# feixue94/sfd2

Measured on AMD Instinct MI355X. Metric: images/sec extract+match (1600x1200, n4096), higher is better.
Workload: dtype f16c

## Files before the change

sfd2_amd/csrc/api_core.hip:

```cpp
#include "sfd2_ctx.h"

static thread_local std::string g_err;
int sfd2_fail(const std::string &m)
{
    g_err = m;
    return -1;
}

std::atomic<unsigned long long> g_alloc_gen{0};

thread_local int g_sfd2_cu_limit = 0;

extern "C" int sfd2_version(void) { return 112; }
extern "C" const char *sfd2_last_error(void) { return g_err.c_str(); }

extern "C" int sfd2_ctx_create(int device, sfd2_ctx **out)
{
    if (!out) return fail("sfd2_ctx_create: out is null");
    int ndev = 0;
    hipError_t e = hipGetDeviceCount(&ndev);
    if (e != hipSuccess || ndev <= 0) return fail("sfd2_ctx_create: no HIP device available (libsfd2hip has no CPU fallback)");
    if (device < 0 || device >= ndev) return fail("sfd2_ctx_create: bad device index");
    HIPCHECK(hipSetDevice(device));
    sfd2_ctx *c = new sfd2_ctx();
    c->device = device;
    HIPCHECK(hipStreamCreateWithFlags(&c->stream, hipStreamNonBlocking));
    for (int i = 0; i < 4; ++i) HIPCHECK(hipEventCreate(&c->ev[i]));
    HIPCHECK(hipEventCreateWithFlags(&c->ev_jobs, hipEventDisableTiming));
    HIPCHECK(hipStreamCreateWithFlags(&c->copy_stream, hipStreamNonBlocking));
    HIPCHECK(hipStreamCreateWithFlags(&c->side_stream, hipStreamNonBlocking));
    HIPCHECK(hipEventCreateWithFlags(&c->ev_fork, hipEventDisableTiming));
    HIPCHECK(hipEventCreateWithFlags(&c->ev_join, hipEventDisableTiming));
    c->cur_stream = c->stream;
    for (int i = 0; i < SFD2_IMG_SLOTS; ++i) {
        HIPCHECK(hipEventCreateWithFlags(&c->ev_copied[i], hipEventDisableTiming));
        HIPCHECK(hipEventCreateWithFlags(&c->ev_img_free[i], hipEventDisableTiming));
    }
    c->fuse = sfd2_env("SFD2_NO_FUSE") ? 0 : 1;
    HIPCHECK(c->zero_page.ensure(SFD2_ZERO_PAGE_BYTES + ((size_t)SFD2_RS_COUNT * (SFD2_RANGE_SUB + 1) + 4) * sizeof(unsigned int)));
    HIPCHECK(hipMemset(c->zero_page.p, 0, c->zero_page.cap));
    c->range_stat.p = c->zero_page.as<char>() + SFD2_ZERO_PAGE_BYTES;
    c->range_hist_dev.p = c->range_stat.as<unsigned int>() + SFD2_RS_COUNT * SFD2_RANGE_SUB;
    c->extract_rec.p = c->range_hist_dev.as<unsigned int>() + SFD2_RS_COUNT;
    static_assert(SFD2_RS_COUNT == SFD2_RANGE_TENSORS && AE_COUNT == SFD2_RANGE_GROUPS, "include/sfd2_hip.h and the internal tables agree");

    *out = c;
    return 0;
}

extern "C" int sfd2_device_pci_bus_id(int device, char *out, int len, int *n_devices)
{
    int ndev = 0;
    hipError_t e = hipGetDeviceCount(&ndev);
    if (e != hipSuccess || ndev <= 0) return fail("sfd2_device_pci_bus_id: no HIP device available");
    if (n_devices) *n_devices = ndev;
    if (device < 0 || device >= ndev) return fail("sfd2_device_pci_bus_id: bad device index");
    if (!out || len < 13) return fail("sfd2_device_pci_bus_id: buffer of at least 13 bytes needed");
    HIPCHECK(hipDeviceGetPCIBusId(out, len, device));
    return 0;
}

extern "C" void sfd2_ctx_destroy(sfd2_ctx *c)
{
    if (!c) return;
    (void)hipSetDevice(c->device);
    (void)hipStreamSynchronize(c->stream);
    graphs_release(c);
    for (int i = 0; i < 4; ++i) if (c->ev[i]) (void)hipEventDestroy(c->ev[i]);
    if (c->ev_jobs) (void)hipEventDestroy(c->ev_jobs);
    for (int i = 0; i < SFD2_IMG_SLOTS; ++i) {
        if (c->ev_copied[i]) (void)hipEventDestroy(c->ev_copied[i]);
        if (c->ev_img_free[i]) (void)hipEventDestroy(c->ev_img_free[i]);
    }
    if (c->copy_stream) (void)hipStreamDestroy(c->copy_stream);
    if (c->side_stream) (void)hipStreamDestroy(c->side_stream);
    if (c->ev_fork) (void)hipEventDestroy(c->ev_fork);
    if (c->ev_join) (void)hipEventDestroy(c->ev_join);
    for (hipEvent_t e : c->prof_ev) (void)hipEventDestroy(e);
    if (c->pin_jobs) (void)hipHostFree(c->pin_jobs);
    if (c->stream) (void)hipStreamDestroy(c->stream);
    delete c;
}

extern "C" void *sfd2_get_stream(sfd2_ctx *c) { return c ? (void *)c->stream : nullptr; }

extern "C" int sfd2_set_precision(sfd2_ctx *c, int mode)
{
    if (!c) return fail("sfd2_set_precision: null ctx");
    if (mode != SFD2_PREC_F16 && mode != SFD2_PREC_F32 && mode != SFD2_PREC_F16X3 && mode != SFD2_PREC_F16C)
        return fail("sfd2_set_precision: unknown mode");
    HIPCHECK(hipSetDevice(c->device));
    HIPCHECK(hipStreamSynchronize(c->stream));
    if (mode != c->precision) graphs_release(c);
    c->precision = mode;
    return sfd2_margin_selfcheck_if_pending(c);
}

extern "C" int sfd2_set_option(sfd2_ctx *c, const char *key, int value)
{
    if (!c || !key) return fail("sfd2_set_option: null argument");
    HIPCHECK(hipSetDevice(c->device));
    HIPCHECK(hipStreamSynchronize(c->stream));
    const std::string k(key);
    graphs_release(c);
    if (k == "fuse") c->fuse = value ? 1 : 0;
    else if (k == "fuse_det") c->fuse_det = value ? 1 : 0;
    else if (k == "alias") c->opt_alias = value ? 1 : 0;
    else if (k == "graphs") c->use_graphs = value ? 1 : 0;
    else if (k == "branches") c->opt_branches = value ? 1 : 0;
    else if (k == "sta_side") c->opt_sta_side = value ? 1 : 0;
    else if (k == "fuse_post") c->opt_fuse_post = value ? 1 : 0;
    else if (k == "sparse_desc") c->opt_sparse_desc = value ? 1 : 0;
    else if (k == "sparse_da3") c->opt_sparse_da3 = value ? 1 : 0;
    else if (k == "cu_limit") c->opt_cu_limit = value < 0 ? 0 : value;
    else if (k == "auto_range") c->opt_auto_range = value ? 1 : 0;
    else if (k == "range_fallback") c->opt_range_fallback = value ? 1 : 0;
    else if (k == "x3_pp") c->opt_x3_pp = value ? 1 : 0;
    else if (k == "x3_desc16") c->opt_x3_desc16 = value ? 1 : 0;
    else if (k == "auto_margin") c->opt_auto_margin = value ? 1 : 0;
    else if (k == "fp6_filters") c->opt_fp6_filters = value ? 1 : 0;
    else if (k == "fp6_acts") c->opt_fp6_acts = value ? 1 : 0;
    else if (k == "s2d") c->opt_s2d = value ? 1 : 0;
    else if (k == "trunk_r1") c->opt_trunk_r1 = value ? 1 : 0;
    else if (k == "fuse_pb") c->opt_fuse_pb = value ? 1 : 0;
    else if (k == "generic_c") c->opt_generic_c = value ? 1 : 0;
    else if (k == "comp_rb") c->opt_comp_rb = value ? 1 : 0;
    else if (k == "no_rf_c") c->opt_no_rf_c = value ? 1 : 0;
    else if (k == "comp_heads") { c->opt_comp_heads = c->user_comp_heads = value ? 1 : 0; c->user_set_comp_heads = true; }
    else if (k == "c3b_plain") { c->user_c3b_plain = value < 0 ? -1 : (value ? 1 : 0); c->opt_c3b_plain = value > 0 ? 1 : 0; }
    else if (k == "comp_det") c->opt_comp_det = value ? 1 : 0;
    else if (k == "fuse_rb23") c->opt_fuse_rb23 = value ? 1 : 0;
    else if (k == "rb_inner") { c->opt_rb_inner = c->user_rb_inner = value < 0 ? 0 : (value > 2 ? 2 : value); c->user_set_rb_inner = true; }
    else return fail("sfd2_set_option: unknown key '" + k + "'");
    return 0;
}

extern "C" int sfd2_get_option(sfd2_ctx *c, const char *key, int *value)
{
    if (!c || !key || !value) return fail("sfd2_get_option: null argument");
    const std::string k(key);
    const struct { const char *name; int v; } tab[] = {
        {"fuse", c->fuse}, {"fuse_det", c->fuse_det}, {"alias", c->opt_alias}, {"graphs", c->use_graphs}, {"branches", c->opt_branches}, {"sta_side", c->opt_sta_side},
        {"fuse_post", c->opt_fuse_post}, {"sparse_desc", c->opt_sparse_desc}, {"sparse_da3", c->opt_sparse_da3}, {"cu_limit", c->opt_cu_limit},
        {"auto_range", c->opt_auto_range}, {"range_fallback", c->opt_range_fallback}, {"x3_pp", c->opt_x3_pp}, {"x3_desc16", c->opt_x3_desc16},
        {"auto_margin", c->opt_auto_margin}, {"fp6_filters", c->opt_fp6_filters}, {"fp6_acts", c->opt_fp6_acts}, {"s2d", c->opt_s2d},
        {"trunk_r1", c->opt_trunk_r1}, {"fuse_pb", c->opt_fuse_pb}, {"generic_c", c->opt_generic_c}, {"comp_rb", c->opt_comp_rb},
        {"no_rf_c", c->opt_no_rf_c}, {"comp_heads", c->opt_comp_heads}, {"c3b_plain", c->opt_c3b_plain}, {"comp_det", c->opt_comp_det},
        {"fuse_rb23", c->opt_fuse_rb23}, {"rb_inner", c->opt_rb_inner},
    };
    for (const auto &e : tab)
        if (k == e.name) { *value = e.v; return 0; }
    return fail("sfd2_get_option: unknown key '" + k + "'");
}

extern "C" int sfd2_sync(sfd2_ctx *c)
{
    if (!c) return fail("sfd2_sync: null ctx");
    HIPCHECK(hipSetDevice(c->device));
    HIPCHECK(hipStreamSynchronize(c->stream));
    return 0;
}

extern "C" int sfd2_set_profiling(sfd2_ctx *c, int max_steps)
{
    if (!c) return fail("sfd2_set_profiling: null ctx");
    HIPCHECK(hipSetDevice(c->device));
    HIPCHECK(hipStreamSynchronize(c->stream));
    if (max_steps < 0 || max_steps > 4096) return fail("sfd2_set_profiling: max_steps out of range");
    const size_t need = (size_t)max_steps * PROF_SLOTS * 2;
    while (c->prof_ev.size() < need) {
        hipEvent_t e;
        HIPCHECK(hipEventCreate(&e));
        c->prof_ev.push_back(e);
    }
    c->prof_max_steps = max_steps;
    c->prof_step = 0;
    c->prof_slot = 0;
    c->prof_used.assign(max_steps, 0);
    c->prof_row.assign((size_t)max_steps * PROF_SLOTS, 0);
    c->prof_tab.clear();
    return 0;
}

extern "C" int sfd2_set_profile_filter(sfd2_ctx *c, const char *substr)
{
    if (!c) return fail("sfd2_set_profile_filter: null ctx");
    c->prof_filter = substr ? substr : "";
    return 0;
}

extern "C" int sfd2_get_layer_timings(sfd2_ctx *c, sfd2_layer_timing *out, int cap, int *n)
{
    if (!c || !n) return fail("sfd2_get_layer_timings: null argument");
    HIPCHECK(hipSetDevice(c->device));
    HIPCHECK(hipStreamSynchronize(c->stream));
    for (int st = 0; st < c->prof_step; ++st)
        for (int sl = 0; sl < c->prof_used[st]; ++sl) {
            float ms = 0.0f;
            const size_t e = ((size_t)st * PROF_SLOTS + sl) * 2;
            const int row = c->prof_row[(size_t)st * PROF_SLOTS + sl];
            if (hipEventElapsedTime(&ms, c->prof_ev[e], c->prof_ev[e + 1]) == hipSuccess) {
                c->prof_tab[row].ms_total += ms;
                c->prof_tab[row].launches += 1;
            }
        }
    c->prof_step = 0;
    *n = (int)c->prof_tab.size();
    if (out)
        for (int i = 0; i < *n && i < cap; ++i) out[i] = c->prof_tab[i];
    return 0;
}

extern "C" int sfd2_get_timings(sfd2_ctx *c, sfd2_timings *out)
{
    if (!c || !out) return fail("sfd2_get_timings: null argument");
    *out = c->tim;
    return 0;
}

static const int kRsGroup[SFD2_RS_COUNT] = {AE_CONV1A, AE_CONV1B, AE_CONV2A, AE_CONV2B, AE_CONV3A, AE_TRUNK, AE_T1_0, AE_T1_1, AE_T1_2,
                                            AE_T2_0, AE_T2_1, AE_T2_2, AE_TRUNK, AE_TRUNK, AE_TRUNK, AE_PA0, AE_DA0};
extern "C" const char *sfd2_range_tensor_name(int i)
{
    static const char *names[SFD2_RS_COUNT] = {"conv1a", "conv1b", "conv2a", "conv2b", "conv3a", "conv3b", "conv4.0.t1", "conv4.1.t1", "conv4.2.t1",
                                               "conv4.0.t2", "conv4.1.t2", "conv4.2.t2", "conv4.0", "conv4.1", "conv4.2", "convPa.0", "convDa.0"};
    return (i >= 0 && i < SFD2_RS_COUNT) ? names[i] : "";
}

static int fetch_range_words(sfd2_ctx *c, unsigned int *raw , bool clear)
{
    const size_t bytes = (size_t)SFD2_RS_COUNT * (SFD2_RANGE_SUB + 1) * sizeof(unsigned int);
    HIPCHECK(hipMemcpyAsync(raw, c->range_stat.p, bytes, hipMemcpyDeviceToHost, c->stream));
    if (clear) HIPCHECK(hipMemsetAsync(c->range_stat.p, 0, bytes, c->stream));
    HIPCHECK(hipStreamSynchronize(c->stream));
    return 0;
}

int read_range_status(sfd2_ctx *c, sfd2_range_status *out, int reset)
{
    unsigned int raw[SFD2_RS_COUNT * (SFD2_RANGE_SUB + 1)];
    if (fetch_range_words(c, raw, reset != 0)) return -1;
    std::memset(out, 0, sizeof(*out));
    out->n_tensors = SFD2_RS_COUNT;
    const unsigned int sat_bits = 0x44E00000u;
    for (int t = 0; t < SFD2_RS_COUNT; ++t) {
        unsigned int m = raw[SFD2_RS_COUNT * SFD2_RANGE_SUB + t];
        for (int s = 0; s < SFD2_RANGE_SUB; ++s) m = std::max(m, raw[t * SFD2_RANGE_SUB + s]);
        float f;
        std::memcpy(&f, &m, 4);
        const bool sat = m >= sat_bits || c->range_hist[t] >= SFD2_C_SAT;
        if (!(f >= c->range_hist[t])) f = c->range_hist[t];
        if (reset) c->range_hist[t] = 0.0f;
        const int e = c->act_exp[kRsGroup[t]];
        out->max_stored[t] = f;
        out->max_value[t] = std::ldexp(f, -e);
        out->exponent[t] = e;
        if (sat) out->saturated |= 1u << t;
        if (f > 0.0f && f < 0.03125f) out->low |= 1u << t;
    }
    out->fallbacks = c->range_fallbacks;
    return 0;
}

int reset_range_records(sfd2_ctx *c)
{
    if (!c->range_stat.p) return 0;
    HIPCHECK(hipMemsetAsync(c->range_stat.p, 0, (size_t)SFD2_RS_COUNT * (SFD2_RANGE_SUB + 1) * sizeof(unsigned int), c->stream));
    for (int t = 0; t < SFD2_RS_COUNT; ++t) c->range_hist[t] = 0.0f;
    return 0;
}

int range_fold_before_sync_extract(sfd2_ctx *c)
{
    if (c->precision != SFD2_PREC_F16C || !c->opt_range_fallback || c->in_fallback) return 0;
    launch_extract_record(c->stream, c->range_stat.as<unsigned int>(), c->range_hist_dev.as<unsigned int>(), nullptr, 0, 0, nullptr);
    HIPCHECK(hipGetLastError());
    return 0;
}

extern "C" int sfd2_get_range_status(sfd2_ctx *c, sfd2_range_status *out, int reset)
{
    if (!c || !out) return fail("sfd2_get_range_status: null argument");
    HIPCHECK(hipSetDevice(c->device));
    return read_range_status(c, out, reset);
}

int range_wants_fallback(sfd2_ctx *c)
{
    if (c->precision != SFD2_PREC_F16C || !c->opt_range_fallback || c->in_fallback) return 0;
    unsigned int raw[SFD2_RS_COUNT * SFD2_RANGE_SUB];
    HIPCHECK(hipMemcpyAsync(raw, c->range_stat.p, sizeof(raw), hipMemcpyDeviceToHost, c->stream));
    HIPCHECK(hipStreamSynchronize(c->stream));
    bool sat = false;
    float mx[SFD2_RS_COUNT];
    for (int t = 0; t < SFD2_RS_COUNT; ++t) {
        unsigned int m = 0;
        for (int s = 0; s < SFD2_RANGE_SUB; ++s) m = std::max(m, raw[t * SFD2_RANGE_SUB + s]);
        std::memcpy(&mx[t], &m, 4);
        sat = sat || m >= 0x44E00000u;
    }
    if (!sat) return 0;
// ... 20 lines not shown
```

sfd2_amd/csrc/api_extract.hip:

```cpp
#include "sfd2_ctx.h"

static int release_image_slot(sfd2_ctx *c);
static int stage_image(sfd2_ctx *c, const void *x, int on_device, int H, int W, const float **dev, int u8 = 0)
{
    if (u8 == 2) {
        const float *raw = nullptr;
        if (on_device) raw = static_cast<const float *>(x);
        else if (stage_image(c, x, 0, H, W, &raw, 3)) return -1;
        HIPCHECK(c->img_u8_packed.ensure((size_t)3 * H * W + 16));
        launch_unpack_rgbx(c->stream, reinterpret_cast<const unsigned char *>(raw), c->img_u8_packed.as<unsigned char>(), (size_t)H * W);
        if (release_image_slot(c)) return -1;
        *dev = c->img_u8_packed.as<float>();
        return 0;
    }
    if (on_device) { *dev = static_cast<const float *>(x); return 0; }
    const size_t bytes = u8 == 3 ? (size_t)4 * H * W : (size_t)3 * H * W * (u8 ? 1 : sizeof(float));
    const int slot = c->img_slot = (c->img_slot + 1) % SFD2_IMG_SLOTS;
    HIPCHECK(c->img2[slot].ensure(bytes));
    HIPCHECK(hipStreamWaitEvent(c->copy_stream, c->ev_img_free[slot], 0));
    HIPCHECK(hipMemcpyAsync(c->img2[slot].p, x, bytes, hipMemcpyHostToDevice, c->copy_stream));
    HIPCHECK(hipEventRecord(c->ev_copied[slot], c->copy_stream));
    HIPCHECK(hipStreamWaitEvent(c->stream, c->ev_copied[slot], 0));
    c->img_slot_used = slot;
    *dev = c->img2[slot].as<float>();
    return 0;
}

static int release_image_slot(sfd2_ctx *c)
{
    if (c->img_slot_used >= 0) {
        HIPCHECK(hipEventRecord(c->ev_img_free[c->img_slot_used], c->stream));
        c->img_slot_used = -1;
    }
    return 0;
}

static int extract_begin(sfd2_ctx *c, int flags)
{
    c->prof_step_entry = c->prof_step;
    if (!(flags & SFD2_FLAG_ASYNC) && range_fold_before_sync_extract(c)) return -1;
    return 0;
}

int copy_out(sfd2_ctx *c, void *dst, const void *src_dev, size_t bytes, int dst_on_device)
{
    if (!dst || bytes == 0) return 0;
    HIPCHECK(hipMemcpyAsync(dst, src_dev, bytes, dst_on_device ? hipMemcpyDeviceToDevice : hipMemcpyDeviceToHost, c->stream));
    return 0;
}

extern "C" int sfd2_det(sfd2_ctx *c, const float *x, int x_on_device, int H, int W, int flags, float *score,
                        float *stability, float *desc, int out_on_device, int *hs, int *ws, int *hc, int *wc)
{
    if (!c || !x) return fail("sfd2_det: null argument");
    if (!c->weights_loaded) return fail("sfd2_det: weights not loaded");
    if (stability && !c->has_sta) return fail("sfd2_det: stability requested but the loaded state_dict has no ConvSta");
    HIPCHECK(hipSetDevice(c->device));
    const PassPlan plan = plan_pass(c, PASS_DET, H, W);
    if (ensure_workspace(c, plan, H, W)) return -1;
    const float *img = nullptr;
    if (stage_image(c, x, x_on_device, H, W, &img)) return -1;
    prof_step_begin(c);
    if (run_network(c, plan, img, (flags & SFD2_FLAG_IMG_NORMALISED) ? 0 : 1)) return -1;
    if (release_image_slot(c)) return -1;
    prof_step_end(c);
    const int HS = 8 * c->H8, WS = 8 * c->W8;
    if (hs) *hs = HS;
    if (ws) *ws = WS;
    if (hc) *hc = c->H4;
    if (wc) *wc = c->W4;
    if (copy_out(c, score, c->score.p, (size_t)HS * WS * sizeof(float), out_on_device)) return -1;
    if (stability) {
        HIPCHECK(c->stab.ensure((size_t)H * W * sizeof(float)));
        launch_heatmap(c->stream, c->score.as<float>(), HS, WS, c->sta.as<float>(), c->H4, c->W4, H, W, nullptr,
                       c->stab.as<float>());
        if (copy_out(c, stability, c->stab.p, (size_t)H * W * sizeof(float), out_on_device)) return -1;
    }
    if (desc) {
        const size_t n = (size_t)c->H4 * c->W4;
        HIPCHECK(c->desc_nchw.ensure(n * 128 * sizeof(float)));
        launch_desc_normalise_nchw(c->stream, c->draw.as<float>(), (int)n, c->desc_nchw.as<float>());
        if (copy_out(c, desc, c->desc_nchw.p, n * 128 * sizeof(float), out_on_device)) return -1;
    }
    HIPCHECK(hipGetLastError());
    if (!(flags & SFD2_FLAG_ASYNC)) HIPCHECK(hipStreamSynchronize(c->stream));
    return 0;
}

static int run_selection(sfd2_ctx *c, const float *heat_dev, int H, int W, float conf_th, int radius, int border,
                         int top_k, float *nms_dense, float *kpts_dev = nullptr, float *scores_dev = nullptr,
                         int Hb = 0, int Wb = 0)
{
    if (Hb <= 0) Hb = H;
    if (Wb <= 0) Wb = W;
    if (radius < 0 || radius > 4) return fail("nms radius must be in [0,4] (reference uses 4)");
    const int sel_cap = top_k > 0 ? std::min(top_k, c->cand_cap) : c->cand_cap;
    c->last_sel_cap = sel_cap;
    HIPCHECK(c->sel.ensure((size_t)sel_cap * 8));
    HIPCHECK(c->sorted.ensure((size_t)sel_cap * 8));
    HIPCHECK(c->kpts.ensure((size_t)sel_cap * 2 * sizeof(float)));
    HIPCHECK(c->kscores.ensure((size_t)sel_cap * sizeof(float)));
    if (!c->counters_clean) HIPCHECK(hipMemsetAsync(c->counters.p, 0, SFD2_COUNTER_BYTES, c->stream));
    c->counters_clean = false;
    bool threshold_done = false;
    {
        ProfScope ps(c, "nms_select", "nms_select_kernel", 0.0, (double)H * W * 4);
        threshold_done = launch_nms_select(c->stream, heat_dev, H, W, radius, conf_th, border, Hb, Wb, nms_dense,
                                           c->cand.as<unsigned long long>(), c->cand_cap, c->counters.as<unsigned int>(), 1, top_k);
    }
    {
        ProfScope ps(c, "topk_sort", "hist_select+compact+rank_sort", 0.0, (double)sel_cap * 24);
        c->kpts_cur = kpts_dev ? kpts_dev : c->kpts.as<float>();
        c->kscores_cur = scores_dev ? scores_dev : c->kscores.as<float>();
        launch_topk_sort(c->stream, threshold_done, c->cand.as<unsigned long long>(), c->cand_cap, top_k,
                         c->sel.as<unsigned long long>(), c->sorted.as<unsigned long long>(), sel_cap,
                         c->counters.as<unsigned int>(), c->bnd.as<unsigned long long>(), W, c->kpts_cur, c->kscores_cur);
    }
    HIPCHECK(hipGetLastError());
    return 0;
}

static int read_counts(sfd2_ctx *c, int64_t cap_out, int *n_out)
{
    unsigned int cnt[4] = {0, 0, 0, 0};
    HIPCHECK(hipMemcpyAsync(cnt, c->counters.p, sizeof(cnt), hipMemcpyDeviceToHost, c->stream));
    HIPCHECK(hipStreamSynchronize(c->stream));
    c->tim.n_candidates = cnt[0];
    if (cnt[0] > (unsigned int)c->cand_cap)
        return fail("candidate buffer overflow: " + std::to_string(cnt[0]) + " NMS survivors > capacity " +
                    std::to_string(c->cand_cap));
    int64_t n = cnt[1];
    if (n > c->last_sel_cap) n = c->last_sel_cap;
    if (cap_out >= 0 && n > cap_out) n = cap_out;
    if (n_out) *n_out = (int)n;
    return 0;
}

extern "C" int sfd2_extract(sfd2_ctx *c, const void *img, int img_on_device, int H, int W, float conf_th, int top_k,
                            int flags, float *kpts_xy, float *scores, float *desc, int out_on_device, int64_t cap_out,
                            int *n_out)
{
    if (!c || !img) return fail("sfd2_extract: null argument");
    if (!c->weights_loaded) return fail("sfd2_extract: weights not loaded");
    if (!(flags & SFD2_FLAG_NO_STABILITY) && !c->has_sta)
        return fail("sfd2_extract: the loaded state_dict has no ConvSta; pass SFD2_FLAG_NO_STABILITY (use_stability=False)");
    HIPCHECK(hipSetDevice(c->device));
    if (extract_begin(c, flags)) return -1;
    const PassPlan plan = plan_pass(c, PASS_EXTRACT, H, W, top_k, desc != nullptr);
    if (ensure_workspace(c, plan, H, W)) return -1;
    const float *img_dev = nullptr;
    const int u8 = (flags & SFD2_FLAG_IMG_U8_HWC) ? 1 : 0;
    if (u8 && (flags & SFD2_FLAG_IMG_NORMALISED)) return fail("sfd2_extract: a uint8 image cannot be pre-normalised");
    if ((flags & SFD2_FLAG_IMG_BGR) && !u8) return fail("sfd2_extract: SFD2_FLAG_IMG_BGR needs SFD2_FLAG_IMG_U8_HWC");
    if ((flags & SFD2_FLAG_IMG_U8_X) && !u8) return fail("sfd2_extract: SFD2_FLAG_IMG_U8_X needs SFD2_FLAG_IMG_U8_HWC");
    if (stage_image(c, img, img_on_device, H, W, &img_dev, u8 ? ((flags & SFD2_FLAG_IMG_U8_X) ? 2 : 1) : 0)) return -1;
    HIPCHECK(hipEventRecord(c->ev[0], c->stream));
    prof_step_begin(c);
    const int in_mode = ((flags & SFD2_FLAG_IMG_NORMALISED) ? 0 : 1) | (u8 ? 2 : 0) | ((flags & SFD2_FLAG_IMG_BGR) ? 4 : 0);
    if (run_network(c, plan, img_dev, in_mode)) return -1;
    if (release_image_slot(c)) return -1;
    HIPCHECK(hipEventRecord(c->ev[1], c->stream));
    const int HS = 8 * c->H8, WS = 8 * c->W8;
    if (plan.skip_pb) {
        ProfScope ps(c, "convPb+heads+heatmap", "pb_heads_heat_kernel", 2.0 * c->H8 * c->W8 * 65 * 256,
                     (double)c->H8 * c->W8 * 512 + (double)H * W * 4);
        launch_pb_heads_heat(c->stream, c->pa_cur, c->H8, c->W8, c->pb.w.as<half_t>(), c->pb.cout_pad, c->pb.scale.as<float>(),
                             c->pb.shift.as<float>(), (flags & SFD2_FLAG_NO_STABILITY) ? nullptr : c->sta.as<float>(), c->H4, c->W4,
                             H, W, c->heat.as<float>(), c->counters.as<unsigned int>(), SFD2_COUNTER_BYTES / 4);
        c->counters_clean = pb_heads_heat_clears(c->H8, c->W8, SFD2_COUNTER_BYTES / 4);
    } else if (plan.skip_head) {
        ProfScope ps(c, "heads+heatmap", "heads_heat_kernel", 0.0, (double)c->H8 * c->W8 * 65 * 4 + (double)H * W * 4);
        launch_heads_heat(c->stream, c->logits.as<float>(), 128, c->H8, c->W8,
                          (flags & SFD2_FLAG_NO_STABILITY) ? nullptr : c->sta.as<float>(), c->H4, c->W4, H, W, c->heat.as<float>());
    } else {
        ProfScope ps(c, "heatmap", "heatmap_kernel", 0.0, (double)H * W * 8);
        launch_heatmap(c->stream, c->score.as<float>(), HS, WS,
                       (flags & SFD2_FLAG_NO_STABILITY) ? nullptr : c->sta.as<float>(), c->H4, c->W4, H, W,
                       c->heat.as<float>(), nullptr);
    }
    const int sel_guess = top_k > 0 ? std::min(top_k, c->cand_cap) : c->cand_cap;
    const bool direct = out_on_device && kpts_xy && scores && cap_out >= sel_guess;
    if (run_selection(c, c->heat.as<float>(), H, W, conf_th, 4, 4, top_k, nullptr, direct ? kpts_xy : nullptr,
                      direct ? scores : nullptr)) return -1;
    const int sel_cap = c->last_sel_cap;
    int64_t ncopy = sel_cap;
    if (cap_out >= 0 && ncopy > cap_out) ncopy = cap_out;
    const bool store64 = desc && (flags & SFD2_FLAG_DESC_STORE64);
    if (store64 && cap_out < 1) return fail("sfd2_extract: SFD2_FLAG_DESC_STORE64 needs cap_out >= 1 (desc is double [128][cap_out])");
    float *desc_dst = nullptr;
    if (desc) {
        if (out_on_device && cap_out >= sel_cap && !store64) {
            desc_dst = desc;
        } else {
            HIPCHECK(c->kdesc.ensure((size_t)sel_cap * 128 * sizeof(float)));
            desc_dst = c->kdesc.as<float>();
        }
        if (plan.sparse_x3 && !plan.desc16) {
            const size_t nin = (size_t)c->H4 * c->W4 * 256;
            const int rows32 = (sel_cap * 4 + 31) / 32;
            HIPCHECK(c->da3_sparse.ensure((size_t)rows32 * 32 * 256 * sizeof(float)));
            HIPCHECK(c->db_sparse.ensure((size_t)rows32 * 32 * 128 * sizeof(float)));
            const ConvW &L3 = c->fda3;
            {
                ProfScope ps(c, "convDa.3", "sparse_da3_kernel<x3>", 2.0 * 4 * sel_cap * 256.0 * 256.0 * 9, (double)sel_cap * (16 * 1024 + 4 * 1024));
                launch_sparse_da3_x3(c->stream, c->x3_da0_planes.as<half_t>(), c->x3_da0_planes.as<half_t>() + nin, c->H4, c->W4, H, W,
                                     L3.wx3p.as<half_t>(), L3.wsl.as<half_t>(), L3.cout_pad, L3.scale.as<float>(), L3.shift.as<float>(), 0, c->kpts_cur,
                                     c->counters.as<unsigned int>() + 1, sel_cap, c->da3_sparse.as<float>(), c->zero_page.as<half_t>());
            }
            if (convf(c, StrictConv{}, "convDb", c->fdb, c->da3_sparse, rows32, 32, c->db_sparse, rows32, 32, 0)) return -1;
            ProfScope ps(c, "sample_desc", "sample_desc_kernel", 0.0, (double)sel_cap * 128 * 4 * 5);
            launch_sample_desc(c->stream, c->db_sparse.as<float>(), c->H4, c->W4, H, W, c->kpts_cur, c->counters.as<unsigned int>() + 1,
                               sel_cap, desc_dst, 1);
        } else if (plan.sparse_da3 || (plan.sparse_x3 && plan.desc16)) {
            HIPCHECK(c->da3_sparse.ensure((size_t)sel_cap * 4 * 256 * sizeof(half_t)));
            {
                ProfScope ps(c, "convDa.3", "sparse_da3_kernel", 2.0 * 4 * sel_cap * 256.0 * 256.0 * 9, (double)sel_cap * (16 * 512 + 4 * 512) + 2.0 * 256 * 256 * 9);
                launch_sparse_da3(c->stream, c->da0_cur, c->H4, c->W4, H, W, c->da3.w.as<half_t>(), c->da3.wsl.as<half_t>(), c->da3.cout_pad, c->da3.scale.as<float>(),
                                  c->da3.shift.as<float>(), 0, c->kpts_cur, c->counters.as<unsigned int>() + 1, sel_cap,
                                  c->da3_sparse.as<half_t>(), c->zero_page.as<half_t>());
            }
            ProfScope ps(c, "desc_head", "desc_head_kernel", 2.0 * 4 * sel_cap * 128 * 256, (double)sel_cap * (4 * 512 + 512));
            launch_desc_head(c->stream, c->da3_sparse.as<half_t>(), c->H4, c->W4, H, W, c->db.w.as<half_t>(), c->db.cout_pad, c->db.scale.as<float>(),
                             c->db.shift.as<float>(), c->kpts_cur, c->counters.as<unsigned int>() + 1, sel_cap, desc_dst, 1);
        } else if (plan.sparse_desc) {
            ProfScope ps(c, "desc_head", "desc_head_kernel", 2.0 * 4 * sel_cap * 128 * 256, (double)sel_cap * (4 * 512 + 512));
            launch_desc_head(c->stream, c->da_cur, c->H4, c->W4, H, W, c->db.w.as<half_t>(), c->db.cout_pad, c->db.scale.as<float>(),
                             c->db.shift.as<float>(), c->kpts_cur, c->counters.as<unsigned int>() + 1, sel_cap, desc_dst);
        } else {
            ProfScope ps(c, "sample_desc", "sample_desc_kernel", 0.0, (double)sel_cap * 128 * 4 * 5);
            launch_sample_desc(c->stream, c->draw.as<float>(), c->H4, c->W4, H, W, c->kpts_cur,
                               c->counters.as<unsigned int>() + 1, sel_cap, desc_dst);
        }
    }
    size_t desc_bytes_fixed = 0;
    if (store64) {
        float *d64_dst = out_on_device ? desc : nullptr;
        if (!out_on_device) {
            HIPCHECK(c->kdesc64.ensure((size_t)128 * cap_out * sizeof(double)));
            d64_dst = c->kdesc64.as<float>();
        }
        ProfScope ps(c, "desc_store64", "desc_store64_kernel", 0.0, (double)sel_cap * 128 * 4 + (double)cap_out * 128 * 8);
        launch_desc_store64(c->stream, desc_dst, c->counters.as<unsigned int>() + 1, sel_cap, reinterpret_cast<double *>(d64_dst), (int)cap_out);
        desc_dst = d64_dst;
        desc_bytes_fixed = (size_t)128 * cap_out * sizeof(double);
    }
    prof_step_end(c);
    HIPCHECK(hipEventRecord(c->ev[2], c->stream));
    HIPCHECK(hipGetLastError());
    if (flags & SFD2_FLAG_ASYNC) {
        if (!direct && copy_out(c, kpts_xy, c->kpts.p, (size_t)ncopy * 2 * sizeof(float), out_on_device)) return -1;
        if (!direct && copy_out(c, scores, c->kscores.p, (size_t)ncopy * sizeof(float), out_on_device)) return -1;
        if (desc && desc_dst != desc && copy_out(c, desc, desc_dst, desc_bytes_fixed ? desc_bytes_fixed : (size_t)ncopy * 128 * sizeof(float), out_on_device)) return -1;
        if (n_out) *n_out = -1;
        return 0;
    }
    int n = 0;
    if (read_counts(c, cap_out, &n)) return -1;
    {
        const int fb = range_wants_fallback(c);
        if (fb < 0) return -1;
        if (fb) {
            FallbackScope scope(c);
            return sfd2_extract(c, img, img_on_device, H, W, conf_th, top_k, flags, kpts_xy, scores, desc, out_on_device, cap_out, n_out);
        }
    }
    if (!direct && copy_out(c, kpts_xy, c->kpts.p, (size_t)n * 2 * sizeof(float), out_on_device)) return -1;
    if (!direct && copy_out(c, scores, c->kscores.p, (size_t)n * sizeof(float), out_on_device)) return -1;
    if (desc && desc_dst != desc && copy_out(c, desc, desc_dst, desc_bytes_fixed ? desc_bytes_fixed : (size_t)n * 128 * sizeof(float), out_on_device)) return -1;
    HIPCHECK(hipStreamSynchronize(c->stream));
    float ms = 0.0f;
    if (hipEventElapsedTime(&ms, c->ev[0], c->ev[2]) == hipSuccess) c->tim.ms_total = ms;
    if (hipEventElapsedTime(&ms, c->ev[0], c->ev[1]) == hipSuccess) c->tim.ms_backbone = ms;
    if (hipEventElapsedTime(&ms, c->ev[1], c->ev[2]) == hipSuccess) c->tim.ms_post = ms;
    if (n_out) *n_out = n;
    return 0;
}

extern "C" int sfd2_preprocess(sfd2_ctx *c, const unsigned char *img_hwc, int on_device, int H, int W, int flags, int new_h,
                               int new_w, float *out_chw_dev)
{
    if (!c || !img_hwc || !out_chw_dev) return fail("sfd2_preprocess: null argument");
    if (H < 1 || W < 1 || new_h < 1 || new_w < 1) return fail("sfd2_preprocess: bad size");
    HIPCHECK(hipSetDevice(c->device));
    const float *staged = nullptr;
    if (stage_image(c, img_hwc, on_device, H, W, &staged, (flags & SFD2_FLAG_IMG_U8_X) ? 2 : 1)) return -1;
    launch_ingest_u8(c->stream, reinterpret_cast<const unsigned char *>(staged), H, W, (flags & SFD2_FLAG_IMG_BGR) ? 1 : 0, new_h,
                     new_w, out_chw_dev);
    if (release_image_slot(c)) return -1;
    HIPCHECK(hipGetLastError());
    if (!(flags & SFD2_FLAG_ASYNC)) HIPCHECK(hipStreamSynchronize(c->stream));
    return 0;
}

extern "C" int sfd2_extract_multiscale(sfd2_ctx *c, const void *img, int img_on_device, int H, int W, const double *scales,
                                       int n_scales, float conf_th, int top_k, int flags, float *kpts_xy, float *scores,
                                       float *desc, int out_on_device, int64_t cap_out, int *n_out)
{
    if (!c || !img || !scales) return fail("sfd2_extract_multiscale: null argument");
    if (n_scales < 1 || n_scales > 8) return fail("sfd2_extract_multiscale: 1..8 scales");
    if (!c->weights_loaded) return fail("sfd2_extract_multiscale: weights not loaded");
    if (!(flags & SFD2_FLAG_NO_STABILITY) && !c->has_sta)
        return fail("sfd2_extract_multiscale: the loaded state_dict has no ConvSta; pass SFD2_FLAG_NO_STABILITY");
    if (flags & SFD2_FLAG_ASYNC) return fail("sfd2_extract_multiscale: SFD2_FLAG_ASYNC is not supported");
    if (flags & SFD2_FLAG_DESC_STORE64) return fail("sfd2_extract_multiscale: SFD2_FLAG_DESC_STORE64 is not supported (single-scale sfd2_extract only)");
    if (!kpts_xy || !scores) return fail("sfd2_extract_multiscale: kpts_xy and scores are required");
    HIPCHECK(hipSetDevice(c->device));
    if (extract_begin(c, 0)) return -1;
    const int u8 = (flags & SFD2_FLAG_IMG_U8_HWC) ? 1 : 0;
    if (u8 && (flags & SFD2_FLAG_IMG_NORMALISED)) return fail("sfd2_extract_multiscale: a uint8 image cannot be pre-normalised");
    if ((flags & SFD2_FLAG_IMG_BGR) && !u8) return fail("sfd2_extract_multiscale: SFD2_FLAG_IMG_BGR needs SFD2_FLAG_IMG_U8_HWC");
    if (flags & SFD2_FLAG_IMG_U8_X) return fail("sfd2_extract_multiscale: SFD2_FLAG_IMG_U8_X is taken by sfd2_extract and sfd2_preprocess only");
    const int in_mode = ((flags & SFD2_FLAG_IMG_NORMALISED) ? 0 : 1) | (u8 ? 2 : 0) | ((flags & SFD2_FLAG_IMG_BGR) ? 4 : 0);
    int nh[8], nw[8], cap[8], off[8];
    int cap_total = 0;
    for (int l = 0; l < n_scales; ++l) {
        nh[l] = scales[l] == 1.0 ? H : (int)((double)H * scales[l]);
        nw[l] = scales[l] == 1.0 ? W : (int)((double)W * scales[l]);
        if (nh[l] < 8 || nw[l] < 8) return fail("sfd2_extract_multiscale: a pyramid level is smaller than 8x8");
        const size_t P1 = (size_t)nh[l] * nw[l];
        const size_t cc = std::min(std::max<size_t>(65536, P1 / 8), P1);
        cap[l] = top_k > 0 ? (int)std::min<size_t>((size_t)top_k, cc) : (int)cc;
        off[l] = cap_total;
        cap_total += cap[l];
    }
    const float *img_dev = nullptr;
    if (stage_image(c, img, img_on_device, H, W, &img_dev, u8)) return -1;
    HIPCHECK(c->ms_kp.ensure((size_t)cap_total * 2 * sizeof(float)));
    HIPCHECK(c->ms_sc.ensure((size_t)cap_total * sizeof(float)));
    if (desc) HIPCHECK(c->ms_de.ensure((size_t)cap_total * 128 * sizeof(float)));
    HIPCHECK(c->ms_keys.ensure((size_t)cap_total * 8));
    HIPCHECK(c->ms_sorted.ensure((size_t)cap_total * 8));
    HIPCHECK(c->ms_cnt.ensure(64));
    HIPCHECK(hipMemsetAsync(c->ms_cnt.p, 0, 64, c->stream));
    unsigned int *level_count = c->ms_cnt.as<unsigned int>();
    unsigned int *ms_counters = level_count + 8;
    HIPCHECK(hipEventRecord(c->ev[0], c->stream));
    for (int l = 0; l < n_scales; ++l) {
        const float *lvl_img = img_dev;
        int mode = in_mode;
        if (nh[l] != H || nw[l] != W) {
            HIPCHECK(c->img_scaled.ensure((size_t)3 * nh[l] * nw[l] * sizeof(float)));
            launch_norm_resize(c->stream, img_dev, in_mode, H, W, nh[l], nw[l], c->img_scaled.as<float>());
            lvl_img = c->img_scaled.as<float>();
            mode = 0;
        }
        const PassPlan plan = plan_pass(c, PASS_DENSE, nh[l], nw[l]);
        if (ensure_workspace(c, plan, nh[l], nw[l])) return -1;
        if (run_network(c, plan, lvl_img, mode)) return -1;
        launch_heatmap(c->stream, c->score.as<float>(), 8 * c->H8, 8 * c->W8,
                       (flags & SFD2_FLAG_NO_STABILITY) ? nullptr : c->sta.as<float>(), c->H4, c->W4, nh[l], nw[l],
                       c->heat.as<float>(), nullptr);
        if (run_selection(c, c->heat.as<float>(), nh[l], nw[l], conf_th, 4, 4, top_k, nullptr, nullptr, nullptr, H, W)) return -1;
        if (c->last_sel_cap != cap[l]) return fail("sfd2_extract_multiscale: internal capacity mismatch");
        if (desc)
            launch_sample_desc(c->stream, c->draw.as<float>(), c->H4, c->W4, nh[l], nw[l], c->kpts_cur,
                               c->counters.as<unsigned int>() + 1, cap[l], c->ms_de.as<float>() + (size_t)off[l] * 128);
        launch_ms_append(c->stream, c->kpts_cur, c->kscores_cur, c->counters.as<unsigned int>() + 1, cap[l], W, nw[l], H, nh[l],
                         c->ms_kp.as<float>() + (size_t)off[l] * 2, c->ms_sc.as<float>() + off[l], level_count + l);
        HIPCHECK(hipMemcpyAsync(c->ms_cand_seen + l, c->counters.p, 4, hipMemcpyDeviceToHost, c->stream));
        c->ms_cand_cap[l] = c->cand_cap;
    }
    if (release_image_slot(c)) return -1;
    const int64_t want = top_k > 0 ? std::min<int64_t>(top_k, cap_total) : cap_total;
    const int64_t n_max = cap_out >= 0 ? std::min<int64_t>(want, cap_out) : want;
    float *kp_dst = kpts_xy, *sc_dst = scores, *de_dst = desc;
    if (!out_on_device) {
        HIPCHECK(c->kpts.ensure((size_t)std::max<int64_t>(n_max, 1) * 2 * sizeof(float)));
        HIPCHECK(c->kscores.ensure((size_t)std::max<int64_t>(n_max, 1) * sizeof(float)));
        kp_dst = c->kpts.as<float>();
        sc_dst = c->kscores.as<float>();
        if (desc) {
            HIPCHECK(c->kdesc.ensure((size_t)std::max<int64_t>(n_max, 1) * 128 * sizeof(float)));
            de_dst = c->kdesc.as<float>();
        }
    }
    launch_ms_merge(c->stream, n_scales, off, level_count, c->ms_kp.as<float>(), c->ms_sc.as<float>(),
                    desc ? c->ms_de.as<float>() : nullptr, cap_total, top_k, c->ms_keys.as<unsigned long long>(),
                    c->ms_sorted.as<unsigned long long>(), ms_counters, (int)n_max, kp_dst, sc_dst, de_dst);
    HIPCHECK(hipEventRecord(c->ev[2], c->stream));
    HIPCHECK(hipGetLastError());
// ... 311 lines not shown
```

sfd2_amd/csrc/api_graph.hip:

```cpp
#include "sfd2_ctx.h"

struct GraphKey {
    int H, W, top_k, flags, k, dim, n0;
    float conf_th;
    sfd2_match_conf conf;
    const void *img, *kp, *sc, *de, *m, *ms;
    unsigned long long db_hash;
    bool operator==(const GraphKey &o) const { return memcmp(this, &o, sizeof(GraphKey)) == 0; }
};
struct GraphEntry {
    GraphKey key;
    hipGraph_t graph = nullptr;
    hipGraphExec_t exec = nullptr;
    unsigned long long gen = 0, last_use = 0;
    int seen = 0;
    void *pin = nullptr;
    size_t pin_cap = 0;
    DevBuf jobs, fins;
};
#define SFD2_MAX_GRAPHS 16

static void graph_entry_release(GraphEntry &e)
{
    if (e.exec) (void)hipGraphExecDestroy(e.exec);
    if (e.graph) (void)hipGraphDestroy(e.graph);
    if (e.pin) (void)hipHostFree(e.pin);
    e.jobs.release();
    e.fins.release();
    e = GraphEntry();
}

void graphs_release(sfd2_ctx *c)
{
    if (!c->graphs) return;
    for (int i = 0; i < c->n_graphs; ++i) graph_entry_release(c->graphs[i]);
    delete[] c->graphs;
    c->graphs = nullptr;
    c->n_graphs = 0;
}

static int extract_match_eager(sfd2_ctx *c, const void *img, int H, int W, float conf_th, int top_k, int flags, float *kp,
                               float *sc, float *de, const sfd2_desc_set *db, int k, int dim, const sfd2_match_conf *conf,
                               int64_t *m, float *ms)
{
    int n_dummy = 0;
    if (sfd2_extract(c, img, 1, H, W, conf_th, top_k, flags | SFD2_FLAG_ASYNC, kp, sc, de, 1, top_k, &n_dummy)) return -1;
    if (k > 0) {
        const sfd2_desc_set q = {de, top_k, SFD2_DT_F32, SFD2_LAYOUT_ND, 1, nullptr, 0, 0};
        if (sfd2_match_batch(c, &q, db, k, dim, conf, m, ms, 1, SFD2_FLAG_ASYNC)) return -1;
    }
    return 0;
}

extern "C" int sfd2_extract_match(sfd2_ctx *c, const void *img_dev, int H, int W, float conf_th, int top_k, int flags,
                                  float *kpts_xy, float *scores, float *desc, const sfd2_desc_set *db, int k, int dim,
                                  const sfd2_match_conf *conf, int64_t *matches0, float *scores0)
{
    if (!c || !img_dev || !kpts_xy || !scores || !desc) return fail("sfd2_extract_match: null argument");
    if (top_k <= 0) return fail("sfd2_extract_match: top_k must be positive (fixed-capacity device outputs)");
    if (flags & SFD2_FLAG_DESC_STORE64) return fail("sfd2_extract_match: SFD2_FLAG_DESC_STORE64 is for stores; the matcher reads the float [n][128] descriptors");
    if (k < 0 || (k > 0 && (!db || !conf || !matches0 || !scores0))) return fail("sfd2_extract_match: null matcher argument");
    for (int i = 0; i < k; ++i)
        if (!db[i].on_device || db[i].rows) return fail("sfd2_extract_match: database sets must be device resident, without row selection");
    HIPCHECK(hipSetDevice(c->device));
    if (!c->use_graphs || c->prof_max_steps > 0)
        return extract_match_eager(c, img_dev, H, W, conf_th, top_k, flags, kpts_xy, scores, desc, db, k, dim, conf, matches0, scores0);

    GraphKey key;
    memset(&key, 0, sizeof(key));
    key.H = H; key.W = W; key.top_k = top_k; key.flags = flags; key.k = k; key.dim = dim; key.n0 = top_k; key.conf_th = conf_th;
    if (conf) key.conf = *conf;
    key.img = img_dev; key.kp = kpts_xy; key.sc = scores; key.de = desc; key.m = matches0; key.ms = scores0;
    unsigned long long h = 1469598103934665603ull;
    for (int i = 0; i < k; ++i) {
        const unsigned long long v[3] = {(unsigned long long)(uintptr_t)db[i].data, (unsigned long long)db[i].n,
                                         ((unsigned long long)db[i].dtype << 8) | (unsigned long long)db[i].layout};
        for (unsigned long long x : v) { h ^= x; h *= 1099511628211ull; }
    }
    key.db_hash = h;
    if (!c->graphs) { c->graphs = new GraphEntry[SFD2_MAX_GRAPHS]; c->n_graphs = SFD2_MAX_GRAPHS; }
    GraphEntry *e = nullptr, *lru = &c->graphs[0];
    for (int i = 0; i < c->n_graphs; ++i) {
        GraphEntry &g = c->graphs[i];
        if (g.seen && g.key == key) { e = &g; break; }
        if (g.last_use < lru->last_use) lru = &g;
    }
    if (!e) {
        graph_entry_release(*lru);
        e = lru;
        e->key = key;
    }
    e->last_use = ++c->graph_clock;
    if (e->exec && e->gen == g_alloc_gen) {
        HIPCHECK(hipGraphLaunch(e->exec, c->stream));
        return 0;
    }
    if (e->exec) {
        (void)hipGraphExecDestroy(e->exec); e->exec = nullptr;
        (void)hipGraphDestroy(e->graph); e->graph = nullptr;
        e->seen = 0;
    }
    if (e->seen == 0) {
        e->seen = 1;
        return extract_match_eager(c, img_dev, H, W, conf_th, top_k, flags, kpts_xy, scores, desc, db, k, dim, conf, matches0, scores0);
    }
    const size_t jb = 2 * (size_t)std::max(k, 1) * sizeof(MatchJob), fb = (size_t)std::max(k, 1) * sizeof(MatchFinal);
    if (!e->pin) {
        HIPCHECK(hipHostMalloc(&e->pin, jb + fb, hipHostMallocDefault));
        e->pin_cap = jb + fb;
        HIPCHECK(e->jobs.ensure(jb + fb));
    }
    HIPCHECK(hipStreamSynchronize(c->stream));
    HIPCHECK(hipEventSynchronize(c->ev_jobs));
    const unsigned long long gen0 = g_alloc_gen.load();
    std::swap(c->pin_jobs, e->pin); std::swap(c->pin_cap, e->pin_cap);
    std::swap(c->m_jobs, e->jobs); std::swap(c->m_fins, e->fins);
    hipError_t be = hipStreamBeginCapture(c->stream, hipStreamCaptureModeThreadLocal);
    int rc = -1;
    hipGraph_t g = nullptr;
    if (be == hipSuccess) {
        rc = extract_match_eager(c, img_dev, H, W, conf_th, top_k, flags, kpts_xy, scores, desc, db, k, dim, conf, matches0, scores0);
        const hipError_t ee = hipStreamEndCapture(c->stream, &g);
        if (ee != hipSuccess) rc = fail(std::string("hipStreamEndCapture: ") + hipGetErrorString(ee));
    } else {
        fail(std::string("hipStreamBeginCapture: ") + hipGetErrorString(be));
    }
    std::swap(c->pin_jobs, e->pin); std::swap(c->pin_cap, e->pin_cap);
    std::swap(c->m_jobs, e->jobs); std::swap(c->m_fins, e->fins);
    if (rc != 0 || g_alloc_gen != gen0) {
        if (g) (void)hipGraphDestroy(g);
        e->seen = 0;
        if (rc == 0) return fail("sfd2_extract_match: workspace changed during capture");
        return -1;
    }
    e->graph = g;
    HIPCHECK(hipGraphInstantiate(&e->exec, g, nullptr, nullptr, 0));
    e->gen = g_alloc_gen;
    HIPCHECK(hipGraphLaunch(e->exec, c->stream));
    return 0;
}
```

sfd2_amd/csrc/api_match.hip:

```cpp
#include "sfd2_ctx.h"

static size_t elt_size(int dtype) { return dtype == SFD2_DT_F64 ? 8 : (dtype == SFD2_DT_F16 ? 2 : 4); }

static int prep_set(sfd2_ctx *c, const void *src, int n_src, const int32_t *rows, int n, int dim, int dtype, int layout,
                    int on_device, int need_lo, DevBuf &stage, size_t &stage_off, half_t *hi_dst, half_t *lo_dst,
                    const half_t **hi, const half_t **lo, const int **rows_dev = nullptr)
{
    if (rows_dev) *rows_dev = nullptr;
    if (!rows && dtype == SFD2_DT_F16 && layout == SFD2_LAYOUT_ND && on_device && dim == 128 && !need_lo) {
        *hi = reinterpret_cast<const half_t *>(src);
        *lo = nullptr;
        return 0;
    }
    const void *dev_src = src;
    if (!on_device) {
        const size_t bytes = (size_t)n_src * dim * elt_size(dtype);
        void *dst = reinterpret_cast<char *>(stage.p) + stage_off;
        HIPCHECK(hipMemcpyAsync(dst, src, bytes, hipMemcpyHostToDevice, c->stream));
        dev_src = dst;
        stage_off += (bytes + 255) & ~(size_t)255;
    }
    const int *rd = nullptr;
    if (rows) {
        void *dst = reinterpret_cast<char *>(stage.p) + stage_off;
        HIPCHECK(hipMemcpyAsync(dst, rows, (size_t)n * sizeof(int32_t), hipMemcpyHostToDevice, c->stream));
        rd = reinterpret_cast<const int *>(dst);
        stage_off += ((size_t)n * sizeof(int32_t) + 255) & ~(size_t)255;
        if (rows_dev) *rows_dev = rd;
    }
    launch_match_prep(c->stream, dev_src, n, n_src, rd, dim, dtype, layout, hi_dst, need_lo ? lo_dst : nullptr);
    *hi = hi_dst;
    *lo = need_lo ? lo_dst : nullptr;
    return 0;
}

extern "C" int sfd2_desc_pack(sfd2_ctx *c, const sfd2_desc_set *src, int dim, void *dst_f16_dev, int flags)
{
    if (!c || !src || !dst_f16_dev) return fail("sfd2_desc_pack: null argument");
    if (dim <= 0 || dim > 128) return fail("descriptor dimension must be in [1,128]");
    if (src->n < 0 || src->n_rows < 0) return fail("negative size");
    if (src->dtype != SFD2_DT_F32 && src->dtype != SFD2_DT_F64 && src->dtype != SFD2_DT_F16) return fail("sfd2_desc_pack: unknown dtype");
    if (src->layout != SFD2_LAYOUT_ND && src->layout != SFD2_LAYOUT_DN) return fail("sfd2_desc_pack: unknown layout");
    const int n = src->rows ? src->n_rows : src->n;
    if (n == 0) return 0;
    if (!src->data) return fail("sfd2_desc_pack: null descriptors");
    if (src->rows)
        for (int r = 0; r < src->n_rows; ++r)
            if (src->rows[r] < 0 || src->rows[r] >= src->n) return fail("sfd2_desc_pack: row index out of range");
    HIPCHECK(hipSetDevice(c->device));
    size_t stage_bytes = 256;
    if (!src->on_device) stage_bytes += (((size_t)src->n * dim * elt_size(src->dtype)) + 255) & ~(size_t)255;
    if (src->rows) stage_bytes += ((size_t)n * sizeof(int32_t) + 255) & ~(size_t)255;
    HIPCHECK(c->m_stage.ensure(stage_bytes));
    size_t off = 0;
    void *dev_src = const_cast<void *>(src->data);
    if (!src->on_device) {
        const size_t bytes = (size_t)src->n * dim * elt_size(src->dtype);
        HIPCHECK(hipMemcpyAsync(c->m_stage.p, src->data, bytes, hipMemcpyHostToDevice, c->stream));
        dev_src = c->m_stage.p;
        off += (bytes + 255) & ~(size_t)255;
    }
    const int *rd = nullptr;
    if (src->rows) {
        void *dst = c->m_stage.as<char>() + off;
        HIPCHECK(hipMemcpyAsync(dst, src->rows, (size_t)n * sizeof(int32_t), hipMemcpyHostToDevice, c->stream));
        rd = reinterpret_cast<const int *>(dst);
    }
    launch_match_prep(c->stream, dev_src, n, src->n, rd, dim, src->dtype, src->layout, reinterpret_cast<half_t *>(dst_f16_dev), nullptr);
    HIPCHECK(hipGetLastError());
    if (!(flags & SFD2_FLAG_ASYNC)) HIPCHECK(hipStreamSynchronize(c->stream));
    return 0;
}

extern "C" int sfd2_match_batch(sfd2_ctx *c, const sfd2_desc_set *q, const sfd2_desc_set *db, int k, int dim,
                                const sfd2_match_conf *conf, int64_t *matches0, float *scores0, int out_on_device,
                                int flags)
{
    if (!c || !conf || !q || (k > 0 && !db)) return fail("sfd2_match_batch: null argument");
    if (dim <= 0 || dim > 128) return fail("descriptor dimension must be in [1,128]");
    const int n0 = q->n;
    if (n0 < 0 || k < 0) return fail("negative size");
    if (k == 0 || n0 == 0) return 0;
    if (!q->data) return fail("sfd2_match_batch: null query descriptors");
    HIPCHECK(hipSetDevice(c->device));
    const int need_lo = conf->sim_mode == SFD2_SIM_F16X2;
    const bool o16 = (flags & SFD2_FLAG_MATCH_OUT16) != 0;
    const size_t msz = o16 ? sizeof(short) : sizeof(long long), ssz = o16 ? sizeof(half_t) : sizeof(float);
    int max_n1 = 0;
    size_t tot_n1 = 0, stage_bytes = 0;
    if (q->rows) return fail("sfd2_match_batch: row selection applies to database sets only");
    std::vector<int> eff_n1(k);
    for (int i = 0; i < k; ++i) {
        if (db[i].n < 0 || db[i].n_rows < 0) return fail("negative n1");
        if (db[i].n > 0 && !db[i].data) return fail("sfd2_match_batch: null database descriptors");
        if (db[i].rows)
            for (int r = 0; r < db[i].n_rows; ++r)
                if (db[i].rows[r] < 0 || db[i].rows[r] >= db[i].n) return fail("sfd2_match_batch: row index out of range");
        eff_n1[i] = db[i].rows ? db[i].n_rows : db[i].n;
        max_n1 = std::max(max_n1, eff_n1[i]);
        tot_n1 += (size_t)eff_n1[i];
        if (!db[i].on_device) stage_bytes += (((size_t)db[i].n * dim * elt_size(db[i].dtype)) + 255) & ~(size_t)255;
        if (db[i].rows) stage_bytes += ((size_t)db[i].n_rows * sizeof(int32_t) + 255) & ~(size_t)255;
    }
    if (!q->on_device) stage_bytes += (((size_t)n0 * dim * elt_size(q->dtype)) + 255) & ~(size_t)255;
    const int max_n = std::max(n0, max_n1);
    const int blocks_per_job = (max_n + 255) / 256;
    int splits = (768 * 6 + 2 * k * blocks_per_job - 1) / (2 * k * blocks_per_job);
    splits = std::max(1, std::min(splits, 8));
    const int min_n = std::max(1, std::min(n0, max_n1 > 0 ? max_n1 : 1));
    splits = std::min(splits, std::max(1, (min_n + 31) / 32));
    if (const char *e = sfd2_env("SFD2_MATCH_SPLITS")) splits = std::max(1, std::min(16, atoi(e)));

    const int need_top2 = (conf->flavour == SFD2_MATCH_ITLOC_NNR) ||
                          (conf->flavour == SFD2_MATCH_HLOC && conf->ratio_threshold > 0.0f);
    const bool single_gemm = !need_lo && !need_top2 && sfd2_env("SFD2_MATCH_TWO_GEMM") == nullptr;
    if (single_gemm) {
        const int qblocks = (n0 + 255) / 256;
        splits = (512 * 6 + k * qblocks - 1) / (k * qblocks);
        splits = std::max(1, std::min(splits, 8));
        splits = std::min(splits, std::max(1, (std::max(1, max_n1) + 31) / 32));
        if (const char *e = sfd2_env("SFD2_MATCH_SPLITS")) splits = std::max(1, std::min(16, atoi(e)));
        splits = std::max(splits, (max_n1 + match_mutual_max_chunk() - 1) / match_mutual_max_chunk());
    }
    const int nstrip = (n0 + match_mutual_strip() - 1) / match_mutual_strip();

    HIPCHECK(c->m_stage.ensure(std::max<size_t>(stage_bytes, 256)));
    HIPCHECK(c->m_hi0.ensure((size_t)n0 * 128 * 2));
    if (need_lo) HIPCHECK(c->m_lo0.ensure((size_t)n0 * 128 * 2));
    HIPCHECK(c->m_hi1.ensure(std::max<size_t>(tot_n1, 1) * 128 * 2));
    if (need_lo) HIPCHECK(c->m_lo1.ensure(std::max<size_t>(tot_n1, 1) * 128 * 2));
    const size_t per_pair_f = (size_t)splits * n0, tot_part = (size_t)k * per_pair_f + (size_t)splits * tot_n1;
    HIPCHECK(c->m_part_f.ensure(std::max<size_t>(tot_part, 1) * 2 * sizeof(float)));
    HIPCHECK(c->m_part_i.ensure(std::max<size_t>(tot_part, 1) * sizeof(int)));
    if (single_gemm) HIPCHECK(c->m_rkeys.ensure(std::max<size_t>((size_t)nstrip * tot_n1, 1) * sizeof(float)));
    HIPCHECK(c->m_red.ensure(((size_t)k * n0 + tot_n1 + 1) * 3 * sizeof(float)));
    HIPCHECK(c->m_jobs.ensure((size_t)2 * k * sizeof(MatchJob) + (size_t)k * sizeof(MatchFinal)));
    HIPCHECK(c->m_out_m.ensure((size_t)k * n0 * sizeof(long long)));
    HIPCHECK(c->m_out_s.ensure((size_t)k * n0 * sizeof(float)));

    HIPCHECK(hipEventRecord(c->ev[0], c->stream));
    prof_step_begin(c);
    size_t stage_off = 0;
    const half_t *q_hi = nullptr, *q_lo = nullptr;
    if (prep_set(c, q->data, n0, nullptr, n0, dim, q->dtype, q->layout, q->on_device, need_lo, c->m_stage, stage_off,
                 c->m_hi0.as<half_t>(), c->m_lo0.as<half_t>(), &q_hi, &q_lo)) return -1;
    static_assert(sizeof(MatchJob2) <= 2 * sizeof(MatchJob), "descriptor buffer sizing");
    const size_t jobs_bytes = 2 * (size_t)k * sizeof(MatchJob), fins_bytes = (size_t)k * sizeof(MatchFinal);
    hipStreamCaptureStatus cap_status = hipStreamCaptureStatusNone;
    (void)hipStreamIsCapturing(c->stream, &cap_status);
    const bool capturing = cap_status != hipStreamCaptureStatusNone;
    if (!capturing) HIPCHECK(hipEventSynchronize(c->ev_jobs));
    if (jobs_bytes + fins_bytes > c->pin_cap) {
        if (c->pin_jobs) (void)hipHostFree(c->pin_jobs);
        c->pin_jobs = nullptr;
        c->pin_cap = 0;
        HIPCHECK(hipHostMalloc(&c->pin_jobs, jobs_bytes + fins_bytes, hipHostMallocDefault));
        c->pin_cap = jobs_bytes + fins_bytes;
    }
    MatchJob *jobs = reinterpret_cast<MatchJob *>(c->pin_jobs);
    MatchJob2 *jobs2 = reinterpret_cast<MatchJob2 *>(c->pin_jobs);
    MatchFinal *fins = reinterpret_cast<MatchFinal *>(reinterpret_cast<char *>(c->pin_jobs) + jobs_bytes);
    float *pf = c->m_part_f.as<float>();
    int *pi = c->m_part_i.as<int>();
    float *red = c->m_red.as<float>();
    size_t off1 = 0, poff = 0, roff = 0;
    for (int i = 0; i < k; ++i) {
        const int n1 = eff_n1[i];
        const half_t *h = nullptr, *l = nullptr;
        const int *remap = nullptr;
        if (n1 > 0) {
            if (prep_set(c, db[i].data, db[i].n, db[i].rows, n1, dim, db[i].dtype, db[i].layout, db[i].on_device, need_lo,
                         c->m_stage, stage_off, c->m_hi1.as<half_t>() + off1 * 128,
                         need_lo ? c->m_lo1.as<half_t>() + off1 * 128 : nullptr, &h, &l, &remap))
                return -1;
        }
        MatchFinal &fn = fins[i];
        fn.remap = remap;
        if (single_gemm) {
            MatchJob2 &j2 = jobs2[i];
            j2.q_hi = q_hi; j2.d_hi = h; j2.n0 = n0; j2.n1 = n1;
            j2.part_v1 = pf + 2 * poff; j2.part_i1 = pi + poff;
            j2.rkeys = c->m_rkeys.as<float>() + (size_t)nstrip * off1;
            poff += (size_t)splits * n0 + (size_t)splits * n1;
            fn.f_v1 = fn.f_v2 = fn.r_v1 = fn.r_v2 = nullptr; fn.f_i1 = fn.r_i1 = nullptr;
        } else {
            MatchJob &f = jobs[2 * i], &r = jobs[2 * i + 1];
            f.a_hi = h; f.a_lo = l; f.b_hi = q_hi; f.b_lo = q_lo; f.na = n1; f.nb = n0;
            f.part_v1 = pf + 2 * poff; f.part_v2 = pf + 2 * poff + (size_t)splits * n0; f.part_i1 = pi + poff;
            poff += (size_t)splits * n0;
            r.a_hi = q_hi; r.a_lo = q_lo; r.b_hi = h; r.b_lo = l; r.na = n0; r.nb = n1;
            r.part_v1 = pf + 2 * poff; r.part_v2 = pf + 2 * poff + (size_t)splits * n1; r.part_i1 = pi + poff;
            poff += (size_t)splits * n1;
            fn.f_v1 = f.part_v1; fn.f_v2 = f.part_v2; fn.f_i1 = f.part_i1;
            fn.r_v1 = r.part_v1; fn.r_v2 = r.part_v2; fn.r_i1 = r.part_i1;
        }
        off1 += (size_t)n1;
        fn.n0 = n0; fn.n1 = n1;
        fn.out16 = o16 ? 1 : 0; fn.pad_ = 0;
        const bool direct_out = out_on_device && matches0 && scores0;
        fn.matches0 = reinterpret_cast<long long *>((direct_out ? reinterpret_cast<char *>(matches0) : c->m_out_m.as<char>()) + (size_t)i * n0 * msz);
        fn.scores0 = reinterpret_cast<float *>((direct_out ? reinterpret_cast<char *>(scores0) : c->m_out_s.as<char>()) + (size_t)i * n0 * ssz);
        fn.red_f = red + 3 * roff; roff += (size_t)n0;
        fn.red_r = red + 3 * roff; roff += (size_t)n1;
    }
    HIPCHECK(hipMemcpyAsync(c->m_jobs.p, jobs, jobs_bytes + fins_bytes, hipMemcpyHostToDevice, c->stream));
    MatchFinal *fins_dev = reinterpret_cast<MatchFinal *>(static_cast<char *>(c->m_jobs.p) + jobs_bytes);
    if (!capturing) HIPCHECK(hipEventRecord(c->ev_jobs, c->stream));
    if (single_gemm) {
        {
            ProfScope ps(c, "match_mutual", "match_mutual_kernel", 2.0 * (double)n0 * (double)tot_n1 * 128.0,
                         2.0 * ((double)k * n0 + (double)tot_n1) * 128.0);
            launch_match_mutual(c->stream, c->m_jobs.as<MatchJob2>(), fins_dev, k, n0, max_n1, splits,
                                conf->flavour == SFD2_MATCH_HLOC && !conf->do_mutual_check);
        }
        {
            ProfScope ps(c, "match_finalize", "match_decide", 0.0, (double)tot_part * 12);
            launch_match_decide(c->stream, fins_dev, k, max_n, conf->flavour, conf->do_mutual_check,
                                conf->ratio_threshold, conf->distance_threshold);
        }
    } else {
        {
            ProfScope ps(c, "match_top2", need_lo ? "match_top2_kernel<x2>" : "match_top2_kernel",
                         2.0 * 2.0 * (double)n0 * (double)tot_n1 * 128.0 * (need_lo ? 3.0 : 1.0),
                         2.0 * 2.0 * ((double)k * n0 + (double)tot_n1) * 128.0);
            launch_match_top2(c->stream, c->m_jobs.as<MatchJob>(), 2 * k, max_n, splits, need_lo, need_top2,
                              c->zero_page.as<half_t>());
        }
        {
            ProfScope ps(c, "match_finalize", "match_reduce+decide", 0.0, (double)tot_part * 12);
            launch_match_finalize(c->stream, fins_dev, k, max_n, splits, conf->flavour,
                                  conf->do_mutual_check, conf->ratio_threshold, conf->distance_threshold);
        }
    }
    prof_step_end(c);
    HIPCHECK(hipGetLastError());
    HIPCHECK(hipEventRecord(c->ev[3], c->stream));
    if (!(out_on_device && matches0 && scores0)) {
        if (copy_out(c, matches0, c->m_out_m.p, (size_t)k * n0 * msz, out_on_device)) return -1;
        if (copy_out(c, scores0, c->m_out_s.p, (size_t)k * n0 * ssz, out_on_device)) return -1;
    }
    if (!(flags & SFD2_FLAG_ASYNC)) {
        HIPCHECK(hipStreamSynchronize(c->stream));
        float ms = 0.0f;
        if (hipEventElapsedTime(&ms, c->ev[0], c->ev[3]) == hipSuccess) c->tim.ms_match = ms;
    }
    return 0;
}

extern "C" int sfd2_match_segments(sfd2_ctx *c, const void *d0, int n0, const void *d1, int n1, int dim, int dtype, int layout,
                                   int on_device, int n_seg, const int32_t *seg0, const int32_t *seg1,
                                   const sfd2_match_conf *conf, int64_t *matches0, float *scores0, int out_on_device)
{
    if (!c || !conf || !seg0 || !seg1 || !matches0 || !scores0) return fail("sfd2_match_segments: null argument");
    if (dim <= 0 || dim > 128) return fail("descriptor dimension must be in [1,128]");
    if (n0 < 0 || n1 < 0 || n_seg < 0) return fail("negative size");
    if (n0 == 0) return 0;
    if (!d0 || (n1 > 0 && !d1)) return fail("sfd2_match_segments: null descriptors");
    if (seg0[0] != 0 || seg1[0] != 0 || seg0[n_seg] != n0 || seg1[n_seg] != n1) return fail("sfd2_match_segments: segment offsets must span [0, n]");
    for (int i = 0; i < n_seg; ++i)
        if (seg0[i + 1] < seg0[i] || seg1[i + 1] < seg1[i]) return fail("sfd2_match_segments: segment offsets must ascend");
    HIPCHECK(hipSetDevice(c->device));
    const int need_lo = conf->sim_mode == SFD2_SIM_F16X2;
    const int need_top2 = (conf->flavour == SFD2_MATCH_ITLOC_NNR) || (conf->flavour == SFD2_MATCH_HLOC && conf->ratio_threshold > 0.0f);
    const bool single_gemm = !need_lo && !need_top2;
    std::vector<int> live;
    int max_a = 0, max_b = 0;
    for (int i = 0; i < n_seg; ++i)
        if (seg0[i + 1] > seg0[i] && seg1[i + 1] > seg1[i]) {
            live.push_back(i);
            max_a = std::max(max_a, seg0[i + 1] - seg0[i]);
            max_b = std::max(max_b, seg1[i + 1] - seg1[i]);
        }
    const int k = (int)live.size();
    HIPCHECK(c->m_out_m.ensure((size_t)n0 * sizeof(long long)));
    HIPCHECK(c->m_out_s.ensure((size_t)n0 * sizeof(float)));
    long long *out_m = out_on_device ? reinterpret_cast<long long *>(matches0) : c->m_out_m.as<long long>();
    float *out_s = out_on_device ? scores0 : c->m_out_s.as<float>();
    HIPCHECK(hipMemsetAsync(out_m, 0xFF, (size_t)n0 * sizeof(long long), c->stream));
    HIPCHECK(hipMemsetAsync(out_s, 0, (size_t)n0 * sizeof(float), c->stream));
    if (k > 0) {
        int splits = std::max(1, (max_b + match_mutual_max_chunk() - 1) / match_mutual_max_chunk());
        const int strip = match_mutual_strip();
        size_t stage_bytes = 256 + (((size_t)n1 * sizeof(int32_t)) + 255);
        if (!on_device) stage_bytes += ((((size_t)n0 + n1) * dim * elt_size(dtype)) + 511);
        HIPCHECK(c->m_stage.ensure(stage_bytes));
        HIPCHECK(c->m_hi0.ensure((size_t)n0 * 128 * 2));
        HIPCHECK(c->m_hi1.ensure((size_t)std::max(n1, 1) * 128 * 2));
        if (need_lo) { HIPCHECK(c->m_lo0.ensure((size_t)n0 * 128 * 2)); HIPCHECK(c->m_lo1.ensure((size_t)std::max(n1, 1) * 128 * 2)); }
        const size_t tot_part = (size_t)splits * ((size_t)n0 + n1);
        HIPCHECK(c->m_part_f.ensure(tot_part * 2 * sizeof(float)));
        HIPCHECK(c->m_part_i.ensure(tot_part * sizeof(int)));
        size_t rk = 0;
        for (int i : live) rk += (size_t)((seg0[i + 1] - seg0[i] + strip - 1) / strip) * (size_t)(seg1[i + 1] - seg1[i]);
        if (single_gemm) HIPCHECK(c->m_rkeys.ensure(std::max<size_t>(rk, 1) * sizeof(float)));
        HIPCHECK(c->m_red.ensure(((size_t)n0 + n1 + 1) * 3 * sizeof(float)));
        HIPCHECK(c->m_jobs.ensure((size_t)2 * k * sizeof(MatchJob) + (size_t)k * sizeof(MatchFinal)));
        prof_step_begin(c);
        size_t stage_off = 0;
        const half_t *h0 = nullptr, *l0 = nullptr, *h1 = nullptr, *l1 = nullptr;
        if (prep_set(c, d0, n0, nullptr, n0, dim, dtype, layout, on_device, need_lo, c->m_stage, stage_off, c->m_hi0.as<half_t>(),
                     c->m_lo0.as<half_t>(), &h0, &l0)) return -1;
        if (prep_set(c, d1, n1, nullptr, n1, dim, dtype, layout, on_device, need_lo, c->m_stage, stage_off, c->m_hi1.as<half_t>(),
                     c->m_lo1.as<half_t>(), &h1, &l1)) return -1;
        std::vector<int32_t> iota((size_t)n1);
        for (int i = 0; i < n1; ++i) iota[i] = i;
        int32_t *iota_dev = reinterpret_cast<int32_t *>(reinterpret_cast<char *>(c->m_stage.p) + ((stage_off + 255) & ~(size_t)255));
        HIPCHECK(hipMemcpyAsync(iota_dev, iota.data(), (size_t)n1 * sizeof(int32_t), hipMemcpyHostToDevice, c->stream));
        HIPCHECK(hipStreamSynchronize(c->stream));
        const size_t jobs_bytes = 2 * (size_t)k * sizeof(MatchJob), fins_bytes = (size_t)k * sizeof(MatchFinal);
        HIPCHECK(hipEventSynchronize(c->ev_jobs));
        if (jobs_bytes + fins_bytes > c->pin_cap) {
            if (c->pin_jobs) (void)hipHostFree(c->pin_jobs);
            c->pin_jobs = nullptr;
            c->pin_cap = 0;
            HIPCHECK(hipHostMalloc(&c->pin_jobs, jobs_bytes + fins_bytes, hipHostMallocDefault));
            c->pin_cap = jobs_bytes + fins_bytes;
        }
        MatchJob *jobs = reinterpret_cast<MatchJob *>(c->pin_jobs);
        MatchJob2 *jobs2 = reinterpret_cast<MatchJob2 *>(c->pin_jobs);
        MatchFinal *fins = reinterpret_cast<MatchFinal *>(reinterpret_cast<char *>(c->pin_jobs) + jobs_bytes);
        float *pf = c->m_part_f.as<float>();
        int *pi = c->m_part_i.as<int>();
        float *red = c->m_red.as<float>();
        size_t poff = 0, roff = 0, rkoff = 0;
        for (int j = 0; j < k; ++j) {
            const int sg = live[j], a0 = seg0[sg], na = seg0[sg + 1] - a0, b0 = seg1[sg], nb = seg1[sg + 1] - b0;
            MatchFinal &fn = fins[j];
            fn.out16 = 0; fn.pad_ = 0;
            fn.remap = iota_dev + b0;
            if (single_gemm) {
                MatchJob2 &j2 = jobs2[j];
                j2.q_hi = h0 + (size_t)a0 * 128; j2.d_hi = h1 + (size_t)b0 * 128; j2.n0 = na; j2.n1 = nb;
                j2.part_v1 = pf + 2 * poff; j2.part_i1 = pi + poff;
                j2.rkeys = c->m_rkeys.as<float>() + rkoff;
                rkoff += (size_t)((na + strip - 1) / strip) * nb;
                poff += (size_t)splits * na + (size_t)splits * nb;
                fn.f_v1 = fn.f_v2 = fn.r_v1 = fn.r_v2 = nullptr; fn.f_i1 = fn.r_i1 = nullptr;
            } else {
                MatchJob &f = jobs[2 * j], &r = jobs[2 * j + 1];
                f.a_hi = h1 + (size_t)b0 * 128; f.a_lo = l1 ? l1 + (size_t)b0 * 128 : nullptr;
                f.b_hi = h0 + (size_t)a0 * 128; f.b_lo = l0 ? l0 + (size_t)a0 * 128 : nullptr; f.na = nb; f.nb = na;
                f.part_v1 = pf + 2 * poff; f.part_v2 = pf + 2 * poff + (size_t)splits * na; f.part_i1 = pi + poff;
                poff += (size_t)splits * na;
                r.a_hi = f.b_hi; r.a_lo = f.b_lo; r.b_hi = f.a_hi; r.b_lo = f.a_lo; r.na = na; r.nb = nb;
                r.part_v1 = pf + 2 * poff; r.part_v2 = pf + 2 * poff + (size_t)splits * nb; r.part_i1 = pi + poff;
                poff += (size_t)splits * nb;
                fn.f_v1 = f.part_v1; fn.f_v2 = f.part_v2; fn.f_i1 = f.part_i1;
                fn.r_v1 = r.part_v1; fn.r_v2 = r.part_v2; fn.r_i1 = r.part_i1;
            }
            fn.n0 = na; fn.n1 = nb;
            fn.matches0 = out_m + a0;
            fn.scores0 = out_s + a0;
            fn.red_f = red + 3 * roff; roff += (size_t)na;
            fn.red_r = red + 3 * roff; roff += (size_t)nb;
        }
        HIPCHECK(hipMemcpyAsync(c->m_jobs.p, jobs, jobs_bytes + fins_bytes, hipMemcpyHostToDevice, c->stream));
        MatchFinal *fins_dev = reinterpret_cast<MatchFinal *>(static_cast<char *>(c->m_jobs.p) + jobs_bytes);
        HIPCHECK(hipEventRecord(c->ev_jobs, c->stream));
        const int max_n = std::max(max_a, max_b);
        if (single_gemm) {
            ProfScope ps(c, "match_segments", "match_mutual_kernel", 0.0, 0.0);
            launch_match_mutual(c->stream, c->m_jobs.as<MatchJob2>(), fins_dev, k, max_a, max_b, splits,
                                conf->flavour == SFD2_MATCH_HLOC && !conf->do_mutual_check);
            launch_match_decide(c->stream, fins_dev, k, max_n, conf->flavour, conf->do_mutual_check,
                                conf->ratio_threshold, conf->distance_threshold);
        } else {
// ... 24 lines not shown
```

sfd2_amd/csrc/match_kernels.hip:

```cpp
#include "sfd2_internal.h"
#include <math.h>
#include <stdlib.h>

#define NT 256
#define KD 128
#define TA 64
#define APITCH 136

__global__ __launch_bounds__(NT)
void match_prep_kernel(const void *__restrict__ src, int n, int n_src, const int *__restrict__ rows, int dim, int dtype,
                       int layout, half_t *__restrict__ hi, half_t *__restrict__ lo)
{
    const size_t t = (size_t)blockIdx.x * blockDim.x + threadIdx.x;
    if (t >= (size_t)n * KD) return;
    const int i = (int)(t / KD), d = (int)(t % KD);
    double v = 0.0;
    if (d < dim) {
        const int r = rows ? rows[i] : i;
        const size_t off = layout == 0 ? (size_t)r * dim + d : (size_t)d * n_src + r;
        if (dtype == 0) v = (double)reinterpret_cast<const float *>(src)[off];
        else if (dtype == 1) v = reinterpret_cast<const double *>(src)[off];
        else v = (double)(float)reinterpret_cast<const half_t *>(src)[off];
    }
    const half_t h = (half_t)(float)v;
// ... 185 lines not shown
        const int ja = ja0 + (stage_)*TA2 + row;                                                          \
        const half_t *src = ja < ja1 ? job.a_hi + (size_t)ja * KD + slot * 8 : zero_page + (lane & 3) * 8; \
        __builtin_amdgcn_global_load_lds((gbl_void_t *)src,                                              \
                                         (lds_void_t *)(smem + (buf_)*TA2 * 256 + (wave * (TA2 / 16) + c) * 1024), 16, 0, 0); \
    }
        ISSUE_A(0, 0)
        SFD2_BARRIER_DRAIN();
        for (int s = 0; s < nst; ++s) {
            const int buf = s & 1;
            if (s + 1 < nst) { ISSUE_A(s + 1, buf ^ 1) }
#pragma unroll
            for (int sub = 0; sub < TA2 / 32; ++sub) {
                f32x16_t acc0 = zero16, acc1 = zero16;
                const int row = sub * 32 + lcol;
                const unsigned char *arow = smem + (buf * TA2 + row) * 256;
                const int sw = row & 15;
#pragma unroll
                for (int ks = 0; ks < 8; ++ks) {
                    const h8_t a = *reinterpret_cast<const h8_t *>(arow + (((ks * 2 + lhi) ^ sw) << 4));
                    acc0 = __builtin_amdgcn_mfma_f32_32x32x16_f16(a, bq[0][ks], acc0, 0, 0, 0);
                    acc1 = __builtin_amdgcn_mfma_f32_32x32x16_f16(a, bq[1][ks], acc1, 0, 0, 0);
                }
                const int jbase = ja0 + s * TA2 + sub * 32 + 4 * lhi;
                const bool full = ja0 + s * TA2 + sub * 32 + 32 <= ja1;
                if (ABL == 1) {
                    bp[0] = fmaxf(bp[0], acc0[0] + acc0[5] + acc0[10] + acc0[15]);
                    bp[1] = fmaxf(bp[1], acc1[0] + acc1[5] + acc1[10] + acc1[15]);
                } else if (!NEED2 && full) {
                    const int sub_id = s * (TA2 / 32) + sub;
                    float m0 = -INFINITY, m1 = -INFINITY;
#pragma unroll
                    for (int r = 0; r < 16; ++r) {
                        const float p0 = __uint_as_float((__float_as_uint(acc0[r]) & 0xFFFFFFF0u) | (unsigned)(15 - r));
                        const float p1 = __uint_as_float((__float_as_uint(acc1[r]) & 0xFFFFFFF0u) | (unsigned)(15 - r));
                        m0 = fmaxf(m0, p0);
                        m1 = fmaxf(m1, p1);
                    }
                    sid[0] = m0 > bp[0] ? sub_id : sid[0]; bp[0] = fmaxf(bp[0], m0);
                    sid[1] = m1 > bp[1] ? sub_id : sid[1]; bp[1] = fmaxf(bp[1], m1);
                } else {
#pragma unroll
                    for (int r = 0; r < 16; ++r) {
                        const int j = jbase + (r & 3) + 8 * (r >> 2);
                        const bool in = j < ja1;
                        const float v0 = in ? acc0[r] : -INFINITY, v1 = in ? acc1[r] : -INFINITY;
                        if (NEED2) {
                            top2_update(v0, j, b1[0], b2[0], i1[0]);
                            top2_update(v1, j, b1[1], b2[1], i1[1]);
                        } else {
                            i1[0] = v0 > b1[0] ? j : i1[0]; b1[0] = fmaxf(b1[0], v0);
                            i1[1] = v1 > b1[1] ? j : i1[1]; b1[1] = fmaxf(b1[1], v1);
                        }
                    }
                }
            }
            SFD2_BARRIER_DRAIN();
        }
#undef ISSUE_A
    }
    if (!NEED2) {
#pragma unroll
        for (int t = 0; t < 2; ++t) {
            const unsigned int bits = __float_as_uint(bp[t]);
            const float v = __uint_as_float(bits & 0xFFFFFFF0u);
            const int r = 15 - (int)(bits & 15u);
            const int j = ja0 + sid[t] * 32 + (r & 3) + 8 * (r >> 2) + 4 * lhi;
            if (bp[t] != -INFINITY && (v > b1[t] || (v == b1[t] && j < i1[t]))) { b1[t] = v; i1[t] = j; }
        }
    }
#pragma unroll
    for (int t = 0; t < 2; ++t) {
        const float c1 = __shfl_xor(b1[t], 32), c2 = __shfl_xor(b2[t], 32);
        const int j1 = __shfl_xor(i1[t], 32);
        float n1v, n2v;
        int n1i;
        if (c1 > b1[t] || (c1 == b1[t] && j1 < i1[t])) { n1v = c1; n1i = j1; n2v = fmaxf(b1[t], c2); }
        else { n1v = b1[t]; n1i = i1[t]; n2v = fmaxf(b2[t], c1); }
        const int qi = i_base + wave * 64 + t * 32 + lcol;
        if (lane < 32 && qi < nb) {
            const size_t o = (size_t)blockIdx.y * nb + qi;
            job.part_v1[o] = n1v;
            job.part_v2[o] = NEED2 ? n2v : -INFINITY;
            job.part_i1[o] = n1i;
        }
    }
}

#define MQ_NEG (-0x1p100f)
void launch_match_mutual_gemm(hipStream_t st, const MatchJob2 *jobs_dev, int npairs, int max_n0, int splits, int fwd_ids);
int match_mutual_strip(void);

__global__ __launch_bounds__(NT)
void match_mutual_reduce_kernel(const MatchJob2 *__restrict__ jobs, const MatchFinal *__restrict__ fins, int splits, int strip, int fwd_ids)
{
    const MatchJob2 job = jobs[blockIdx.y];
    const MatchFinal f = fins[blockIdx.y];
    const int dir = blockIdx.z;
    const int n = dir == 0 ? job.n0 : job.n1;
    const int i = blockIdx.x * blockDim.x + threadIdx.x;
    if (i >= n) return;
    float b1 = -INFINITY;
    int bi = 0;
    if (dir == 0) {
        for (int s = 0; s < splits; ++s) {
            const float c1 = job.part_v1[(size_t)s * n + i];
            if (c1 > b1) { b1 = c1; if (fwd_ids) bi = job.part_i1[(size_t)s * n + i]; }
        }
        if (!fwd_ids) bi = -1;
        f.red_f[i] = b1;
        f.red_f[(size_t)n + i] = -INFINITY;
        reinterpret_cast<int *>(f.red_f)[2 * (size_t)n + i] = bi;
    } else {
        const int nstrip = (job.n0 + strip - 1) / strip;
        float best = MQ_NEG;
        unsigned int bkey = __float_as_uint(MQ_NEG);
        int bs = 0;
        int sidx = 0;
        for (; sidx + 8 <= nstrip; sidx += 8) {
            float k[8];
#pragma unroll
            for (int u = 0; u < 8; ++u) k[u] = job.rkeys[(size_t)(sidx + u) * n + i];
#pragma unroll
            for (int u = 0; u < 8; ++u) {
                const float v = __uint_as_float(__float_as_uint(k[u]) & 0xFFFFFF00u);
                if (v > best) { best = v; bkey = __float_as_uint(k[u]); bs = sidx + u; }
            }
        }
        for (; sidx < nstrip; ++sidx) {
            const float k = job.rkeys[(size_t)sidx * n + i];
            const float v = __uint_as_float(__float_as_uint(k) & 0xFFFFFF00u);
            if (v > best) { best = v; bkey = __float_as_uint(k); bs = sidx; }
        }
        const unsigned int bits = bkey;
        const bool any = best > MQ_NEG;
        f.red_r[i] = any ? __uint_as_float(bits & 0xFFFFFF00u) : -INFINITY;
        f.red_r[(size_t)n + i] = -INFINITY;
        reinterpret_cast<int *>(f.red_r)[2 * (size_t)n + i] = any ? bs * strip + 255 - (int)(bits & 255u) : 0;
    }
}

__global__ __launch_bounds__(NT)
void match_mutual_claim_kernel(const MatchFinal *__restrict__ fins)
{
    const MatchFinal f = fins[blockIdx.y];
    const int j = blockIdx.x * blockDim.x + threadIdx.x;
    if (j >= f.n1) return;
    const float r = f.red_r[j];
    if (!(r > -INFINITY)) return;
    const int i = reinterpret_cast<const int *>(f.red_r)[2 * (size_t)f.n1 + j];
    if ((__float_as_uint(f.red_f[i]) & 0xFFFFFF00u) == __float_as_uint(r))
        atomicMin(reinterpret_cast<unsigned int *>(f.red_f) + 2 * (size_t)f.n0 + i, (unsigned int)j);
}

void launch_match_mutual(hipStream_t st, const MatchJob2 *jobs_dev, const MatchFinal *fins_dev, int npairs, int max_n0,
                         int max_n1, int splits, int fwd_ids)
{
    if (npairs <= 0 || max_n0 <= 0) return;
    launch_match_mutual_gemm(st, jobs_dev, npairs, max_n0, splits, fwd_ids);
    const int max_n = max_n0 > max_n1 ? max_n0 : max_n1;
    hipLaunchKernelGGL(match_mutual_reduce_kernel, dim3((max_n + NT - 1) / NT, npairs, 2), dim3(NT), 0, st, jobs_dev, fins_dev, splits,
                       match_mutual_strip(), fwd_ids);
    if (!fwd_ids && max_n1 > 0)
        hipLaunchKernelGGL(match_mutual_claim_kernel, dim3((max_n1 + NT - 1) / NT, npairs), dim3(NT), 0, st, fins_dev);
}

void launch_match_top2(hipStream_t st, const MatchJob *jobs_dev, int njobs, int max_nb, int splits, int use_lo,
                       int need_top2, const half_t *zero_page)
{
    if (njobs <= 0 || max_nb <= 0) return;
    static bool attr_done = false;
    const size_t lds_hi = (size_t)2 * TA * APITCH * sizeof(half_t);
    if (!attr_done) {
        (void)hipFuncSetAttribute(reinterpret_cast<const void *>(match_top2_kernel<true>),
                                  hipFuncAttributeMaxDynamicSharedMemorySize, (int)(2 * lds_hi));
        attr_done = true;
    }
    if (!use_lo && zero_page && sfd2_env("SFD2_MATCH_V1") == nullptr) {
        const dim3 grid((max_nb + 255) / 256, splits, njobs);
        const size_t lds = (size_t)2 * TA2 * 256;
        static bool attr2 = false;
        if (!attr2) {
            (void)hipFuncSetAttribute(reinterpret_cast<const void *>(match_top2_v2_kernel<true>), hipFuncAttributeMaxDynamicSharedMemorySize, (int)lds);
            (void)hipFuncSetAttribute(reinterpret_cast<const void *>(match_top2_v2_kernel<false>), hipFuncAttributeMaxDynamicSharedMemorySize, (int)lds);
#ifdef SFD2_EXPERIMENTS
            (void)hipFuncSetAttribute(reinterpret_cast<const void *>(match_top2_v2_kernel<false, 1>), hipFuncAttributeMaxDynamicSharedMemorySize, (int)lds);
#endif
            attr2 = true;
        }
        if (need_top2) hipLaunchKernelGGL(match_top2_v2_kernel<true>, grid, dim3(NT), lds, st, jobs_dev, splits, zero_page);
#ifdef SFD2_EXPERIMENTS
        else if (sfd2_env("SFD2_MATCH_ABLATE")) hipLaunchKernelGGL((match_top2_v2_kernel<false, 1>), grid, dim3(NT), lds, st, jobs_dev, splits, zero_page);
#endif
        else hipLaunchKernelGGL(match_top2_v2_kernel<false>, grid, dim3(NT), lds, st, jobs_dev, splits, zero_page);
        return;
    }
    const dim3 grid((max_nb + 127) / 128, splits, njobs);
    if (use_lo) hipLaunchKernelGGL(match_top2_kernel<true>, grid, dim3(NT), 2 * lds_hi, st, jobs_dev, splits);
    else hipLaunchKernelGGL(match_top2_kernel<false>, grid, dim3(NT), lds_hi, st, jobs_dev, splits);
}

__global__ __launch_bounds__(NT)
void match_reduce_kernel(const MatchFinal *__restrict__ fins, int splits)
{
    const MatchFinal f = fins[blockIdx.y];
    const int dir = blockIdx.z;
    const int n = dir == 0 ? f.n0 : f.n1;
    const int i = blockIdx.x * blockDim.x + threadIdx.x;
    if (i >= n) return;
    const float *v1 = dir == 0 ? f.f_v1 : f.r_v1;
    const float *v2 = dir == 0 ? f.f_v2 : f.r_v2;
    const int *i1 = dir == 0 ? f.f_i1 : f.r_i1;
    float *red = dir == 0 ? f.red_f : f.red_r;
    float b1 = -INFINITY, b2 = -INFINITY;
    int bi = 0;
    for (int s = 0; s < splits; ++s) {
        const float c1 = v1[(size_t)s * n + i], c2 = v2[(size_t)s * n + i];
        const int ci = i1[(size_t)s * n + i];
        if (c1 > b1) { b2 = fmaxf(b1, c2); b1 = c1; bi = ci; }
        else { b2 = fmaxf(b2, c1); }
    }
    red[i] = b1;
    red[(size_t)n + i] = b2;
    reinterpret_cast<int *>(red)[2 * (size_t)n + i] = bi;
}

__device__ __forceinline__ bool hloc_pass(float s1, float s2, float ratio, float dist)
{
    const float d0 = 2.0f * (1.0f - s1), d1 = 2.0f * (1.0f - s2);
    bool ok = true;
    if (ratio > 0.0f) ok = ok && (d0 <= (ratio * ratio) * d1);
    if (dist > 0.0f) ok = ok && (d0 <= dist * dist);
    return ok;
}
__device__ __forceinline__ float lowe_ratio(float s1, float s2)
{
    const float d0 = sqrtf(fmaxf(2.0f - 2.0f * s1, 0.0f)), d1 = sqrtf(fmaxf(2.0f - 2.0f * s2, 0.0f));
    return d0 / (d1 + 1e-8f);
}

__global__ __launch_bounds__(NT)
void match_decide_kernel(const MatchFinal *__restrict__ fins, int flavour, int mutual, float ratio, float dist)
{
    const MatchFinal f = fins[blockIdx.y];
    const int i = blockIdx.x * blockDim.x + threadIdx.x;
    if (i >= f.n0) return;
    const float s1 = f.red_f[i], s2 = f.red_f[(size_t)f.n0 + i];
    const int j = reinterpret_cast<const int *>(f.red_f)[2 * (size_t)f.n0 + i];
    long long m = -1;
    float score = 0.0f;
    if (f.n1 > 0 && j < 0) {
        score = flavour == 0 ? (hloc_pass(s1, s2, ratio, dist) ? (s1 + 1.0f) / 2.0f : 0.0f) : s1;
    } else if (f.n1 > 0) {
        const float t1 = f.red_r[j], t2 = f.red_r[(size_t)f.n1 + j];
        const int back = reinterpret_cast<const int *>(f.red_r)[2 * (size_t)f.n1 + j];
        if (flavour == 0) {
            const bool ok = hloc_pass(s1, s2, ratio, dist);
            score = ok ? (s1 + 1.0f) / 2.0f : 0.0f;
            m = ok ? j : -1;
            if (ok && mutual) {
                const bool ok_back = hloc_pass(t1, t2, ratio, dist);
                if (!(ok_back && back == i)) m = -1;
            }
        } else if (flavour == 1) {
            score = s1;
            m = (back == i) ? j : -1;
        } else {
            score = s1;
            const bool ok = (back == i) && lowe_ratio(s1, s2) <= ratio && lowe_ratio(t1, t2) <= ratio;
            m = ok ? j : -1;
        }
    }
    const long long mm = (m >= 0 && f.remap) ? (long long)f.remap[m] : m;
    if (f.out16) {
        reinterpret_cast<short *>(f.matches0)[i] = (short)mm;
        reinterpret_cast<half_t *>(f.scores0)[i] = (half_t)score;
    } else {
        f.matches0[i] = mm;
        f.scores0[i] = score;
    }
}

void launch_match_decide(hipStream_t st, const MatchFinal *fin_dev, int npairs, int max_n, int flavour, int mutual,
                         float ratio, float dist)
{
    if (npairs <= 0 || max_n <= 0) return;
    hipLaunchKernelGGL(match_decide_kernel, dim3((max_n + NT - 1) / NT, npairs), dim3(NT), 0, st, fin_dev, flavour,
                       mutual, ratio, dist);
}

void launch_match_finalize(hipStream_t st, const MatchFinal *fin_dev, int npairs, int max_n, int splits, int flavour,
                           int mutual, float ratio, float dist)
{
    if (npairs <= 0 || max_n <= 0) return;
    hipLaunchKernelGGL(match_reduce_kernel, dim3((max_n + NT - 1) / NT, npairs, 2), dim3(NT), 0, st, fin_dev, splits);
    hipLaunchKernelGGL(match_decide_kernel, dim3((max_n + NT - 1) / NT, npairs), dim3(NT), 0, st, fin_dev, flavour,
                       mutual, ratio, dist);
}
```

sfd2_amd/csrc/post_kernels.hip:

```cpp
#include "sfd2_internal.h"
#include <math.h>
#include <stdlib.h>

#define NT 256

__device__ __forceinline__ float wave_sum(float v)
{
#pragma unroll
    for (int m = 32; m >= 1; m >>= 1) v += __shfl_xor(v, m);
    return v;
}

__global__ __launch_bounds__(NT)
void detector_head_kernel(const float *__restrict__ logits, int pitch, int hc, int wc, float *__restrict__ score)
{
    const int lane = threadIdx.x & 63;
    const int cell = blockIdx.x * (NT / 64) + (threadIdx.x >> 6);
    if (cell >= hc * wc) return;
    const int y = cell / wc, x = cell - y * wc;
    const float *p = logits + (size_t)cell * pitch;
    const float e = expf(p[lane]);
    const float ed = expf(p[64]);
    const float den = (wave_sum(e) + ed) + 0.00001f;
    score[(size_t)(8 * y + (lane >> 3)) * (8 * wc) + 8 * x + (lane & 7)] = e / den;
// ... 193 lines not shown
{
    const float st_y = hc > 0 ? (float)hc / (float)H : 1.0f, st_x = wc > 0 ? (float)wc / (float)W : 1.0f;
    const int cells = hc8 * wc8;
    const int grid = (cells + PH_CELLS - 1) / PH_CELLS;
    if (grid * NT < n_zero) zero_words = nullptr;
    hipLaunchKernelGGL(pb_heads_heat_kernel, dim3(grid), dim3(NT), 0, st, fmap, hc8, wc8, wpk, CoutP,
                       scale, shift, sta, hc, wc, st_y, st_x, H, W, heat, zero_words, n_zero);
}

bool pb_heads_heat_clears(int hc8, int wc8, int n_zero) { return ((hc8 * wc8 + PH_CELLS - 1) / PH_CELLS) * NT >= n_zero; }

#define NMS_TH 32
#define NMS_TW 64
#define NMS_RMAX 4
#define NMS_RH (NMS_TH + 10 * NMS_RMAX)
#define NMS_RW (NMS_TW + 10 * NMS_RMAX)
#define NMS_N (NMS_RH * NMS_RW)

__device__ __forceinline__ void pool_rows(const float *__restrict__ src, float *__restrict__ dst, int r)
{
    for (int i = threadIdx.x; i < NMS_N; i += blockDim.x) {
        const int y = i / NMS_RW, x = i - y * NMS_RW;
        const int a = x - r < 0 ? 0 : x - r, b = x + r >= NMS_RW ? NMS_RW - 1 : x + r;
        float m = src[y * NMS_RW + a];
        for (int t = a + 1; t <= b; ++t) m = fmaxf(m, src[y * NMS_RW + t]);
        dst[i] = m;
    }
}
__device__ __forceinline__ void pool_cols(const float *__restrict__ src, float *__restrict__ dst, int r)
{
    for (int i = threadIdx.x; i < NMS_N; i += blockDim.x) {
        const int y = i / NMS_RW, x = i - y * NMS_RW;
        const int a = y - r < 0 ? 0 : y - r, b = y + r >= NMS_RH ? NMS_RH - 1 : y + r;
        float m = src[a * NMS_RW + x];
        for (int t = a + 1; t <= b; ++t) m = fmaxf(m, src[t * NMS_RW + x]);
        dst[i] = m;
    }
}

__global__ __launch_bounds__(512)
void nms_select_kernel(const float *__restrict__ heat, int H, int W, int radius, float conf_th, int border, int Hb, int Wb,
                       float *__restrict__ nms_dense, unsigned long long *__restrict__ cand, int cand_cap,
                       unsigned int *__restrict__ counters)
{
    extern __shared__ __attribute__((aligned(16))) unsigned char smem[];
    float *S = reinterpret_cast<float *>(smem);
    float *A = S + NMS_N;
    float *B = A + NMS_N;
    unsigned char *M = reinterpret_cast<unsigned char *>(B + NMS_N);
    const int halo = 5 * radius;
    const int gy0 = blockIdx.y * NMS_TH - halo, gx0 = blockIdx.x * NMS_TW - halo;
    const float NEG = -INFINITY;

    for (int i = threadIdx.x; i < NMS_N; i += blockDim.x) {
        const int y = i / NMS_RW, x = i - y * NMS_RW;
        const int gy = gy0 + y, gx = gx0 + x;
        S[i] = (gy >= 0 && gy < H && gx >= 0 && gx < W) ? heat[(size_t)gy * W + gx] : NEG;
    }
    __syncthreads();
    pool_rows(S, A, radius);
    __syncthreads();
    pool_cols(A, B, radius);
    __syncthreads();
    for (int i = threadIdx.x; i < NMS_N; i += blockDim.x) {
        const bool oob = S[i] == NEG;
        const bool mk = !oob && (S[i] == B[i]);
        M[i] = mk ? 1 : 0;
        B[i] = mk ? 1.0f : 0.0f;
    }
    __syncthreads();
    for (int it = 0; it < 2; ++it) {
        pool_rows(B, A, radius);
        __syncthreads();
        pool_cols(A, B, radius);
        __syncthreads();
        for (int i = threadIdx.x; i < NMS_N; i += blockDim.x) {
            const bool oob = S[i] == NEG;
            const bool supp = B[i] > 0.0f;
            M[i] = (M[i] & 1) | (supp ? 2 : 0);
            B[i] = oob ? NEG : (supp ? 0.0f : S[i]);
        }
        __syncthreads();
        pool_rows(B, A, radius);
        __syncthreads();
        pool_cols(A, B, radius);
        __syncthreads();
        for (int i = threadIdx.x; i < NMS_N; i += blockDim.x) {
            const bool oob = S[i] == NEG;
            const bool supp = (M[i] & 2) != 0;
            const float ss = supp ? 0.0f : S[i];
            const bool new_max = (ss == B[i]);
            bool mk = (M[i] & 1) != 0;
            if (!oob && new_max && !supp) mk = true;
            M[i] = mk ? 1 : 0;
            B[i] = mk ? 1.0f : 0.0f;
        }
        __syncthreads();
    }
    for (int i = threadIdx.x; i < NMS_TH * NMS_TW; i += blockDim.x) {
        const int ty = i / NMS_TW, tx = i - ty * NMS_TW;
        const int gy = blockIdx.y * NMS_TH + ty, gx = blockIdx.x * NMS_TW + tx;
        if (gy >= H || gx >= W) continue;
        const int li = (ty + halo) * NMS_RW + tx + halo;
        const float v = M[li] ? S[li] : 0.0f;
        if (nms_dense) nms_dense[(size_t)gy * W + gx] = v;
        if (cand && v > conf_th && gx >= border && gx < Wb - border && gy >= border && gy < Hb - border) {
            const unsigned int idx = (unsigned int)(gy * W + gx);
            const unsigned long long key =
                ((unsigned long long)__float_as_uint(v) << 32) | (unsigned long long)(0xFFFFFFFFu - idx);
            const unsigned int pos = atomicAdd(&counters[0], 1u);
            if (pos < (unsigned int)cand_cap) cand[pos] = key;
        }
    }
}

__global__ __launch_bounds__(NT)
void hist_from_cand_kernel(const unsigned long long *__restrict__ cand, int cand_cap,
                           const unsigned int *__restrict__ counters, unsigned int *__restrict__ hist)
{
    unsigned int n = counters[0];
    if (n > (unsigned int)cand_cap) n = cand_cap;
    for (unsigned int i = blockIdx.x * blockDim.x + threadIdx.x; i < n; i += gridDim.x * blockDim.x)
        atomicAdd(&hist[key_bin(cand[i])], 1u);
}

bool launch_nms_select(hipStream_t st, const float *heat, int H, int W, int radius, float conf_th, int border, int Hb, int Wb,
                       float *nms_dense, unsigned long long *cand, int cand_cap, unsigned int *counters, int fuse_threshold, int top_k)
{
    unsigned int *hist = counters + 16;
    if (radius == 4) {
        launch_nms4_select(st, heat, H, W, conf_th, border, Hb, Wb, nms_dense, cand, cand_cap, counters, hist, fuse_threshold, top_k);
        return fuse_threshold != 0 && cand != nullptr;
    }
    static bool attr_done = false;
    const size_t lds = (size_t)NMS_N * (3 * sizeof(float) + 1);
    if (!attr_done) {
        (void)hipFuncSetAttribute(reinterpret_cast<const void *>(nms_select_kernel),
                                  hipFuncAttributeMaxDynamicSharedMemorySize, (int)lds);
        attr_done = true;
    }
    hipLaunchKernelGGL(nms_select_kernel, dim3((W + NMS_TW - 1) / NMS_TW, (H + NMS_TH - 1) / NMS_TH), dim3(512), lds,
                       st, heat, H, W, radius, conf_th, border, Hb, Wb, nms_dense, cand, cand_cap, counters);
    if (cand) hipLaunchKernelGGL(hist_from_cand_kernel, dim3(64), dim3(NT), 0, st, cand, cand_cap, counters, hist);
    return false;
}

__global__ __launch_bounds__(1024)
void select_threshold_kernel(int cand_cap, int top_k, unsigned int *__restrict__ counters)
{
    __shared__ unsigned int wsum[16];
    sfd2_select_threshold<false>(cand_cap, top_k, counters, wsum);
}

__global__ __launch_bounds__(NT)
void compact_selected_kernel(const unsigned long long *__restrict__ cand, int cand_cap,
                             unsigned long long *__restrict__ sel, int sel_cap,
                             unsigned long long *__restrict__ bnd, unsigned int *__restrict__ counters)
{
    unsigned int n = counters[0];
    if (n > (unsigned int)cand_cap) n = cand_cap;
    const unsigned int bstar = counters[4], all = counters[6];
    const int lane = threadIdx.x & 63;
    const unsigned long long below = (1ull << lane) - 1ull;
    const unsigned int stride = gridDim.x * blockDim.x;
    for (unsigned int i0 = blockIdx.x * blockDim.x; i0 < n; i0 += stride) {
        const unsigned int i = i0 + threadIdx.x;
        const bool live = i < n;
        const unsigned long long key = live ? cand[i] : 0ull;
        const unsigned int bin = key_bin(key);
        const bool to_sel = live && (all || bin > bstar), to_bnd = live && !to_sel && bin == bstar;
        const unsigned long long ms = __ballot(to_sel), mb = __ballot(to_bnd);
        unsigned int base_s = 0, base_b = 0;
        if (lane == 0) {
            if (ms) base_s = atomicAdd(&counters[2], (unsigned int)__popcll(ms));
            if (mb) base_b = atomicAdd(&counters[3], (unsigned int)__popcll(mb));
        }
        base_s = __shfl(base_s, 0);
        base_b = __shfl(base_b, 0);
        if (to_sel) {
            const unsigned int pos = base_s + (unsigned int)__popcll(ms & below);
            if (pos < (unsigned int)sel_cap) sel[pos] = key;
        } else if (to_bnd) {
            __hip_atomic_store(bnd + base_b + (unsigned int)__popcll(mb & below), key, __ATOMIC_RELAXED, __HIP_MEMORY_SCOPE_AGENT);
        }
    }
    __shared__ unsigned int s_last;
    SFD2_BARRIER_DRAIN();
    if (threadIdx.x == 0) s_last = atomicAdd(&counters[8], 1u) == gridDim.x - 1 ? 1u : 0u;
    __syncthreads();
    if (!s_last) return;
    const unsigned int nb = sfd2_ld_agent(counters + 3), need = counters[5], k = counters[1];
    if (counters[6] || need == 0) return;
    __shared__ unsigned long long tile[NT];
    const unsigned int base_out = k - need;
    for (unsigned int i0 = 0; i0 < nb; i0 += blockDim.x) {
        const unsigned int i = i0 + threadIdx.x;
        const unsigned long long mine = i < nb ? __hip_atomic_load(bnd + i, __ATOMIC_RELAXED, __HIP_MEMORY_SCOPE_AGENT) : 0ull;
        unsigned int rank = 0;
        for (unsigned int b = 0; b < nb; b += NT) {
            tile[threadIdx.x] = (b + threadIdx.x < nb) ? __hip_atomic_load(bnd + b + threadIdx.x, __ATOMIC_RELAXED, __HIP_MEMORY_SCOPE_AGENT) : 0ull;
            __syncthreads();
            const unsigned int lim = nb - b < NT ? nb - b : NT;
            for (unsigned int t = 0; t < lim; ++t) rank += tile[t] > mine ? 1u : 0u;
            __syncthreads();
        }
        if (i < nb && rank < need && base_out + rank < (unsigned int)sel_cap) sel[base_out + rank] = mine;
    }
}

#define RS_KEYS 16
#define RS_SL 16
__global__ __launch_bounds__(NT)
void rank_sort_kernel(const unsigned long long *__restrict__ sel, unsigned long long *__restrict__ sorted,
                      int sel_cap, const unsigned int *__restrict__ counters, int W, float *__restrict__ kpts,
                      float *__restrict__ scores)
{
    __shared__ unsigned long long tile[RS_SL][64];
    __shared__ unsigned int part[RS_SL][RS_KEYS];
    unsigned int n = counters[1];
    if (n > (unsigned int)sel_cap) n = sel_cap;
    if (blockIdx.x * (unsigned int)RS_KEYS >= n) return;
    const int li = threadIdx.x & (RS_KEYS - 1), q = threadIdx.x / RS_KEYS;
    const unsigned int i = blockIdx.x * RS_KEYS + li;
    const unsigned long long mine = i < n ? sel[i] : 0ull;
    const unsigned int qlen = (n + RS_SL - 1) / RS_SL, j0 = q * qlen;
    const unsigned int j1 = j0 + qlen < n ? j0 + qlen : n;
    unsigned int rank = 0;
    unsigned long long pre[4][64 / RS_KEYS];
#pragma unroll
    for (int pb = 0; pb < 4; ++pb)
#pragma unroll
        for (int tt = 0; tt < 64 / RS_KEYS; ++tt) {
            const unsigned int j = j0 + pb * 64 + li + tt * RS_KEYS;
            pre[pb][tt] = (pb * 64u < qlen && j < j1) ? sel[j] : 0ull;
        }
    for (unsigned int b = 0; b < qlen; b += 64) {
        if (b < 256) {
#pragma unroll
            for (int pb = 0; pb < 4; ++pb)
                if (b == pb * 64u)
#pragma unroll
                    for (int tt = 0; tt < 64 / RS_KEYS; ++tt) tile[q][li + tt * RS_KEYS] = pre[pb][tt];
        } else {
            for (int t = li; t < 64; t += RS_KEYS) tile[q][t] = (j0 + b + t < j1) ? sel[j0 + b + t] : 0ull;
        }
        __syncthreads();
#pragma unroll 8
        for (int t = 0; t < 64; ++t) rank += tile[q][t] > mine ? 1u : 0u;
        __syncthreads();
    }
    part[q][li] = rank;
    __syncthreads();
    if (q == 0 && i < n) {
        unsigned int r = 0;
#pragma unroll
        for (int k = 0; k < RS_SL; ++k) r += part[k][li];
        sorted[r] = mine;
        if (kpts) {
            const unsigned int idx = 0xFFFFFFFFu - (unsigned int)(mine & 0xFFFFFFFFull);
            kpts[2 * r] = (float)(idx % (unsigned int)W);
            kpts[2 * r + 1] = (float)(idx / (unsigned int)W);
            scores[r] = __uint_as_float((unsigned int)(mine >> 32));
        }
    }
}

void launch_topk_sort(hipStream_t st, bool threshold_done, const unsigned long long *cand, int cand_cap, int top_k,
                      unsigned long long *sel, unsigned long long *sorted, int sel_cap, unsigned int *counters,
                      unsigned long long *bnd, int W, float *kpts, float *scores)
{
    if (!threshold_done) hipLaunchKernelGGL(select_threshold_kernel, dim3(1), dim3(1024), 0, st, cand_cap, top_k, counters);
    int grid = (cand_cap + NT - 1) / NT;
    if (grid > 256) grid = 256;
    hipLaunchKernelGGL(compact_selected_kernel, dim3(grid), dim3(NT), 0, st, cand, cand_cap, sel, sel_cap, bnd, counters);
    hipLaunchKernelGGL(rank_sort_kernel, dim3((sel_cap + RS_KEYS - 1) / RS_KEYS), dim3(NT), 0, st, sel, sorted, sel_cap, counters, W,
                       kpts, scores);
}

__global__ __launch_bounds__(NT)
void keys_to_kpts_kernel(const unsigned long long *__restrict__ sorted, const unsigned int *__restrict__ counters,
                         int W, float *__restrict__ kpts, float *__restrict__ scores, int cap)
{
    unsigned int n = counters[1];
    if (n > (unsigned int)cap) n = cap;
    const unsigned int i = blockIdx.x * blockDim.x + threadIdx.x;
    if (i >= n) return;
    const unsigned long long key = sorted[i];
    const unsigned int idx = 0xFFFFFFFFu - (unsigned int)(key & 0xFFFFFFFFull);
    kpts[2 * i] = (float)(idx % (unsigned int)W);
    kpts[2 * i + 1] = (float)(idx / (unsigned int)W);
    scores[i] = __uint_as_float((unsigned int)(key >> 32));
}

void launch_keys_to_kpts(hipStream_t st, const unsigned long long *sorted, const unsigned int *counters, int W,
                         float *kpts, float *scores, int cap)
{
    if (cap <= 0) return;
    hipLaunchKernelGGL(keys_to_kpts_kernel, dim3((cap + NT - 1) / NT), dim3(NT), 0, st, sorted, counters, W, kpts, scores, cap);
}

#define GS_NONE 0
#define GS_UNDECIDED 1
#define GS_KEPT 2
#define GS_SUPPRESSED 3
__global__ __launch_bounds__(NT)
void greedy_init_kernel(const float *__restrict__ heat, int n, float conf_th, unsigned long long *__restrict__ keys,
                        unsigned char *__restrict__ state)
{
    const int i = blockIdx.x * blockDim.x + threadIdx.x;
    if (i >= n) return;
    const float v = heat[i];
    const bool c = v >= conf_th;
    keys[i] = c ? (((unsigned long long)__float_as_uint(v) << 32) | (unsigned long long)(0xFFFFFFFFu - (unsigned)i)) : 0ull;
    state[i] = c ? GS_UNDECIDED : GS_NONE;
}

__global__ __launch_bounds__(NT)
void greedy_iter_kernel(const unsigned long long *__restrict__ keys, const unsigned char *__restrict__ sin,
                        unsigned char *__restrict__ sout, int H, int W, int dist, unsigned int *__restrict__ undecided)
{
    const int x = blockIdx.x * 64 + (threadIdx.x & 63), y = blockIdx.y * 4 + (threadIdx.x >> 6);
    if (x >= W || y >= H) return;
    const int i = y * W + x;
    const unsigned char st = sin[i];
    if (st != GS_UNDECIDED) { sout[i] = st; return; }
    const unsigned long long mine = keys[i];
    bool any_kept = false, blocked = false;
    const int y0 = max(0, y - dist), y1 = min(H - 1, y + dist), x0 = max(0, x - dist), x1 = min(W - 1, x + dist);
    for (int yy = y0; yy <= y1; ++yy)
        for (int xx = x0; xx <= x1; ++xx) {
            const int j = yy * W + xx;
            const unsigned char sj = sin[j];
            if (sj == GS_KEPT) any_kept = true;
            else if (sj == GS_UNDECIDED && keys[j] > mine) blocked = true;
        }
    unsigned char ns = GS_UNDECIDED;
    if (any_kept) ns = GS_SUPPRESSED;
    else if (!blocked) ns = GS_KEPT;
    sout[i] = ns;
    if (ns == GS_UNDECIDED) atomicAdd(undecided, 1u);
}

__global__ __launch_bounds__(NT)
void greedy_final_kernel(const float *__restrict__ heat, const unsigned char *__restrict__ state, int n, float *__restrict__ kept)
{
    const int i = blockIdx.x * blockDim.x + threadIdx.x;
    if (i < n) kept[i] = state[i] == GS_KEPT ? heat[i] : 0.0f;
}

void launch_greedy_init(hipStream_t st, const float *heat, int n, float conf_th, unsigned long long *keys, unsigned char *state)
{
    hipLaunchKernelGGL(greedy_init_kernel, dim3((n + NT - 1) / NT), dim3(NT), 0, st, heat, n, conf_th, keys, state);
}
void launch_greedy_iter(hipStream_t st, const unsigned long long *keys, const unsigned char *sin, unsigned char *sout,
                        int H, int W, int dist, unsigned int *undecided)
{
    hipLaunchKernelGGL(greedy_iter_kernel, dim3((W + 63) / 64, (H + 3) / 4), dim3(NT), 0, st, keys, sin, sout, H, W, dist, undecided);
}
void launch_greedy_final(hipStream_t st, const float *heat, const unsigned char *state, int n, float *kept)
{
    hipLaunchKernelGGL(greedy_final_kernel, dim3((n + NT - 1) / NT), dim3(NT), 0, st, heat, state, n, kept);
}

struct SampleGeom {
    int x0, y0, x1, y1;
    bool vx0, vx1, vy0, vy1;
    float w_nw, w_ne, w_sw, w_se;
};
__device__ __forceinline__ SampleGeom sample_geom(float kx, float ky, float half_w, float half_h, int hc, int wc)
{
    SampleGeom g;
    const float gx = __fsub_rn(__fdiv_rn(kx, half_w), 1.0f);
    const float gy = __fsub_rn(__fdiv_rn(ky, half_h), 1.0f);
    const float ix = __fdiv_rn(__fsub_rn(__fmul_rn(__fadd_rn(gx, 1.0f), (float)wc), 1.0f), 2.0f);
    const float iy = __fdiv_rn(__fsub_rn(__fmul_rn(__fadd_rn(gy, 1.0f), (float)hc), 1.0f), 2.0f);
    const float fx = floorf(ix), fy = floorf(iy);
    g.x0 = (int)fx; g.y0 = (int)fy; g.x1 = g.x0 + 1; g.y1 = g.y0 + 1;
    const float ex = __fsub_rn(__fadd_rn(fx, 1.0f), ix), ey = __fsub_rn(__fadd_rn(fy, 1.0f), iy);
    const float dx = __fsub_rn(ix, fx), dy = __fsub_rn(iy, fy);
    g.w_nw = __fmul_rn(ex, ey); g.w_ne = __fmul_rn(dx, ey); g.w_sw = __fmul_rn(ex, dy); g.w_se = __fmul_rn(dx, dy);
    g.vx0 = g.x0 >= 0 && g.x0 < wc; g.vx1 = g.x1 >= 0 && g.x1 < wc;
    g.vy0 = g.y0 >= 0 && g.y0 < hc; g.vy1 = g.y1 >= 0 && g.y1 < hc;
    return g;
}

__global__ __launch_bounds__(NT)
void sample_desc_kernel(const float *__restrict__ dmap, int hc, int wc, float half_w, float half_h,
                        const float *__restrict__ kpts, const unsigned int *__restrict__ count, int n_max,
                        float *__restrict__ out, int compact )
{
    const int lane = threadIdx.x & 63;
    const int i = blockIdx.x * (NT / 64) + (threadIdx.x >> 6);
    int n = n_max;
    if (count) { const unsigned int c = *count; if ((unsigned int)n > c) n = (int)c; }
    if (i >= n) return;
    const SampleGeom g = sample_geom(kpts[2 * i], kpts[2 * i + 1], half_w, half_h, hc, wc);
    float a0 = 0.0f, a1 = 0.0f;
#define SFD2_TAP(valid_, yy_, xx_, wgt_, corner_)                                                    \
    if (valid_) {                                                                                    \
        const size_t row = compact ? (size_t)i * 4 + (corner_) : (size_t)(yy_) * wc + (xx_);         \
        const float2 v = *reinterpret_cast<const float2 *>(dmap + row * 128 + 2 * lane);             \
        const float nrm = fmaxf(sqrtf(wave_sum(v.x * v.x + v.y * v.y)), 1e-12f);                     \
        a0 += __fdiv_rn(v.x, nrm) * (wgt_);                                                          \
        a1 += __fdiv_rn(v.y, nrm) * (wgt_);                                                          \
    }
    SFD2_TAP(g.vy0 && g.vx0, g.y0, g.x0, g.w_nw, 0)
    SFD2_TAP(g.vy0 && g.vx1, g.y0, g.x1, g.w_ne, 1)
    SFD2_TAP(g.vy1 && g.vx0, g.y1, g.x0, g.w_sw, 2)
    SFD2_TAP(g.vy1 && g.vx1, g.y1, g.x1, g.w_se, 3)
#undef SFD2_TAP
    const float nrm = sqrtf(wave_sum(a0 * a0 + a1 * a1));
    *reinterpret_cast<float2 *>(out + (size_t)i * 128 + 2 * lane) = make_float2(__fdiv_rn(a0, nrm), __fdiv_rn(a1, nrm));
}

void launch_sample_desc(hipStream_t st, const float *dmap, int hc, int wc, int nh, int nw, const float *kpts,
                        const unsigned int *count, int n_max, float *out, int compact)
{
    if (n_max <= 0) return;
    hipLaunchKernelGGL(sample_desc_kernel, dim3((n_max + 3) / 4), dim3(NT), 0, st, dmap, hc, wc, (float)nw / 2.0f,
                       (float)nh / 2.0f, kpts, count, n_max, out, compact);
}

#define DH_KP 8
#define DH_XREC 528
#define DH_OREC 132
__global__ __launch_bounds__(NT)
void desc_head_kernel(const half_t *__restrict__ fmap , int hc, int wc, float half_w, float half_h,
                      const half_t *__restrict__ wpk , int CoutP, const float *__restrict__ scale,
                      const float *__restrict__ shift, const float *__restrict__ kpts, const unsigned int *__restrict__ count,
                      int n_max, float *__restrict__ out, int compact )
{
    __shared__ __attribute__((aligned(16))) unsigned char X[4 * DH_KP * DH_XREC];
    __shared__ __attribute__((aligned(16))) float O[4 * DH_KP * DH_OREC];
    const int tid = threadIdx.x, lane = tid & 63, wave = tid >> 6;
    int n = n_max;
    if (count) { const unsigned int c = *count; if ((unsigned int)n > c) n = (int)c; }
    const int k0 = blockIdx.x * DH_KP;
    if (k0 >= n) return;

    h8_t a[16];
    const int lrow = lane & 31, lhi = lane >> 5;
#pragma unroll
    for (int kk = 0; kk < 16; ++kk)
        a[kk] = *reinterpret_cast<const h8_t *>(wpk + ((size_t)(kk >> 1) * CoutP + wave * 32 + lrow) * 32 + (kk & 1) * 16 + lhi * 8);

    constexpr int DH_NR = 4 * DH_KP / 8;
    float kx[DH_NR], ky[DH_NR];
#pragma unroll
    for (int i = 0; i < DH_NR; ++i) {
        const int kp = k0 + ((wave * 2 + lhi + 8 * i) >> 2);
        const int kc = kp < n ? kp : n - 1;
        kx[i] = kpts[2 * kc];
        ky[i] = kpts[2 * kc + 1];
    }
    uint4 gv[DH_NR];
    bool gok[DH_NR];
#pragma unroll
    for (int i = 0; i < DH_NR; ++i) {
        const int rec = wave * 2 + lhi + 8 * i;
        const int kp = k0 + (rec >> 2), corner = rec & 3;
        const SampleGeom g = sample_geom(kx[i], ky[i], half_w, half_h, hc, wc);
        const int yy = (corner & 2) ? g.y1 : g.y0, xx = (corner & 1) ? g.x1 : g.x0;
        gok[i] = kp < n && ((corner & 2) ? g.vy1 : g.vy0) && ((corner & 1) ? g.vx1 : g.vx0);
        const size_t pix = gok[i] ? (compact ? (size_t)kp * 4 + corner : (size_t)yy * wc + xx) : 0;
        gv[i] = *reinterpret_cast<const uint4 *>(fmap + pix * 256 + lrow * 8);
    }
#pragma unroll
    for (int i = 0; i < DH_NR; ++i) {
        const int rec = wave * 2 + lhi + 8 * i;
        *reinterpret_cast<uint4 *>(X + rec * DH_XREC + lrow * 16) = gok[i] ? gv[i] : make_uint4(0, 0, 0, 0);
    }
    __syncthreads();

    constexpr int DH_NT = 4 * DH_KP / 32;
    f32x16_t acc[DH_NT];
#pragma unroll
    for (int t = 0; t < DH_NT; ++t)
#pragma unroll
        for (int r = 0; r < 16; ++r) acc[t][r] = 0.0f;
#pragma unroll
    for (int kk = 0; kk < 16; ++kk)
#pragma unroll
        for (int t = 0; t < DH_NT; ++t) {
            const h8_t b = *reinterpret_cast<const h8_t *>(X + (t * 32 + lrow) * DH_XREC + kk * 32 + lhi * 16);
            acc[t] = __builtin_amdgcn_mfma_f32_32x32x16_f16(a[kk], b, acc[t], 0, 0, 0);
        }
#pragma unroll
    for (int t = 0; t < DH_NT; ++t)
#pragma unroll
        for (int q = 0; q < 4; ++q) {
            const int c0 = wave * 32 + 8 * q + 4 * lhi;
            const float4 sc = *reinterpret_cast<const float4 *>(scale + c0);
            const float4 sh = *reinterpret_cast<const float4 *>(shift + c0);
            const float4 v = make_float4(acc[t][4 * q + 0] * sc.x + sh.x, acc[t][4 * q + 1] * sc.y + sh.y,
                                         acc[t][4 * q + 2] * sc.z + sh.z, acc[t][4 * q + 3] * sc.w + sh.w);
            *reinterpret_cast<float4 *>(O + (t * 32 + lrow) * DH_OREC + c0) = v;
        }
    __syncthreads();

    for (int j = wave; j < DH_KP; j += NT / 64) {
        const int kp = k0 + j;
        if (kp >= n) break;
        const SampleGeom g = sample_geom(kpts[2 * kp], kpts[2 * kp + 1], half_w, half_h, hc, wc);
        float a0 = 0.0f, a1 = 0.0f;
#define SFD2_TAP(valid_, wgt_, corner_)                                                              \
        if (valid_) {                                                                                \
            const float2 v = *reinterpret_cast<const float2 *>(O + (4 * j + (corner_)) * DH_OREC + 2 * lane); \
            const float nrm = fmaxf(sqrtf(wave_sum(v.x * v.x + v.y * v.y)), 1e-12f);                 \
            a0 += __fdiv_rn(v.x, nrm) * (wgt_);                                                      \
            a1 += __fdiv_rn(v.y, nrm) * (wgt_);                                                      \
        }
        SFD2_TAP(g.vy0 && g.vx0, g.w_nw, 0)
        SFD2_TAP(g.vy0 && g.vx1, g.w_ne, 1)
        SFD2_TAP(g.vy1 && g.vx0, g.w_sw, 2)
        SFD2_TAP(g.vy1 && g.vx1, g.w_se, 3)
#undef SFD2_TAP
        const float nrm = sqrtf(wave_sum(a0 * a0 + a1 * a1));
        *reinterpret_cast<float2 *>(out + (size_t)kp * 128 + 2 * lane) = make_float2(__fdiv_rn(a0, nrm), __fdiv_rn(a1, nrm));
    }
}

void launch_desc_head(hipStream_t st, const half_t *fmap, int hc, int wc, int nh, int nw, const half_t *wpk, int CoutP,
                      const float *scale, const float *shift, const float *kpts, const unsigned int *count, int n_max, float *out, int compact)
{
    if (n_max <= 0) return;
    hipLaunchKernelGGL(desc_head_kernel, dim3((n_max + DH_KP - 1) / DH_KP), dim3(NT), 0, st, fmap, hc, wc, (float)nw / 2.0f,
                       (float)nh / 2.0f, wpk, CoutP, scale, shift, kpts, count, n_max, out, compact);
}

__global__ __launch_bounds__(NT)
void desc_store64_kernel(const float *__restrict__ in, const unsigned int *__restrict__ count, int n_max, double *__restrict__ out, int pitch)
{
    __shared__ float tile[64][129];
    int n = n_max;
    if (count) { const unsigned int c = *count; if ((unsigned int)n > c) n = (int)c; }
    const int k0 = blockIdx.x * 64, tid = threadIdx.x;
    for (int i = tid; i < 64 * 128; i += NT) {
        const int r = i >> 7, ch = i & 127;
        tile[r][ch] = (k0 + r < n) ? in[(size_t)(k0 + r) * 128 + ch] : 0.0f;
    }
    __syncthreads();
    for (int i = tid; i < 64 * 128; i += NT) {
        const int ch = i >> 6, r = i & 63;
        if (k0 + r < pitch) out[(size_t)ch * pitch + k0 + r] = (double)tile[r][ch];
    }
}

void launch_desc_store64(hipStream_t st, const float *in, const unsigned int *count, int n_max, double *out, int pitch)
{
    if (pitch <= 0) return;
    hipLaunchKernelGGL(desc_store64_kernel, dim3((pitch + 63) / 64), dim3(NT), 0, st, in, count, n_max, out, pitch);
}

__global__ __launch_bounds__(NT)
void desc_normalise_nchw_kernel(const float *__restrict__ in, int npix, float *__restrict__ out)
{
    __shared__ float tile[64][129];
    const int lane = threadIdx.x & 63, wave = threadIdx.x >> 6;
    const int p0 = blockIdx.x * 64;
    for (int r = wave; r < 64; r += 4) {
        const int p = p0 + r;
        float2 v = make_float2(0.0f, 0.0f);
        if (p < npix) v = *reinterpret_cast<const float2 *>(in + (size_t)p * 128 + 2 * lane);
        const float nrm = fmaxf(sqrtf(wave_sum(v.x * v.x + v.y * v.y)), 1e-12f);
        tile[r][2 * lane] = __fdiv_rn(v.x, nrm);
        tile[r][2 * lane + 1] = __fdiv_rn(v.y, nrm);
    }
    __syncthreads();
    for (int c = wave; c < 128; c += 4) {
        const int p = p0 + lane;
        if (p < npix) out[(size_t)c * npix + p] = tile[lane][c];
    }
}

void launch_desc_normalise_nchw(hipStream_t st, const float *in, int npix, float *out)
{
    hipLaunchKernelGGL(desc_normalise_nchw_kernel, dim3((npix + 63) / 64), dim3(NT), 0, st, in, npix, out);
}

__device__ __forceinline__ float norm_tap(const float *__restrict__ img, int mode, int c, size_t plane, int W, int y, int x)
{
    float v;
    if (mode & 2) {
        const int cs = (mode & 4) ? 2 - c : c;
        v = __fdiv_rn((float)reinterpret_cast<const unsigned char *>(img)[((size_t)y * W + x) * 3 + cs], 255.0f);
    } else {
        v = img[c * plane + (size_t)y * W + x];
    }
    if (mode & 1) {
        const float m = c == 0 ? 0.485f : (c == 1 ? 0.456f : 0.406f);
        const float sd = c == 0 ? 0.229f : (c == 1 ? 0.224f : 0.225f);
        v = __fdiv_rn(__fsub_rn(v, m), sd);
    }
    return v;
}

__global__ __launch_bounds__(NT)
void norm_resize_kernel(const float *__restrict__ img, int mode, int H, int W, int nh, int nw, float sc_y, float sc_x,
                        float *__restrict__ out)
{
    const int x = blockIdx.x * 64 + (threadIdx.x & 63);
    const int y = blockIdx.y * 4 + (threadIdx.x >> 6);
    const int c = blockIdx.z;
    if (x >= nw || y >= nh) return;
    const LinCoef cy = lin_coef(y, H, nh, sc_y), cx = lin_coef(x, W, nw, sc_x);
    const size_t plane = (size_t)H * W;
    const float v00 = norm_tap(img, mode, c, plane, W, cy.i0, cx.i0), v01 = norm_tap(img, mode, c, plane, W, cy.i0, cx.i1);
    const float v10 = norm_tap(img, mode, c, plane, W, cy.i1, cx.i0), v11 = norm_tap(img, mode, c, plane, W, cy.i1, cx.i1);
    const float top = __fmaf_rn(v00, cx.l0, __fmul_rn(v01, cx.l1));
    const float bot = __fmaf_rn(v10, cx.l0, __fmul_rn(v11, cx.l1));
    out[(size_t)c * nh * nw + (size_t)y * nw + x] = __fmaf_rn(top, cy.l0, __fmul_rn(bot, cy.l1));
}

void launch_norm_resize(hipStream_t st, const float *img, int mode, int H, int W, int nh, int nw, float *out)
{
    hipLaunchKernelGGL(norm_resize_kernel, dim3((nw + 63) / 64, (nh + 3) / 4, 3), dim3(NT), 0, st, img, mode, H, W, nh, nw,
                       (float)H / (float)nh, (float)W / (float)nw, out);
}

__global__ __launch_bounds__(NT)
void ms_append_kernel(const float *__restrict__ kpts, const float *__restrict__ scores, const unsigned int *__restrict__ count,
                      int cap, float W, float nw, float H, float nh, float *__restrict__ kp_out, float *__restrict__ sc_out,
                      unsigned int *__restrict__ level_count)
{
    unsigned int n = *count;
    if (n > (unsigned int)cap) n = cap;
    const unsigned int i = blockIdx.x * blockDim.x + threadIdx.x;
    if (i == 0) *level_count = n;
    if (i >= n) return;
    kp_out[2 * i] = __fdiv_rn(__fmul_rn(kpts[2 * i], W), nw);
    kp_out[2 * i + 1] = __fdiv_rn(__fmul_rn(kpts[2 * i + 1], H), nh);
    sc_out[i] = scores[i];
}

void launch_ms_append(hipStream_t st, const float *kpts, const float *scores, const unsigned int *count, int cap, int W, int nw,
                      int H, int nh, float *kp_out, float *sc_out, unsigned int *level_count)
{
    hipLaunchKernelGGL(ms_append_kernel, dim3((cap + NT - 1) / NT > 0 ? (cap + NT - 1) / NT : 1), dim3(NT), 0, st, kpts, scores,
                       count, cap, (float)W, (float)nw, (float)H, (float)nh, kp_out, sc_out, level_count);
}

struct MsLevels { int n_levels; int offset[8]; };

__device__ __forceinline__ void ms_locate(const MsLevels &lv, const unsigned int *__restrict__ level_count, unsigned int pos,
                                          int *level, unsigned int *idx)
{
    unsigned int base = 0;
    int l = 0;
    for (; l < lv.n_levels - 1; ++l) {
        const unsigned int n = level_count[l];
        if (pos < base + n) break;
        base += n;
    }
    *level = l;
    *idx = pos - base;
}

__global__ __launch_bounds__(NT)
void ms_keys_kernel(MsLevels lv, const unsigned int *__restrict__ level_count, const float *__restrict__ sc_stage,
                    unsigned long long *__restrict__ keys, int cap_total, unsigned int *__restrict__ ms_counters)
{
    unsigned int total = 0;
    for (int l = 0; l < lv.n_levels; ++l) total += level_count[l];
    const unsigned int pos = blockIdx.x * blockDim.x + threadIdx.x;
    if (pos == 0) ms_counters[1] = total;
    if (pos >= total || pos >= (unsigned int)cap_total) return;
    int l; unsigned int i;
    ms_locate(lv, level_count, pos, &l, &i);
    const float s = sc_stage[lv.offset[l] + i];
    keys[pos] = ((unsigned long long)__float_as_uint(s) << 32) | (unsigned long long)(0xFFFFFFFFu - pos);
}

__global__ __launch_bounds__(NT)
void ms_gather_kernel(MsLevels lv, const unsigned int *__restrict__ level_count, const unsigned long long *__restrict__ sorted,
                      const float *__restrict__ kp_stage, const float *__restrict__ sc_stage, const float *__restrict__ de_stage,
                      int n_max, float *__restrict__ kp_out, float *__restrict__ sc_out, float *__restrict__ de_out,
                      unsigned int *__restrict__ ms_counters)
{
    unsigned int total = 0;
    for (int l = 0; l < lv.n_levels; ++l) total += level_count[l];
// ... 36 lines not shown
```

sfd2_amd/csrc/sfd2_ctx.h:

```cpp
#pragma once
#include "../../include/sfd2_hip.h"
#include "sfd2_internal.h"

#include <algorithm>
#include <atomic>
#include <cstdlib>
#include <cmath>
#include <cstdio>
#include <cstring>
#include <map>
#include <string>
#include <vector>

int sfd2_fail(const std::string &m);
#define fail sfd2_fail
struct PoseCam;
bool sfd2_pose_cam(int model, const double *params, PoseCam &c, std::string &why);
#define HIPCHECK(expr)                                                                           \
    do {                                                                                          \
        hipError_t e_ = (expr);                                                                   \
        if (e_ != hipSuccess)                                                                     \
            return fail(std::string(#expr) + ": " + hipGetErrorString(e_) + " @" + std::to_string(__LINE__)); \
    } while (0)

// ... 6 lines not shown
};
struct DevBuf : DevPtr {
    DevBuf() = default;
    DevBuf(const DevBuf &) = delete;
    DevBuf &operator=(const DevBuf &) = delete;
    DevBuf(DevBuf &&o) noexcept { p = o.p; cap = o.cap; o.p = nullptr; o.cap = 0; }
    DevBuf &operator=(DevBuf &&o) noexcept
    {
        if (this != &o) { release(); p = o.p; cap = o.cap; o.p = nullptr; o.cap = 0; }
        return *this;
    }
    ~DevBuf() { release(); }
    hipError_t ensure(size_t bytes)
    {
        if (bytes <= cap) return hipSuccess;
        ++g_alloc_gen;
        if (p) (void)hipFree(p);
        p = nullptr;
        cap = 0;
        hipError_t e = hipMalloc(&p, bytes);
        if (e == hipSuccess) cap = bytes;
        return e;
    }
    void release()
    {
        if (p) (void)hipFree(p);
        p = nullptr;
        cap = 0;
    }
};

struct ConvW {
    int cin = 0, cout = 0, cout_pad = 0, ks = 0, stride = 1;
    DevBuf w, scale, shift;
    DevBuf scale_rawin;
    DevBuf wsl;
    DevBuf wrm;
    DevBuf wfh, wfc, wfl;
    DevBuf wlk;
    DevBuf wgc;
    DevBuf wx3;
    DevBuf wx3p;
    DevBuf wc;
    int sbyte = 127;
    DevBuf wf8l;
    DevBuf wfr;
    DevBuf wc6;
    DevBuf sa6;
    size_t w_floats = 0;
    std::vector<float> h_scale, h_shift;
    std::vector<int> h_sa6;
    DevBuf wc66, sa66;
    std::vector<int> h_sa66;
};

enum { AE_CONV1A, AE_CONV1B, AE_CONV2A, AE_CONV2B, AE_CONV3A, AE_TRUNK ,
       AE_T1_0, AE_T1_1, AE_T1_2, AE_T2_0, AE_T2_1, AE_T2_2, AE_PA0, AE_DA0, AE_COUNT };

struct ActInfo { const void *p; int f32; int planar; int c, pitch, h, w; Rec rec = Rec::None;  int exp2 = 0;  bool absent = false;  };

struct JpegBuf {
    void *p = nullptr;
    size_t cap = 0;
    JpegBuf() = default;
    JpegBuf(const JpegBuf &) = delete;
    JpegBuf &operator=(const JpegBuf &) = delete;
    ~JpegBuf() { if (p) (void)hipFree(p); }
    template <typename T> T *as() const { return reinterpret_cast<T *>(p); }
};
struct JpegScratch {
    JpegBuf in[2];
    hipEvent_t ev_copied[2] = {}, ev_free[2] = {};
    int slot = 0;
    JpegBuf lanes, pre, coef, planes;
    JpegBuf words;
    ~JpegScratch()
    {
        for (int i = 0; i < 2; ++i) {
            if (ev_copied[i]) (void)hipEventDestroy(ev_copied[i]);
            if (ev_free[i]) (void)hipEventDestroy(ev_free[i]);
        }
    }
};

struct sfd2_ctx {
    int device = 0;
    hipStream_t stream = nullptr;
    hipEvent_t ev[4] = {nullptr, nullptr, nullptr, nullptr};
    hipEvent_t ev_jobs = nullptr;
    hipStream_t copy_stream = nullptr;
#define SFD2_IMG_SLOTS 4
    hipEvent_t ev_copied[SFD2_IMG_SLOTS] = {}, ev_img_free[SFD2_IMG_SLOTS] = {};
    DevBuf img2[SFD2_IMG_SLOTS];
    int img_slot = 0, img_slot_used = -1;
    void *pin_jobs = nullptr;
    size_t pin_cap = 0;
    bool weights_loaded = false;
    bool counters_clean = false;
    bool has_sta = false;
    int opt_alias = 1;
    int act_exp[AE_COUNT] = {};
    float act_max[AE_COUNT] = {};
    int opt_range_fallback = 1;
    int range_fallbacks = 0;
    int in_fallback = 0;
    int prof_step_entry = 0;
    float range_hist[SFD2_RS_COUNT] = {};
    int opt_auto_range = 1;
    std::vector<float> h_sta_w;
    int opt_cu_limit = 0;
    int fuse_det = 0;
    int use_graphs = 0;
    DevBuf x3_chain[2];
    DevBuf x3_rb_planes[3];
    int opt_fuse_post = 1;
    int opt_sparse_desc = 1;
    const half_t *da0_cur = nullptr;
    DevBuf da3_sparse;
    int opt_fp6_acts = 1;
    int net_error = 0;
    int opt_trunk_r1 = 1;
    int opt_s2d = 1;
    int opt_fp6_filters = 0;
    int opt_x3_pp = 1;
    int opt_auto_margin = 1;
    float margin_err[4] = {-1.0f, -1.0f, -1.0f, -1.0f};
    int margin_choice = -1;
    int opt_c3b_plain = 0;
    int user_c3b_plain = -1;
    bool margin_done = false, margin_pending = false;
    float relax_err = -1.0f;
    bool user_set_rb_inner = false, user_set_comp_heads = false;
    int user_rb_inner = 2, user_comp_heads = 0;
    int opt_x3_desc16 = 0;
    DevBuf x3_planes;
    DevBuf x3_da0_planes;
    DevBuf db_sparse;
    int opt_sparse_da3 = 1;
    int opt_fuse_pb = 1;
    const half_t *pa_cur = nullptr;
    const half_t *da_cur = nullptr;
    int opt_comp_rb = 1;
    int opt_rb_inner = 2;
    int opt_fuse_rb23 = 1;
    int opt_comp_det = 0;
    int opt_comp_heads = 0;
    int opt_no_rf_c = 0;
    int opt_generic_c = 0;
    int opt_branches = 0;
    int opt_sta_side = 0;
    hipStream_t side_stream = nullptr;
    hipStream_t cur_stream = nullptr;
    hipEvent_t ev_fork = nullptr, ev_join = nullptr;
    struct GraphEntry *graphs = nullptr;
    int n_graphs = 0;
    unsigned long long graph_clock = 0;
    ConvW c1a, c1b, c2a, c2b, c3a, c3b, rb1[3], rb2[3], rb3[3], pa0, pa3, da0, da3, pb, db;
    DevBuf sta_w16;
    DevPtr range_stat;
    DevPtr range_hist_dev;
    DevPtr extract_rec;
    DevBuf range_scratch;
    DevBuf sta_w, sta_b, zero_page, w1b_fused;
    DevBuf w1b_stem_c6;
    DevBuf w1b_stem_c;
    DevBuf w1b_stem_x3;
    int fuse = 1;
    int precision = SFD2_PREC_F16;
    ConvW f1a, f1b, f2a, f2b, f3a, f3b, frb1[3], frb2[3], frb3[3], fpa0, fpa3, fda0, fda3, fpb, fdb;
    DevBuf g1a, g1b, g2a, g2b, g3a, g3b, grt1[3], grt2[3], gro[3], gpa0_o, gpa_o, gda0_o, gda_o;
    int H = 0, W = 0, H2 = 0, W2 = 0, H4 = 0, W4 = 0, H8 = 0, W8 = 0;
    DevBuf img, a1a, a1b, a2a, a2b, a3a, a3b, rt1[3], rt2[3], ro[3], pa0_o, pa_o, da0_o, da_o;
    DevBuf logits , draw , sta , score , heat ;
    DevBuf stab , desc_nchw, tmp_f32;
    DevBuf cand, bnd, sel, sorted, counters, kpts, kscores, kdesc;
    DevBuf kdesc64;
    DevBuf g_keys, g_state0, g_state1, g_kept;
    int cand_cap = 0;
    int last_sel_cap = 0;
    float *kpts_cur = nullptr, *kscores_cur = nullptr;
    DevBuf arena;
    DevBuf img_u8_packed;
    JpegScratch jpeg;
    JpegBuf asm_in, asm_ws, asm_out;
    JpegBuf pose_in, pose_ws, pose_out;
    JpegBuf tri_in, tri_ws;
    DevBuf img_scaled, ms_kp, ms_sc, ms_de, ms_keys, ms_sorted, ms_cnt;
    unsigned int ms_cand_seen[8] = {};
    int ms_cand_cap[8] = {};
    DevBuf m_stage, m_hi0, m_lo0, m_hi1, m_lo1, m_part_f, m_part_i, m_red, m_jobs, m_fins, m_out_m, m_out_s, m_rkeys;
    sfd2_timings tim = {};
    std::map<std::string, ActInfo> acts;
    int prof_max_steps = 0, prof_step = 0, prof_slot = 0;
    std::vector<hipEvent_t> prof_ev;
    std::vector<sfd2_layer_timing> prof_tab;
    std::vector<int> prof_used;
    std::vector<int> prof_row;
    std::string prof_filter;
};

void graphs_release(sfd2_ctx *c);
#define PROF_SLOTS 48
struct ProfScope {
    sfd2_ctx *c; int slot;
    ProfScope(sfd2_ctx *c_, const char *name, const char *kernel, double flops, double bytes) : c(c_), slot(-1)
    {
        if (c->prof_max_steps <= 0 || c->prof_step >= c->prof_max_steps || c->prof_slot >= PROF_SLOTS) return;
        if (!c->prof_filter.empty() && strstr(kernel, c->prof_filter.c_str()) == nullptr) return;
        slot = c->prof_slot++;
        int row = -1;
        for (size_t i = 0; i < c->prof_tab.size(); ++i)
            if (strncmp(c->prof_tab[i].name, name, sizeof(c->prof_tab[i].name) - 1) == 0) { row = (int)i; break; }
        if (row < 0) {
            c->prof_tab.push_back(sfd2_layer_timing{});
            row = (int)c->prof_tab.size() - 1;
            snprintf(c->prof_tab[row].name, sizeof(c->prof_tab[row].name), "%s", name);
            snprintf(c->prof_tab[row].kernel, sizeof(c->prof_tab[row].kernel), "%s", kernel);
        }
        c->prof_tab[row].flops = flops;
        c->prof_tab[row].bytes = bytes;
        c->prof_row[(size_t)c->prof_step * PROF_SLOTS + slot] = row;
        (void)hipEventRecord(c->prof_ev[((size_t)c->prof_step * PROF_SLOTS + slot) * 2], c->cur_stream);
    }
    void cancel()
    {
        if (slot >= 0 && slot == c->prof_slot - 1) c->prof_slot--;
        slot = -1;
    }
    ~ProfScope()
    {
        if (slot >= 0) (void)hipEventRecord(c->prof_ev[((size_t)c->prof_step * PROF_SLOTS + slot) * 2 + 1], c->cur_stream);
    }
};
static inline void prof_step_begin(sfd2_ctx *c) { c->prof_slot = 0; }
static inline void prof_step_end(sfd2_ctx *c)
{
    if (c->prof_max_steps > 0 && c->prof_step < c->prof_max_steps) {
        c->prof_used[c->prof_step] = c->prof_slot;
        c->prof_step++;
    }
}

int apply_act_exponents(sfd2_ctx *c);
int read_range_status(sfd2_ctx *c, sfd2_range_status *out, int reset);
int range_wants_fallback(sfd2_ctx *c);
int range_fold_before_sync_extract(sfd2_ctx *c);
int sfd2_margin_selfcheck_if_pending(sfd2_ctx *c);
int reset_range_records(sfd2_ctx *c);
struct FallbackScope {
    sfd2_ctx *c; int prec;
    explicit FallbackScope(sfd2_ctx *c_) : c(c_), prec(c_->precision)
    {
        c->precision = SFD2_PREC_F16X3; c->in_fallback = 1; c->range_fallbacks++;
        if (c->prof_step > c->prof_step_entry) c->prof_step = c->prof_step_entry;
    }
    ~FallbackScope() { c->precision = prec; c->in_fallback = 0; }
};
enum PassEntry { PASS_DET , PASS_DENSE , PASS_EXTRACT  };
enum StrictLayer { SL_C1B, SL_C2A, SL_C2B, SL_C3A, SL_C3B, SL_RB1, SL_RB3 = SL_RB1 + 3, SL_PA0 = SL_RB3 + 3, SL_PA3, SL_PB, SL_DA0, SL_DA3, SL_DB, SL_COUNT };
template <class Ctx> auto &strict_layer(Ctx *c, int i)
{
    decltype(&c->f1b) t[] = {&c->f1b, &c->f2a, &c->f2b, &c->f3a, &c->f3b, &c->frb1[0], &c->frb1[1], &c->frb1[2], &c->frb3[0], &c->frb3[1], &c->frb3[2],
                             &c->fpa0, &c->fpa3, &c->fpb, &c->fda0, &c->fda3, &c->fdb};
    static_assert(sizeof(t) == SL_COUNT * sizeof(t[0]), "one entry per StrictLayer");
    return *t[i];
}
enum X3Kind { XK_GENERIC, XK_PP, XK_RF, XK_S2D, XK_SKIP };
enum X3Out { X3_F32, X3_CHAIN_A, X3_CHAIN_B, X3_RB, X3_DA0 };
struct StrictConv { X3Kind kind = XK_GENERIC; bool planes_in = false; X3Out out = X3_F32; bool s2d_out = false; };
struct X3Pair { half_t *hi = nullptr, *lo = nullptr; };
struct PassPlan {
    bool f32 = false, comp = false;
    bool fuse = false, alias = false;
    bool fused_stem = false, rb_fused = false;
    bool comp_rb = false;
    int rb_inner = 0;
    bool rb23 = false, generic_c = false, no_rf_c = false, fp6_filters = false;
    struct { Rec a1b, a2a, a2b, a3a, a3b, t1[3], t2[3], ro[3], pa0, da0; } rec = {};
    Rec a3a_in = Rec::None;
    bool a2a_s2d = false;
    bool ch = false, chp = false;
    bool branches = false, sta_early = false, sta_side = false;
    bool skip_head = false, skip_pb = false, skip_db = false, skip_da3 = false;
    bool sparse_desc = false, sparse_da3 = false, sparse_x3 = false;
    struct { int a1b, a2a, a2b, a3a, a3b, t1[3], t2[3], ro[3], pa0, pa, da0, da, n; size_t bytes; } slot = {};
    bool x3_pp = false, x3_fast = false;
    bool x3_stem = false, x3_rb = false;
    bool desc16 = false;
    StrictConv sl[SL_COUNT];
};
PassPlan plan_pass(const sfd2_ctx *c, PassEntry entry, int H, int W, int top_k = 0, bool desc = false);
int ensure_workspace(sfd2_ctx *c, const PassPlan &p, int H, int W);
int run_network(sfd2_ctx *c, const PassPlan &p, const float *img_dev, int normalise);
int convf(sfd2_ctx *c, const StrictConv &s, const char *name, const ConvW &L, const DevPtr &in, int H, int W, const DevPtr &out, int Ho, int Wo,
          int relu, const float *res = nullptr, X3Pair *planes = nullptr);
int ensure_strict_filters(sfd2_ctx *c, const PassPlan &p);
int copy_out(sfd2_ctx *c, void *dst, const void *src_dev, size_t bytes, int dst_on_device);
```

sfd2_amd/csrc/sfd2_internal.h:

```cpp
#pragma once
#include <hip/hip_runtime.h>
#include <hip/hip_fp16.h>
#include <stdint.h>

#ifdef SFD2_EXPERIMENTS
#include <stdlib.h>
static inline const char *sfd2_env(const char *name) { return getenv(name); }
#else
static inline const char *sfd2_env(const char *) { return nullptr; }
#endif

extern thread_local int g_sfd2_cu_limit;
static inline int sfd2_slots(int cus) { return (g_sfd2_cu_limit > 0 && g_sfd2_cu_limit < cus) ? g_sfd2_cu_limit : cus; }

#define SFD2_BARRIER_DRAIN() asm volatile("s_waitcnt vmcnt(0) lgkmcnt(0)\n\ts_barrier" ::: "memory")

typedef _Float16 half_t;
typedef _Float16 h8_t __attribute__((ext_vector_type(8)));
typedef _Float16 h4_t __attribute__((ext_vector_type(4)));
typedef float f32x16_t __attribute__((ext_vector_type(16)));

#ifdef __HIPCC__
__device__ __forceinline__ float4 sfd2_lds_f4(const float *p)
{
// ... 186 lines not shown
    f32x16v_t v, l;
    float m = 0.0f;
#pragma unroll
    for (int q = 0; q < 4; ++q) {
        f32x2_t v01 = f32x2_t{acc[4 * q], acc[4 * q + 1]} * f32x2_t{sc[q].x, sc[q].y} + f32x2_t{sh[q].x, sh[q].y};
        f32x2_t v23 = f32x2_t{acc[4 * q + 2], acc[4 * q + 3]} * f32x2_t{sc[q].z, sc[q].w} + f32x2_t{sh[q].z, sh[q].w};
        m = sfd2_max3(sfd2_max3(m, v01[0], v01[1]), v23[0], v23[1]);
        v01[0] = __builtin_amdgcn_fmed3f(v01[0], lo, SFD2_C_SAT); v01[1] = __builtin_amdgcn_fmed3f(v01[1], lo, SFD2_C_SAT);
        v23[0] = __builtin_amdgcn_fmed3f(v23[0], lo, SFD2_C_SAT); v23[1] = __builtin_amdgcn_fmed3f(v23[1], lo, SFD2_C_SAT);
        const h2_t h01 = __builtin_convertvector(v01, h2_t), h23 = __builtin_convertvector(v23, h2_t);
        __builtin_memcpy(&hv[q].x, &h01, 4);
        __builtin_memcpy(&hv[q].y, &h23, 4);
        const f32x2_t l01 = (v01 - f32x2_t{(float)h01[0], (float)h01[1]}) * 2048.0f, l23 = (v23 - f32x2_t{(float)h23[0], (float)h23[1]}) * 2048.0f;
        v[4 * q] = v01[0]; v[4 * q + 1] = v01[1]; v[4 * q + 2] = v23[0]; v[4 * q + 3] = v23[1];
        l[4 * q] = l01[0]; l[4 * q + 1] = l01[1]; l[4 * q + 2] = l23[0]; l[4 * q + 3] = l23[1];
    }
#ifndef SFD2_NO_RANGE
    if (TRACK) mx = counted ? __builtin_fmaxf(mx, m) : mx;
#endif
    const unsigned int mb = __float_as_uint(__builtin_fminf(__builtin_fmaxf(m, 0.0f), SFD2_C_SAT));
    v6i_t d;
#if SFD2_PIX6_BF6
    int e8 = (int)(mb >> 23) - 4 + ((mb & 0x7fffffu) > 0x600000u ? 1 : 0);
    e8 = e8 < 1 ? 1 : e8;
    const float scale = __uint_as_float((unsigned int)e8 << 23);
    asm volatile("v_cvt_scalef32_2xpk16_bf6_f32 %0, %1, %2, %3" : "=&v"(d) : "v"(l), "v"(v), "v"(scale));
#else
    int e8 = (int)(mb >> 23) - 2 + ((mb & 0x7fffffu) > 0x700000u ? 1 : 0);
    e8 = e8 < 1 ? 1 : e8;
    const float scale = __uint_as_float((unsigned int)e8 << 23);
    asm volatile("v_cvt_scalef32_2xpk16_fp6_f32 %0, %1, %2, %3" : "=&v"(d) : "v"(l), "v"(v), "v"(scale));
#endif
    rec0 = make_uint4((unsigned)d[0], (unsigned)d[1], (unsigned)d[2], (unsigned)d[3]);
    rec1 = make_uint4((unsigned)d[4], (unsigned)d[5], (unsigned)e8 * 0x01010101u, 0u);
}
__device__ __forceinline__ float sfd2_corr_lo(unsigned d, int ch )
{
    return (ch ? __builtin_amdgcn_cvt_f32_fp8((int)d, 2) : __builtin_amdgcn_cvt_f32_fp8((int)d, 0)) * (1.0f / (float)(1 << SFD2_C_XL_SHIFT));
}
#endif


void launch_conv1a(hipStream_t st, const float *img_chw, int H, int W, int normalise,
                   const half_t *wpk , const float *scale, const float *shift,
                   half_t *out );

void launch_fused_stem(hipStream_t st, const float *img, int H, int W, int normalise, const half_t *w1, const float *sc1,
                       const float *sh1, const half_t *w2, const float *sc2, const float *sh2, half_t *out, int H2, int W2);

bool conv3x3_pp_serves(int ks, int stride, int CoutP, int Cin);
bool launch_conv3x3_rf_x3(hipStream_t st, const half_t *in_hi, const half_t *in_lo, int H, int W, int Cin, const half_t *wpl,
                          const float *scale, const float *shift, int CoutP, int stride, int relu, half_t *out_hi, half_t *out_lo,
                          float *out_f32, int Ho, int Wo, const half_t *zero_page);
bool conv3x3_rf_serves(int ks, int stride, int CoutP, int Cin, int Ho, int Wo);
void launch_conv_igemm(hipStream_t st, const half_t *in, int H, int W, int Cin,
                       const half_t *wpk, const float *scale, const float *shift, int Cout_pad,
                       int ks, int stride, int relu, const half_t *residual,
                       void *out, int out_f32, int Ho, int Wo, const half_t *zero_page );

int conv_igemm_chunk(int ks, int stride, int Cout_pad, int Cin);

void launch_gconv3x3_g8(hipStream_t st, const half_t *in, int H, int W, const half_t *wpk,
                        const float *scale, const float *shift, half_t *out);

void launch_convsta(hipStream_t st, const half_t *in, int npix, const float *w , const float *b,
                    float *out );

enum class Rec {
    None,
    Unit8,
    Half6,
    Resid8,
};
void launch_convc_igemm(hipStream_t st, const half_t *in, const half_t *in_c, int H, int W, int Cin, const half_t *wpk,
                        const float *scale, const float *shift, int Cout_pad, int ks, int stride, int relu,
                        const half_t *res, const half_t *res_c, half_t *out, half_t *out_c, int Ho, int Wo, int sbyte, unsigned int *range = nullptr);
bool launch_conv3x3_pp_c(hipStream_t st, const half_t *in, const half_t *in_c, int H, int W, int Cin, const half_t *wpk,
                         const float *scale, const float *shift, int CoutP, int relu, half_t *out, half_t *out_c,
                         int Ho, int Wo, const half_t *zero_page, int sbyte,
                         unsigned int *range ,
                         Rec rin, Rec rout, bool s2d_out, bool fp6_w);
bool conv3x3_rf_c_serves(int ks, int stride, int CoutP, int Cin, int Ho, int Wo);
bool conv2b_s2d_serves(int H2, int W2, int Cin, int CoutP);
void launch_conv2b_s2d(hipStream_t st, const half_t *in_s2d, const half_t *in_c_s2d, int H4, int W4, const half_t *wpk, const float *scale,
                       const float *shift, int relu, half_t *out, half_t *out_c, const half_t *zero_page, int sbyte, unsigned int *range, Rec rout );
void launch_conv2b_s2d_x3(hipStream_t st, const half_t *in_hi_s2d, const half_t *in_lo_s2d, int H4, int W4, const half_t *wpk ,
                          const float *scale, const float *shift, int relu, half_t *out_hi, half_t *out_lo, const half_t *zero_page);
bool launch_conv3x3_rf_c(hipStream_t st, const half_t *in, const half_t *in_c, int H, int W, int Cin, const half_t *wpk,
                         const float *scale, const float *shift, int CoutP, int stride, int relu, half_t *out, half_t *out_c,
                         int Ho, int Wo, const half_t *zero_page, int sbyte, unsigned int *range, Rec rin , Rec rout );
bool launch_conv_igemm2_c(hipStream_t st, const half_t *in, const half_t *in_c, int H, int W, int Cin, const half_t *wpk,
                          const float *scale, const float *shift, int CoutP, int ks, int stride, int relu,
                          const half_t *res, const half_t *res_c, half_t *out, half_t *out_c, int Ho, int Wo,
                          const half_t *zero_page, int sbyte, unsigned int *range = nullptr);
void launch_fused_stem_c(hipStream_t st, const float *img, int H, int W, int normalise, const half_t *w1, const float *sc1,
                         const float *sh1, const void *w2, const float *sc2, const float *sh2, half_t *out, half_t *out_c,
                         int H2, int W2, int sbyte, unsigned int *range_base = nullptr ,
                         Rec rout = Rec::Unit8 );
void launch_conv1x1_c256_c(hipStream_t st, const half_t *in, const half_t *in_c, int npix, const half_t *w_frag,
                           const half_t *wc_frag, const float *scale, const float *shift, int relu, const half_t *res,
                           const half_t *res_c, half_t *out, half_t *out_c, const half_t *zero_page, int sbyte, unsigned int *range,
                           Rec rin , Rec rout );
void launch_sparse_da3(hipStream_t st, const half_t *fmap, int hc, int wc, int nh, int nw, const half_t *wpk, const half_t *wsl, int CoutP,
                       const float *scale, const float *shift, int relu, const float *kpts, const unsigned int *count, int n_max,
                       half_t *out, const half_t *zero_page);
void launch_sparse_da3_repack(hipStream_t st, const half_t *w, half_t *dst, int CoutP, int cin);
void launch_sparse_da3_x3(hipStream_t st, const half_t *fmap_hi, const half_t *fmap_lo, int hc, int wc, int nh, int nw, const half_t *wpk, const half_t *wsl,
                          int CoutP, const float *scale, const float *shift, int relu, const float *kpts, const unsigned int *count,
                          int n_max, float *out, const half_t *zero_page);
void launch_rb23_c(hipStream_t st, const half_t *t1, int H, int W, const half_t *w2h, const half_t *w2l, const float *sc2,
                   const float *sh2, const half_t *w3h, const half_t *w3l, const float *sc3, const float *sh3,
                   const half_t *res, const half_t *res_c, half_t *out, half_t *out_c, const half_t *zero_page,
                   unsigned int *range_t2, unsigned int *range_out, Rec rres, Rec rout ,
                   const half_t *w3l8, int sbyte3 );
void launch_conv1x1_c256_x3(hipStream_t st, const half_t *in, const half_t *in_lo, int npix, const half_t *w, const half_t *wl,
                            const float *scale, const float *shift, int relu, const void *res, const half_t *res_lo, float *out, half_t *out_hi,
                            half_t *out_lo, const half_t *zero_page);
void launch_conv1a_c(hipStream_t st, const float *img, int H, int W, int normalise, const half_t *wpk ,
                     const float *scale, const float *shift, half_t *out, half_t *out_c, unsigned int *range = nullptr);
void launch_gconv_c(hipStream_t st, const half_t *in, const half_t *in_c, int H, int W, const half_t *wpk ,
                    const void *wck , const float *scale, const float *shift, half_t *out, half_t *out_c, int sbyte,
                    int row0, int row1 , unsigned int *range = nullptr);
void launch_nhwc_hc_to_nchw_f(hipStream_t st, const half_t *in, const half_t *in_c, int npix, int pitch, int c, float *out, Rec rec );

void launch_conv_igemm_f32(hipStream_t st, const float *in, int H, int W, int Cin, const float *wpk,
                           const float *scale, const float *shift, int Cout_pad, int ks, int stride, int relu,
                           const float *residual, float *out, int Ho, int Wo);
void launch_x3_split(hipStream_t st, const float *w, size_t n_floats, void *out);
void launch_x3_split_planes(hipStream_t st, const float *in, size_t n_floats, void *hi_out, void *lo_out);
void launch_conv3x3_pp_x3(hipStream_t st, const half_t *in, const half_t *in_lo, int H, int W, int Cin, const half_t *wpk,
                          const float *scale, const float *shift, int CoutP, int relu, half_t *out_hi, half_t *out_lo, float *out_f32,
                          int Ho, int Wo, const half_t *zero_page, int s2d = 0 );
void launch_gconv_x3_pack(hipStream_t st, const float *w , void *out );
void launch_gconv_x3(hipStream_t st, const float *in, int H, int W, const void *wpk, const float *scale, const float *shift, float *out);
void launch_conv_igemm_x3(hipStream_t st, const float *in, int H, int W, int Cin, const float *wpk,
                           const float *scale, const float *shift, int Cout_pad, int ks, int stride, int relu,
                           const float *residual, float *out, int Ho, int Wo);
void launch_conv1a_f32(hipStream_t st, const float *img_chw, int H, int W, int normalise, const float *w ,
                       const float *scale, const float *shift, float *out );
void launch_gconv_f32(hipStream_t st, const float *in, int H, int W, const float *w , const float *scale,
                      const float *shift, float *out);
void launch_convsta_f32(hipStream_t st, const float *in, int npix, const float *w, const float *b, float *out);

void launch_detector_head(hipStream_t st, const float *logits, int pitch, int hc, int wc, float *score);
void launch_heatmap(hipStream_t st, const float *score, int hs, int ws, const float *sta, int hc, int wc,
                    int H, int W, float *heat, float *stab_out );
bool launch_nms_select(hipStream_t st, const float *heat, int H, int W, int radius, float conf_th, int border, int Hb, int Wb,
                       float *nms_dense , unsigned long long *cand_keys, int cand_cap,
                       unsigned int *counters , int fuse_threshold = 0, int top_k = 0);
void launch_heads_heat(hipStream_t st, const float *logits, int pitch, int hc8, int wc8, const float *sta, int hc, int wc,
                       int H, int W, float *heat);
void launch_topk_sort(hipStream_t st, bool threshold_done, const unsigned long long *cand, int cand_cap, int top_k,
                      unsigned long long *sel, unsigned long long *sorted, int sel_cap, unsigned int *counters,
                      unsigned long long *bnd, int W, float *kpts, float *scores);
#define SFD2_HIST_BINS 4096
#define SFD2_COUNTER_BYTES (64 + SFD2_HIST_BINS * 4)
__device__ __forceinline__ unsigned int key_bin(unsigned long long key)
{
    const int b = (int)((unsigned int)(key >> 47) & 0xFFFFu) - ((127 - 12) << 8);
    return (unsigned int)(b < 0 ? 0 : (b > SFD2_HIST_BINS - 1 ? SFD2_HIST_BINS - 1 : b));
}

__device__ __forceinline__ unsigned int sfd2_ld_agent(const unsigned int *p)
{
    return __hip_atomic_load(p, __ATOMIC_RELAXED, __HIP_MEMORY_SCOPE_AGENT);
}

template <bool COHERENT>
__device__ __forceinline__ void sfd2_select_threshold(int cand_cap, int top_k, unsigned int *__restrict__ counters, unsigned int *wsum)
{
    static_assert(SFD2_HIST_BINS == 4096, "one uint4 of bins per thread");
    const unsigned int *hist = counters + 16;
    unsigned int n = COHERENT ? sfd2_ld_agent(counters) : counters[0];
    if (n > (unsigned int)cand_cap) n = cand_cap;
    const unsigned int k = (top_k <= 0 || (unsigned int)top_k > n) ? n : (unsigned int)top_k;
    if (k == n) {
        if (threadIdx.x == 0) { counters[1] = n; counters[2] = 0; counters[3] = 0; counters[4] = 0; counters[5] = 0; counters[6] = 1; }
        return;
    }
    const int t = threadIdx.x, lane = t & 63, wave = t >> 6;
    uint4 hv;
    if (COHERENT) hv = make_uint4(sfd2_ld_agent(hist + 4 * t), sfd2_ld_agent(hist + 4 * t + 1), sfd2_ld_agent(hist + 4 * t + 2), sfd2_ld_agent(hist + 4 * t + 3));
    else hv = reinterpret_cast<const uint4 *>(hist)[t];
    const unsigned int sum = hv.x + hv.y + hv.z + hv.w;
    unsigned int suf = sum;
#pragma unroll
    for (int d = 1; d < 64; d <<= 1) {
        const unsigned int o = __shfl_down(suf, d);
        if (lane + d < 64) suf += o;
    }
    if (lane == 0) wsum[wave] = suf;
    __syncthreads();
    unsigned int higher = 0;
    for (int w = wave + 1; w < 16; ++w) higher += wsum[w];
    const unsigned int above_incl = higher + suf;
    unsigned int above = above_incl - sum;
    if (above < k && above_incl >= k) {
        const unsigned int b[4] = {hv.x, hv.y, hv.z, hv.w};
#pragma unroll
        for (int j = 3; j >= 0; --j) {
            if (above < k && above + b[j] >= k) {
                counters[1] = k; counters[2] = 0; counters[3] = 0;
                counters[4] = 4 * t + j;
                counters[5] = k - above;
                counters[6] = 0;
            }
            above += b[j];
        }
    }
}

void launch_nms4_select(hipStream_t st, const float *heat, int H, int W, float conf_th, int border, int Hb, int Wb, float *nms_dense,
                        unsigned long long *cand, int cand_cap, unsigned int *counters, unsigned int *hist, int fuse_threshold, int top_k);
void launch_greedy_init(hipStream_t st, const float *heat, int n, float conf_th, unsigned long long *keys, unsigned char *state);
void launch_greedy_iter(hipStream_t st, const unsigned long long *keys, const unsigned char *sin, unsigned char *sout,
                        int H, int W, int dist, unsigned int *undecided);
void launch_greedy_final(hipStream_t st, const float *heat, const unsigned char *state, int n, float *kept);
void launch_keys_to_kpts(hipStream_t st, const unsigned long long *sorted_keys, const unsigned int *counters,
                         int W, float *kpts_xy, float *scores, int cap);
void launch_sample_desc(hipStream_t st, const float *desc_nhwc, int hc, int wc, int nh, int nw,
                        const float *kpts_xy, const unsigned int *count , int n_max,
                        float *out, int compact = 0);
void launch_pb_heads_heat(hipStream_t st, const half_t *fmap, int hc8, int wc8, const half_t *wpk, int CoutP, const float *scale,
                          const float *shift, const float *sta, int hc, int wc, int H, int W, float *heat,
                          unsigned int *zero_words , int n_zero);
bool pb_heads_heat_clears(int hc8, int wc8, int n_zero);
void launch_desc_store64(hipStream_t st, const float *in , const unsigned int *count, int n_max, double *out , int pitch);
void launch_desc_head(hipStream_t st, const half_t *fmap, int hc, int wc, int nh, int nw, const half_t *wpk, int CoutP,
                      const float *scale, const float *shift, const float *kpts, const unsigned int *count, int n_max, float *out, int compact = 0);
void launch_desc_normalise_nchw(hipStream_t st, const float *desc_nhwc, int npix, float *out_nchw);
void launch_nhwc_h_to_nchw_f(hipStream_t st, const half_t *in, int npix, int c_pitch, int c, float *out);
void launch_nhwc_f_to_nchw_f(hipStream_t st, const float *in, int npix, int c_pitch, int c, float *out);
void launch_nchw_f_to_nhwc_f(hipStream_t st, const float *in, int npix, int c, float *out);

void launch_scale_inplace(hipStream_t st, float *p, size_t n, float mul);
void launch_absmax_f32(hipStream_t st, const float *in, size_t n, unsigned int *out);

void launch_ingest_u8(hipStream_t st, const unsigned char *src, int H, int W, int bgr, int nh, int nw, float *out);
void launch_unpack_rgbx(hipStream_t st, const unsigned char *src, unsigned char *dst, size_t npix);
void launch_extract_record(hipStream_t st, unsigned int *range_stat, unsigned int *hist, const unsigned int *counters, int sel_cap,
                           int cand_cap, unsigned int *rec );

void launch_match_prep(hipStream_t st, const void *src, int n, int n_src, const int *rows, int dim, int dtype, int layout,
                       half_t *hi, half_t *lo);
struct MatchJob {
    const half_t *a_hi;
    const half_t *a_lo;
    const half_t *b_hi;
    const half_t *b_lo;
    int na, nb;
    float *part_v1;
    float *part_v2;
    int *part_i1;
};
void launch_match_top2(hipStream_t st, const MatchJob *jobs_dev, int njobs, int max_nb, int splits, int use_lo,
                       int need_top2, const half_t *zero_page);
struct MatchJob2 {
    const half_t *q_hi;
    const half_t *d_hi;
    int n0, n1;
    float *part_v1;
    int *part_i1;
    float *rkeys;
};
struct MatchFinal;
void launch_match_mutual(hipStream_t st, const MatchJob2 *jobs_dev, const MatchFinal *fins_dev, int npairs, int max_n0,
                         int max_n1, int splits, int fwd_ids);
int match_mutual_max_chunk(void);
int match_mutual_strip(void);
void launch_match_decide(hipStream_t st, const MatchFinal *fin_dev, int npairs, int max_n, int flavour, int mutual,
                         float ratio, float dist);
struct MatchFinal {
    const float *f_v1, *f_v2; const int *f_i1;
    const float *r_v1, *r_v2; const int *r_i1;
    int n0, n1;
    int out16, pad_;
    long long *matches0; float *scores0;
    float *red_f;
    float *red_r;
    const int *remap;
};
void launch_match_finalize(hipStream_t st, const MatchFinal *fin_dev, int npairs, int max_n, int splits,
                           int flavour, int mutual, float ratio, float dist);

void launch_conv1x1_c256(hipStream_t st, const half_t *in, int npix, const half_t *w_rowmajor, const float *scale,
                         const float *shift, int relu, const half_t *res, half_t *out, const half_t *zero_page);

void launch_resblock(hipStream_t st, const half_t *x, int H, int W, const half_t *w1, const float *sc1, const float *sh1,
                     const half_t *wg, const float *sc2, const float *sh2, const half_t *w3, const float *sc3, const float *sh3,
                     half_t *out, const half_t *zero_page);

void launch_norm_resize(hipStream_t st, const float *img, int mode, int H, int W, int nh, int nw, float *out);
void launch_ms_append(hipStream_t st, const float *kpts, const float *scores, const unsigned int *count, int cap, int W, int nw,
                      int H, int nh, float *kp_out, float *sc_out, unsigned int *level_count);
void launch_ms_merge(hipStream_t st, int n_levels, const int *offsets, const unsigned int *level_count, const float *kp_stage,
                     const float *sc_stage, const float *de_stage, int cap_total, int top_k, unsigned long long *keys,
                     unsigned long long *sorted, unsigned int *ms_counters, int n_max, float *kp_out, float *sc_out, float *de_out);

#define SFD2_JPEG_LANE_BITS 256
#define SFD2_JPEG_SYNC_LAUNCHES 12
#define SFD2_JPEG_BAD_CODE 1u
#define SFD2_JPEG_BAD_COUNT 2u
#define SFD2_JPEG_BAD_END 4u
#define SFD2_JPEG_NO_SYNC 8u
struct JpegHuff {
    uint16_t lut[512];
    int32_t maxcode[18];
    int32_t valoff[18];
    uint8_t vals[256];
};
struct JpegTables {
    JpegHuff huff[3][2];
    uint16_t q[3][64];
};
static inline int64_t jpeg_tail_bytes(int64_t lanes, int64_t intervals)
{
    return (int64_t)sizeof(JpegTables) + 4 * (lanes + 1) + 4 * lanes + 4 * (intervals + 1);
}
struct JpegGeom {
    int ncomp, bpm, mcus_x, total_blocks, ri_blocks , nlanes, nint;
    uint32_t ecs_words;
    int unit_comp[10], unit_dx[10], unit_dy[10];
    int hs[3], vs[3];
    int bw[3], bh[3];
    int blk_base[3];
    int64_t plane_off[3];
    int W, H, mode;
    int cw, ch;
};
struct JpegLane {
    uint32_t spos, epos;
    int32_t su, eu, bad, cnt;
    int32_t dc[3];
    int32_t pad;
};
void launch_jpeg_decode(hipStream_t st, const unsigned char *in, int64_t tab_off, const JpegGeom &g, JpegLane *lanes, int *lane_pre,
                        int *wg_pre, unsigned int *sync_flags, short *coef, unsigned char *planes, unsigned char *out_rgbx,
                        unsigned int *status);

#define SFD2_POSE_WG 256
struct PoseCam {
    double f[2], c[2];
    double k1, k2, p1, p2;
    int32_t distorted, pad;
};
struct PoseProbDev {
    int64_t off;
    int32_t n, pad;
    PoseCam cam;
    double thresh2;
    double qt[7];
};
struct PoseConfDev {
    int64_t max_trials, min_trials;
    double confidence;
    uint64_t seed;
    int32_t refine_only, pad;
};
struct PoseResDev {
    double q[4], t[3];
    int32_t success, num_inliers, num_trials, pad;
};
void launch_pose(hipStream_t st, const PoseProbDev *probs, int k, const PoseConfDev &conf, const double *p2, const double *p3, float4 *xf4,
                 float2 *xf2, double2 *xn, double *hyp, const unsigned char *mask_in, unsigned char *mask_out, PoseResDev *res);

#define SFD2_ASM_WG 256
#define SFD2_ASM_ST_MATCH_RANGE 1
#define SFD2_ASM_ST_ROW_RANGE 2
#define SFD2_ASM_ST_CAPACITY 4
struct AsmImgDev {
    const int32_t *tab;
    int32_t n1;
    int32_t mrow;
};
struct AsmJobDev {
    const long long *matches0;
    const AsmImgDev *imgs;
    const float *kpq, *scores;
    int32_t k, n, nchunk, gate;
    int64_t ws_off, blk_off, cnt_off;
    int32_t cap, pad;
    double obs_th, radius;
    double R[9], t[3];
    PoseCam cam;
    double *p2, *p3;
    int32_t *prow, *qidx, *iidx;
    float *score;
};
struct AsmResDev { int32_t m, status; };
void launch_assemble(hipStream_t st, const AsmJobDev *jobs, int n_jobs, int max_blocks, const double *xyz, const int32_t *track, int n_points,
                     int32_t *rows, unsigned char *keep, int32_t *blk, int32_t *counts, AsmResDev *res);

#define SFD2_TRI_WG 256
#define SFD2_TRI_WAVE 64
#define SFD2_TRI_MAX_POINTS 4
#define SFD2_TRI_ST_RANGE 1
#define SFD2_TRI_ST_NOT_CONVERGED 2
#define SFD2_TRI_ST_SHORT 1
#define SFD2_TRI_ST_NONFINITE 2
struct TriViewDev {
    double R[9], t[3], C[3];
    PoseCam cam;
};
struct TriPairDev {
    double E[9];
    double thr_i, thr_j;
    int64_t moff, kp_i, kp_j;
    int32_t n, n_i, n_j, blk0;
};
struct TriConfDev {
    double tan_create, cos_min_angle, max_reproj;
    uint64_t seed;
    int32_t lm_iters, pad;
};
void launch_tri_normalise(hipStream_t st, const TriViewDev *views, int n_views, const int64_t *offsets, const float *kp, int64_t n, double2 *xn);
void launch_tri_verify(hipStream_t st, const TriPairDev *pairs, int n_pairs, const int32_t *blk_pair, int n_blocks, const double2 *xn,
                       int32_t *matches, int32_t *blk_cnt, int32_t *pair_cnt, int32_t *pair_status, int min_inliers);
void launch_tri_cc_init(hipStream_t st, int32_t *parent, int64_t n, int32_t *words);
void launch_tri_cc_round(hipStream_t st, const int32_t *edges, int64_t n_edges, int32_t *parent, int64_t n, int32_t *words);
void launch_tri_cc_flags(hipStream_t st, const int32_t *sorted_labels, int64_t n, int32_t *keep, int32_t *head);
// ... 8 lines not shown
```

Measured before the change: 718.8.

## Fuse match reduce/claim/decide, emit f16 query descriptors, defer job upload, block-cursor compaction

Adds four default-on options. The mutual-match reduce, claim and decide kernels are merged into one per-pair kernel that works in LDS. The descriptor head now writes an f16 copy of the query descriptors, so the match stage skips its separate prep/convert pass. The host-to-device copy of the match job descriptors is moved out of the captured graph and issued once before graph launch. Top-k compaction uses block-level atomic cursors instead of per-wave ones. Together these cut kernel launches, memory passes and atomic traffic, at the cost of an LDS-capacity limit on the fused path and more complex state passed between the extract and match stages.

```diff
diff --git a/sfd2_amd/csrc/api_core.hip b/sfd2_amd/csrc/api_core.hip
--- a/sfd2_amd/csrc/api_core.hip
+++ b/sfd2_amd/csrc/api_core.hip
@@ -130,6 +130,10 @@
     else if (k == "c3b_plain") { c->user_c3b_plain = value < 0 ? -1 : (value ? 1 : 0); c->opt_c3b_plain = value > 0 ? 1 : 0; }
     else if (k == "comp_det") c->opt_comp_det = value ? 1 : 0;
     else if (k == "fuse_rb23") c->opt_fuse_rb23 = value ? 1 : 0;
+    else if (k == "finalize_fused") c->opt_finalize_fused = value ? 1 : 0;
+    else if (k == "desc_f16_direct") c->opt_desc_f16_direct = value ? 1 : 0;
+    else if (k == "jobs_static") c->opt_jobs_static = value ? 1 : 0;
+    else if (k == "topk_block_cursor") c->opt_topk_block_cursor = value ? 1 : 0;
     else if (k == "rb_inner") { c->opt_rb_inner = c->user_rb_inner = value < 0 ? 0 : (value > 2 ? 2 : value); c->user_set_rb_inner = true; }
     else return fail("sfd2_set_option: unknown key '" + k + "'");
     return 0;
@@ -146,7 +150,8 @@
         {"auto_margin", c->opt_auto_margin}, {"fp6_filters", c->opt_fp6_filters}, {"fp6_acts", c->opt_fp6_acts}, {"s2d", c->opt_s2d},
         {"trunk_r1", c->opt_trunk_r1}, {"fuse_pb", c->opt_fuse_pb}, {"generic_c", c->opt_generic_c}, {"comp_rb", c->opt_comp_rb},
         {"no_rf_c", c->opt_no_rf_c}, {"comp_heads", c->opt_comp_heads}, {"c3b_plain", c->opt_c3b_plain}, {"comp_det", c->opt_comp_det},
-        {"fuse_rb23", c->opt_fuse_rb23}, {"rb_inner", c->opt_rb_inner},
+        {"fuse_rb23", c->opt_fuse_rb23}, {"rb_inner", c->opt_rb_inner}, {"finalize_fused", c->opt_finalize_fused},
+        {"desc_f16_direct", c->opt_desc_f16_direct}, {"jobs_static", c->opt_jobs_static}, {"topk_block_cursor", c->opt_topk_block_cursor},
     };
     for (const auto &e : tab)
         if (k == e.name) { *value = e.v; return 0; }
diff --git a/sfd2_amd/csrc/api_extract.hip b/sfd2_amd/csrc/api_extract.hip
--- a/sfd2_amd/csrc/api_extract.hip
+++ b/sfd2_amd/csrc/api_extract.hip
@@ -114,7 +114,7 @@
         c->kscores_cur = scores_dev ? scores_dev : c->kscores.as<float>();
         launch_topk_sort(c->stream, threshold_done, c->cand.as<unsigned long long>(), c->cand_cap, top_k,
                          c->sel.as<unsigned long long>(), c->sorted.as<unsigned long long>(), sel_cap,
-                         c->counters.as<unsigned int>(), c->bnd.as<unsigned long long>(), W, c->kpts_cur, c->kscores_cur);
+                         c->counters.as<unsigned int>(), c->bnd.as<unsigned long long>(), W, c->kpts_cur, c->kscores_cur, c->opt_topk_block_cursor);
     }
     HIPCHECK(hipGetLastError());
     return 0;
@@ -195,6 +195,7 @@
             HIPCHECK(c->kdesc.ensure((size_t)sel_cap * 128 * sizeof(float)));
             desc_dst = c->kdesc.as<float>();
         }
+        half_t *q16 = (c->q16_want && desc_dst == desc && sel_cap == top_k) ? c->m_hi0.as<half_t>() : nullptr;
         if (plan.sparse_x3 && !plan.desc16) {
             const size_t nin = (size_t)c->H4 * c->W4 * 256;
             const int rows32 = (sel_cap * 4 + 31) / 32;
@@ -221,11 +222,13 @@
             }
             ProfScope ps(c, "desc_head", "desc_head_kernel", 2.0 * 4 * sel_cap * 128 * 256, (double)sel_cap * (4 * 512 + 512));
             launch_desc_head(c->stream, c->da3_sparse.as<half_t>(), c->H4, c->W4, H, W, c->db.w.as<half_t>(), c->db.cout_pad, c->db.scale.as<float>(),
-                             c->db.shift.as<float>(), c->kpts_cur, c->counters.as<unsigned int>() + 1, sel_cap, desc_dst, 1);
+                             c->db.shift.as<float>(), c->kpts_cur, c->counters.as<unsigned int>() + 1, sel_cap, desc_dst, 1, q16);
+            if (q16) { c->q16_src = desc; c->q16_rows = sel_cap; }
         } else if (plan.sparse_desc) {
             ProfScope ps(c, "desc_head", "desc_head_kernel", 2.0 * 4 * sel_cap * 128 * 256, (double)sel_cap * (4 * 512 + 512));
             launch_desc_head(c->stream, c->da_cur, c->H4, c->W4, H, W, c->db.w.as<half_t>(), c->db.cout_pad, c->db.scale.as<float>(),
-                             c->db.shift.as<float>(), c->kpts_cur, c->counters.as<unsigned int>() + 1, sel_cap, desc_dst);
+                             c->db.shift.as<float>(), c->kpts_cur, c->counters.as<unsigned int>() + 1, sel_cap, desc_dst, 0, q16);
+            if (q16) { c->q16_src = desc; c->q16_rows = sel_cap; }
         } else {
             ProfScope ps(c, "sample_desc", "sample_desc_kernel", 0.0, (double)sel_cap * 128 * 4 * 5);
             launch_sample_desc(c->stream, c->draw.as<float>(), c->H4, c->W4, H, W, c->kpts_cur,
diff --git a/sfd2_amd/csrc/api_graph.hip b/sfd2_amd/csrc/api_graph.hip
--- a/sfd2_amd/csrc/api_graph.hip
+++ b/sfd2_amd/csrc/api_graph.hip
@@ -44,10 +44,20 @@
                                int64_t *m, float *ms)
 {
     int n_dummy = 0;
-    if (sfd2_extract(c, img, 1, H, W, conf_th, top_k, flags | SFD2_FLAG_ASYNC, kp, sc, de, 1, top_k, &n_dummy)) return -1;
+    c->q16_src = nullptr;
+    c->q16_want = false;
+    if (k > 0 && c->opt_desc_f16_direct && dim == 128 && conf->sim_mode != SFD2_SIM_F16X2) {
+        HIPCHECK(c->m_hi0.ensure((size_t)top_k * 128 * 2));
+        c->q16_want = true;
+    }
+    const int rc = sfd2_extract(c, img, 1, H, W, conf_th, top_k, flags | SFD2_FLAG_ASYNC, kp, sc, de, 1, top_k, &n_dummy);
+    c->q16_want = false;
+    if (rc) { c->q16_src = nullptr; return -1; }
     if (k > 0) {
         const sfd2_desc_set q = {de, top_k, SFD2_DT_F32, SFD2_LAYOUT_ND, 1, nullptr, 0, 0};
-        if (sfd2_match_batch(c, &q, db, k, dim, conf, m, ms, 1, SFD2_FLAG_ASYNC)) return -1;
+        const int rm = sfd2_match_batch(c, &q, db, k, dim, conf, m, ms, 1, SFD2_FLAG_ASYNC);
+        c->q16_src = nullptr;
+        if (rm) return -1;
     }
     return 0;
 }
@@ -115,6 +125,8 @@
     const unsigned long long gen0 = g_alloc_gen.load();
     std::swap(c->pin_jobs, e->pin); std::swap(c->pin_cap, e->pin_cap);
     std::swap(c->m_jobs, e->jobs); std::swap(c->m_fins, e->fins);
+    c->jobs_defer = c->opt_jobs_static != 0;
+    c->jobs_deferred = 0;
     hipError_t be = hipStreamBeginCapture(c->stream, hipStreamCaptureModeThreadLocal);
     int rc = -1;
     hipGraph_t g = nullptr;
@@ -127,6 +139,9 @@
     }
     std::swap(c->pin_jobs, e->pin); std::swap(c->pin_cap, e->pin_cap);
     std::swap(c->m_jobs, e->jobs); std::swap(c->m_fins, e->fins);
+    const size_t jobs_deferred = c->jobs_deferred;
+    c->jobs_defer = false;
+    c->jobs_deferred = 0;
     if (rc != 0 || g_alloc_gen != gen0) {
         if (g) (void)hipGraphDestroy(g);
         e->seen = 0;
@@ -136,6 +151,7 @@
     e->graph = g;
     HIPCHECK(hipGraphInstantiate(&e->exec, g, nullptr, nullptr, 0));
     e->gen = g_alloc_gen;
+    if (jobs_deferred) HIPCHECK(hipMemcpyAsync(e->jobs.p, e->pin, jobs_deferred, hipMemcpyHostToDevice, c->stream));
     HIPCHECK(hipGraphLaunch(e->exec, c->stream));
     return 0;
 }
diff --git a/sfd2_amd/csrc/api_match.hip b/sfd2_amd/csrc/api_match.hip
--- a/sfd2_amd/csrc/api_match.hip
+++ b/sfd2_amd/csrc/api_match.hip
@@ -142,8 +142,12 @@
     prof_step_begin(c);
     size_t stage_off = 0;
     const half_t *q_hi = nullptr, *q_lo = nullptr;
-    if (prep_set(c, q->data, n0, nullptr, n0, dim, q->dtype, q->layout, q->on_device, need_lo, c->m_stage, stage_off,
-                 c->m_hi0.as<half_t>(), c->m_lo0.as<half_t>(), &q_hi, &q_lo)) return -1;
+    const bool q16 = c->q16_src != nullptr && c->q16_src == q->data && c->q16_rows == n0 && q->on_device && q->dtype == SFD2_DT_F32 &&
+                     q->layout == SFD2_LAYOUT_ND && dim == 128 && !need_lo;
+    c->q16_src = nullptr;
+    if (q16) q_hi = c->m_hi0.as<half_t>();
+    else if (prep_set(c, q->data, n0, nullptr, n0, dim, q->dtype, q->layout, q->on_device, need_lo, c->m_stage, stage_off,
+                      c->m_hi0.as<half_t>(), c->m_lo0.as<half_t>(), &q_hi, &q_lo)) return -1;
     static_assert(sizeof(MatchJob2) <= 2 * sizeof(MatchJob), "descriptor buffer sizing");
     const size_t jobs_bytes = 2 * (size_t)k * sizeof(MatchJob), fins_bytes = (size_t)k * sizeof(MatchFinal);
     hipStreamCaptureStatus cap_status = hipStreamCaptureStatusNone;
@@ -203,15 +207,27 @@
         fn.red_f = red + 3 * roff; roff += (size_t)n0;
         fn.red_r = red + 3 * roff; roff += (size_t)n1;
     }
-    HIPCHECK(hipMemcpyAsync(c->m_jobs.p, jobs, jobs_bytes + fins_bytes, hipMemcpyHostToDevice, c->stream));
+    if (capturing && c->jobs_defer) c->jobs_deferred = jobs_bytes + fins_bytes;
+    else HIPCHECK(hipMemcpyAsync(c->m_jobs.p, jobs, jobs_bytes + fins_bytes, hipMemcpyHostToDevice, c->stream));
     MatchFinal *fins_dev = reinterpret_cast<MatchFinal *>(static_cast<char *>(c->m_jobs.p) + jobs_bytes);
     if (!capturing) HIPCHECK(hipEventRecord(c->ev_jobs, c->stream));
-    if (single_gemm) {
+    const bool fwd_ids = conf->flavour == SFD2_MATCH_HLOC && !conf->do_mutual_check;
+    if (single_gemm && c->opt_finalize_fused && !fwd_ids && n0 <= match_finalize_fused_cap() && max_n1 <= match_finalize_fused_cap()) {
         {
             ProfScope ps(c, "match_mutual", "match_mutual_kernel", 2.0 * (double)n0 * (double)tot_n1 * 128.0,
                          2.0 * ((double)k * n0 + (double)tot_n1) * 128.0);
-            launch_match_mutual(c->stream, c->m_jobs.as<MatchJob2>(), fins_dev, k, n0, max_n1, splits,
-                                conf->flavour == SFD2_MATCH_HLOC && !conf->do_mutual_check);
+            launch_match_mutual(c->stream, c->m_jobs.as<MatchJob2>(), fins_dev, k, n0, max_n1, splits, 0, 0);
+        }
+        {
+            ProfScope ps(c, "match_finalize", "match_mutual_finalize", 0.0, (double)tot_part * 12);
+            launch_match_mutual_finalize(c->stream, c->m_jobs.as<MatchJob2>(), fins_dev, k, n0, max_n1, splits, conf->flavour, conf->do_mutual_check,
+                                         conf->ratio_threshold, conf->distance_threshold);
+        }
+    } else if (single_gemm) {
+        {
+            ProfScope ps(c, "match_mutual", "match_mutual_kernel", 2.0 * (double)n0 * (double)tot_n1 * 128.0,
+                         2.0 * ((double)k * n0 + (double)tot_n1) * 128.0);
+            launch_match_mutual(c->stream, c->m_jobs.as<MatchJob2>(), fins_dev, k, n0, max_n1, splits, fwd_ids);
         }
         {
             ProfScope ps(c, "match_finalize", "match_decide", 0.0, (double)tot_part * 12);
diff --git a/sfd2_amd/csrc/match_kernels.hip b/sfd2_amd/csrc/match_kernels.hip
--- a/sfd2_amd/csrc/match_kernels.hip
+++ b/sfd2_amd/csrc/match_kernels.hip
@@ -361,16 +361,119 @@
         atomicMin(reinterpret_cast<unsigned int *>(f.red_f) + 2 * (size_t)f.n0 + i, (unsigned int)j);
 }
 
+#define MF_NT 1024
+#define MF_CAP 8192
+int match_finalize_fused_cap(void) { return MF_CAP; }
+__device__ __forceinline__ void decide_one(const MatchFinal &f, int i, float s1, float s2, int j, float t1, float t2, int back, int flavour, int mutual,
+                                           float ratio, float dist);
+__global__ __launch_bounds__(MF_NT)
+void match_mutual_finalize_kernel(const MatchJob2 *__restrict__ jobs, const MatchFinal *__restrict__ fins, int splits, int strip, int flavour,
+                                  int mutual, float ratio, float dist)
+{
+    extern __shared__ __attribute__((aligned(16))) unsigned char smem[];
+    const MatchJob2 job = jobs[blockIdx.x];
+    const MatchFinal f = fins[blockIdx.x];
+    const int n0 = job.n0, n1 = job.n1;
+    float *F = reinterpret_cast<float *>(smem);
+    unsigned int *J = reinterpret_cast<unsigned int *>(smem) + n0;
+    float *RV = reinterpret_cast<float *>(smem) + 2 * (size_t)n0;
+    int *RI = reinterpret_cast<int *>(smem) + 2 * (size_t)n0 + n1;
+    for (int i0 = threadIdx.x; i0 < n0; i0 += 4 * MF_NT) {
+        float b1[4] = {-INFINITY, -INFINITY, -INFINITY, -INFINITY};
+        for (int s = 0; s < splits; s += 4) {
+            float c1[4][4];
+#pragma unroll
+            for (int ss = 0; ss < 4; ++ss)
+#pragma unroll
+                for (int u = 0; u < 4; ++u) {
+                    const int i = i0 + u * MF_NT;
+                    c1[ss][u] = (s + ss < splits && i < n0) ? job.part_v1[(size_t)(s + ss) * n0 + i] : -INFINITY;
+                }
+#pragma unroll
+            for (int ss = 0; ss < 4; ++ss)
+#pragma unroll
+                for (int u = 0; u < 4; ++u)
+                    if (c1[ss][u] > b1[u]) b1[u] = c1[ss][u];
+        }
+#pragma unroll
+        for (int u = 0; u < 4; ++u) {
+            const int i = i0 + u * MF_NT;
+            if (i < n0) { F[i] = b1[u]; J[i] = 0xFFFFFFFFu; }
+        }
+    }
+    const int nstrip = (n0 + strip - 1) / strip;
+    for (int j0 = threadIdx.x; j0 < n1; j0 += 4 * MF_NT) {
+        float best[4] = {MQ_NEG, MQ_NEG, MQ_NEG, MQ_NEG};
+        unsigned int bkey[4];
+        int bs[4] = {0, 0, 0, 0};
+#pragma unroll
+        for (int u = 0; u < 4; ++u) bkey[u] = __float_as_uint(MQ_NEG);
+        for (int sidx = 0; sidx < nstrip; sidx += 8) {
+            float k[8][4];
+#pragma unroll
+            for (int t = 0; t < 8; ++t)
+#pragma unroll
+                for (int u = 0; u < 4; ++u) {
+                    const int j = j0 + u * MF_NT;
+                    k[t][u] = (sidx + t < nstrip && j < n1) ? job.rkeys[(size_t)(sidx + t) * n1 + j] : MQ_NEG;
+                }
+#pragma unroll
+            for (int t = 0; t < 8; ++t)
+#pragma unroll
+                for (int u = 0; u < 4; ++u) {
+                    const float v = __uint_as_float(__float_as_uint(k[t][u]) & 0xFFFFFF00u);
+                    if (v > best[u]) { best[u] = v; bkey[u] = __float_as_uint(k[t][u]); bs[u] = sidx + t; }
+                }
+        }
+#pragma unroll
+        for (int u = 0; u < 4; ++u) {
+            const int j = j0 + u * MF_NT;
+            if (j >= n1) continue;
+            const bool any = best[u] > MQ_NEG;
+            RV[j] = any ? __uint_as_float(bkey[u] & 0xFFFFFF00u) : -INFINITY;
+            RI[j] = any ? bs[u] * strip + 255 - (int)(bkey[u] & 255u) : 0;
+        }
+    }
+    __syncthreads();
+    for (int j = threadIdx.x; j < n1; j += MF_NT) {
+        const float r = RV[j];
+        const int i = RI[j];
+        if (r > -INFINITY && (unsigned int)i < (unsigned int)n0 && (__float_as_uint(F[i]) & 0xFFFFFF00u) == __float_as_uint(r))
+            atomicMin(&J[i], (unsigned int)j);
+    }
+    __syncthreads();
+    for (int i = threadIdx.x; i < n0; i += MF_NT) {
+        const int j = (int)J[i];
+        const bool has = n1 > 0 && j >= 0;
+        decide_one(f, i, F[i], -INFINITY, j, has ? RV[j] : 0.0f, -INFINITY, has ? RI[j] : 0, flavour, mutual, ratio, dist);
+    }
+}
+
 void launch_match_mutual(hipStream_t st, const MatchJob2 *jobs_dev, const MatchFinal *fins_dev, int npairs, int max_n0,
-                         int max_n1, int splits, int fwd_ids)
+                         int max_n1, int splits, int fwd_ids, int merge)
 {
     if (npairs <= 0 || max_n0 <= 0) return;
     launch_match_mutual_gemm(st, jobs_dev, npairs, max_n0, splits, fwd_ids);
+    if (!merge) return;
     const int max_n = max_n0 > max_n1 ? max_n0 : max_n1;
     hipLaunchKernelGGL(match_mutual_reduce_kernel, dim3((max_n + NT - 1) / NT, npairs, 2), dim3(NT), 0, st, jobs_dev, fins_dev, splits,
                        match_mutual_strip(), fwd_ids);
     if (!fwd_ids && max_n1 > 0)
         hipLaunchKernelGGL(match_mutual_claim_kernel, dim3((max_n1 + NT - 1) / NT, npairs), dim3(NT), 0, st, fins_dev);
+}
+
+void launch_match_mutual_finalize(hipStream_t st, const MatchJob2 *jobs_dev, const MatchFinal *fins_dev, int npairs, int max_n0, int max_n1, int splits,
+                                  int flavour, int mutual, float ratio, float dist)
+{
+    if (npairs <= 0 || max_n0 <= 0) return;
+    static bool attr_done = false;
+    if (!attr_done) {
+        (void)hipFuncSetAttribute(reinterpret_cast<const void *>(match_mutual_finalize_kernel), hipFuncAttributeMaxDynamicSharedMemorySize, 16 * MF_CAP);
+        attr_done = true;
+    }
+    const size_t lds = 8 * ((size_t)max_n0 + (size_t)(max_n1 > 0 ? max_n1 : 0));
+    hipLaunchKernelGGL(match_mutual_finalize_kernel, dim3(npairs), dim3(MF_NT), lds, st, jobs_dev, fins_dev, splits, match_mutual_strip(), flavour, mutual,
+                       ratio, dist);
 }
 
 void launch_match_top2(hipStream_t st, const MatchJob *jobs_dev, int njobs, int max_nb, int splits, int use_lo,
@@ -447,21 +550,14 @@
     return d0 / (d1 + 1e-8f);
 }
 
-__global__ __launch_bounds__(NT)
-void match_decide_kernel(const MatchFinal *__restrict__ fins, int flavour, int mutual, float ratio, float dist)
-{
-    const MatchFinal f = fins[blockIdx.y];
-    const int i = blockIdx.x * blockDim.x + threadIdx.x;
-    if (i >= f.n0) return;
-    const float s1 = f.red_f[i], s2 = f.red_f[(size_t)f.n0 + i];
-    const int j = reinterpret_cast<const int *>(f.red_f)[2 * (size_t)f.n0 + i];
+__device__ __forceinline__ void decide_one(const MatchFinal &f, int i, float s1, float s2, int j, float t1, float t2, int back, int flavour, int mutual,
+                                           float ratio, float dist)
+{
     long long m = -1;
     float score = 0.0f;
     if (f.n1 > 0 && j < 0) {
         score = flavour == 0 ? (hloc_pass(s1, s2, ratio, dist) ? (s1 + 1.0f) / 2.0f : 0.0f) : s1;
     } else if (f.n1 > 0) {
-        const float t1 = f.red_r[j], t2 = f.red_r[(size_t)f.n1 + j];
-        const int back = reinterpret_cast<const int *>(f.red_r)[2 * (size_t)f.n1 + j];
         if (flavour == 0) {
             const bool ok = hloc_pass(s1, s2, ratio, dist);
             score = ok ? (s1 + 1.0f) / 2.0f : 0.0f;
@@ -489,6 +585,23 @@
     }
 }
 
+__global__ __launch_bounds__(NT)
+void match_decide_kernel(const MatchFinal *__restrict__ fins, int flavour, int mutual, float ratio, float dist)
+{
+    const MatchFinal f = fins[blockIdx.y];
+    const int i = blockIdx.x * blockDim.x + threadIdx.x;
+    if (i >= f.n0) return;
+    const float s1 = f.red_f[i], s2 = f.red_f[(size_t)f.n0 + i];
+    const int j = reinterpret_cast<const int *>(f.red_f)[2 * (size_t)f.n0 + i];
+    float t1 = 0.0f, t2 = 0.0f;
+    int back = 0;
+    if (f.n1 > 0 && j >= 0) {
+        t1 = f.red_r[j]; t2 = f.red_r[(size_t)f.n1 + j];
+        back = reinterpret_cast<const int *>(f.red_r)[2 * (size_t)f.n1 + j];
+    }
+    decide_one(f, i, s1, s2, j, t1, t2, back, flavour, mutual, ratio, dist);
+}
+
 void launch_match_decide(hipStream_t st, const MatchFinal *fin_dev, int npairs, int max_n, int flavour, int mutual,
                          float ratio, float dist)
 {
diff --git a/sfd2_amd/csrc/post_kernels.hip b/sfd2_amd/csrc/post_kernels.hip
--- a/sfd2_amd/csrc/post_kernels.hip
+++ b/sfd2_amd/csrc/post_kernels.hip
@@ -369,6 +369,34 @@
     sfd2_select_threshold<false>(cand_cap, top_k, counters, wsum);
 }
 
+template <int BT>
+__device__ __forceinline__ void compact_boundary_tail(unsigned long long *__restrict__ sel, int sel_cap, const unsigned long long *__restrict__ bnd,
+                                                      unsigned int *__restrict__ counters)
+{
+    __shared__ unsigned int s_last;
+    SFD2_BARRIER_DRAIN();
+    if (threadIdx.x == 0) s_last = atomicAdd(&counters[8], 1u) == gridDim.x - 1 ? 1u : 0u;
+    __syncthreads();
+    if (!s_last) return;
+    const unsigned int nb = sfd2_ld_agent(counters + 3), need = counters[5], k = counters[1];
+    if (counters[6] || need == 0) return;
+    __shared__ unsigned long long tile[BT];
+    const unsigned int base_out = k - need;
+    for (unsigned int i0 = 0; i0 < nb; i0 += blockDim.x) {
+        const unsigned int i = i0 + threadIdx.x;
+        const unsigned long long mine = i < nb ? __hip_atomic_load(bnd + i, __ATOMIC_RELAXED, __HIP_MEMORY_SCOPE_AGENT) : 0ull;
+        unsigned int rank = 0;
+        for (unsigned int b = 0; b < nb; b += BT) {
+            tile[threadIdx.x] = (b + threadIdx.x < nb) ? __hip_atomic_load(bnd + b + threadIdx.x, __ATOMIC_RELAXED, __HIP_MEMORY_SCOPE_AGENT) : 0ull;
+            __syncthreads();
+            const unsigned int lim = nb - b < BT ? nb - b : BT;
+            for (unsigned int t = 0; t < lim; ++t) rank += tile[t] > mine ? 1u : 0u;
+            __syncthreads();
+        }
+        if (i < nb && rank < need && base_out + rank < (unsigned int)sel_cap) sel[base_out + rank] = mine;
+    }
+}
+
 __global__ __launch_bounds__(NT)
 void compact_selected_kernel(const unsigned long long *__restrict__ cand, int cand_cap,
                              unsigned long long *__restrict__ sel, int sel_cap,
@@ -401,28 +429,52 @@
             __hip_atomic_store(bnd + base_b + (unsigned int)__popcll(mb & below), key, __ATOMIC_RELAXED, __HIP_MEMORY_SCOPE_AGENT);
         }
     }
-    __shared__ unsigned int s_last;
-    SFD2_BARRIER_DRAIN();
-    if (threadIdx.x == 0) s_last = atomicAdd(&counters[8], 1u) == gridDim.x - 1 ? 1u : 0u;
-    __syncthreads();
-    if (!s_last) return;
-    const unsigned int nb = sfd2_ld_agent(counters + 3), need = counters[5], k = counters[1];
-    if (counters[6] || need == 0) return;
-    __shared__ unsigned long long tile[NT];
-    const unsigned int base_out = k - need;
-    for (unsigned int i0 = 0; i0 < nb; i0 += blockDim.x) {
+    compact_boundary_tail<NT>(sel, sel_cap, bnd, counters);
+}
+
+#define CB_NT 1024
+__global__ __launch_bounds__(CB_NT)
+void compact_selected_block_kernel(const unsigned long long *__restrict__ cand, int cand_cap,
+                                   unsigned long long *__restrict__ sel, int sel_cap,
+                                   unsigned long long *__restrict__ bnd, unsigned int *__restrict__ counters)
+{
+    unsigned int n = counters[0];
+    if (n > (unsigned int)cand_cap) n = cand_cap;
+    const unsigned int bstar = counters[4], all = counters[6];
+    const int lane = threadIdx.x & 63, wave = threadIdx.x >> 6;
+    const unsigned long long below = (1ull << lane) - 1ull;
+    const unsigned int stride = gridDim.x * blockDim.x;
+    __shared__ unsigned int w_s[CB_NT / 64], w_b[CB_NT / 64], base[2];
+    for (unsigned int i0 = blockIdx.x * blockDim.x; i0 < n; i0 += stride) {
         const unsigned int i = i0 + threadIdx.x;
-        const unsigned long long mine = i < nb ? __hip_atomic_load(bnd + i, __ATOMIC_RELAXED, __HIP_MEMORY_SCOPE_AGENT) : 0ull;
-        unsigned int rank = 0;
-        for (unsigned int b = 0; b < nb; b += NT) {
-            tile[threadIdx.x] = (b + threadIdx.x < nb) ? __hip_atomic_load(bnd + b + threadIdx.x, __ATOMIC_RELAXED, __HIP_MEMORY_SCOPE_AGENT) : 0ull;
-            __syncthreads();
-            const unsigned int lim = nb - b < NT ? nb - b : NT;
-            for (unsigned int t = 0; t < lim; ++t) rank += tile[t] > mine ? 1u : 0u;
-            __syncthreads();
-        }
-        if (i < nb && rank < need && base_out + rank < (unsigned int)sel_cap) sel[base_out + rank] = mine;
-    }
+        const bool live = i < n;
+        const unsigned long long key = live ? cand[i] : 0ull;
+        const unsigned int bin = key_bin(key);
+        const bool to_sel = live && (all || bin > bstar), to_bnd = live && !to_sel && bin == bstar;
+        const unsigned long long ms = __ballot(to_sel), mb = __ballot(to_bnd);
+        if (lane == 0) { w_s[wave] = (unsigned int)__popcll(ms); w_b[wave] = (unsigned int)__popcll(mb); }
+        __syncthreads();
+        if (threadIdx.x == 0) {
+            unsigned int ts = 0, tb = 0;
+#pragma unroll
+            for (int w = 0; w < CB_NT / 64; ++w) { ts += w_s[w]; tb += w_b[w]; }
+            unsigned int bs = 0, bb = 0;
+            if (ts) bs = atomicAdd(&counters[2], ts);
+            if (tb) bb = atomicAdd(&counters[3], tb);
+            base[0] = bs; base[1] = bb;
+        }
+        __syncthreads();
+        unsigned int base_s = base[0], base_b = base[1];
+        for (int w = 0; w < wave; ++w) { base_s += w_s[w]; base_b += w_b[w]; }
+        if (to_sel) {
+            const unsigned int pos = base_s + (unsigned int)__popcll(ms & below);
+            if (pos < (unsigned int)sel_cap) sel[pos] = key;
+        } else if (to_bnd) {
+            __hip_atomic_store(bnd + base_b + (unsigned int)__popcll(mb & below), key, __ATOMIC_RELAXED, __HIP_MEMORY_SCOPE_AGENT);
+        }
+        __syncthreads();
+    }
+    compact_boundary_tail<CB_NT>(sel, sel_cap, bnd, counters);
 }
 
 #define RS_KEYS 16
@@ -484,12 +536,13 @@
 
 void launch_topk_sort(hipStream_t st, bool threshold_done, const unsigned long long *cand, int cand_cap, int top_k,
                       unsigned long long *sel, unsigned long long *sorted, int sel_cap, unsigned int *counters,
-                      unsigned long long *bnd, int W, float *kpts, float *scores)
+                      unsigned long long *bnd, int W, float *kpts, float *scores, int block_cursor)
 {
     if (!threshold_done) hipLaunchKernelGGL(select_threshold_kernel, dim3(1), dim3(1024), 0, st, cand_cap, top_k, counters);
     int grid = (cand_cap + NT - 1) / NT;
     if (grid > 256) grid = 256;
-    hipLaunchKernelGGL(compact_selected_kernel, dim3(grid), dim3(NT), 0, st, cand, cand_cap, sel, sel_cap, bnd, counters);
+    if (block_cursor) hipLaunchKernelGGL(compact_selected_block_kernel, dim3((grid * NT + CB_NT - 1) / CB_NT), dim3(CB_NT), 0, st, cand, cand_cap, sel, sel_cap, bnd, counters);
+    else hipLaunchKernelGGL(compact_selected_kernel, dim3(grid), dim3(NT), 0, st, cand, cand_cap, sel, sel_cap, bnd, counters);
     hipLaunchKernelGGL(rank_sort_kernel, dim3((sel_cap + RS_KEYS - 1) / RS_KEYS), dim3(NT), 0, st, sel, sorted, sel_cap, counters, W,
                        kpts, scores);
 }
@@ -645,7 +698,8 @@
 void desc_head_kernel(const half_t *__restrict__ fmap , int hc, int wc, float half_w, float half_h,
                       const half_t *__restrict__ wpk , int CoutP, const float *__restrict__ scale,
                       const float *__restrict__ shift, const float *__restrict__ kpts, const unsigned int *__restrict__ count,
-                      int n_max, float *__restrict__ out, int compact )
+                      int n_max, float *__restrict__ out, int compact ,
+                      half_t *__restrict__ out_f16 )
 {
     __shared__ __attribute__((aligned(16))) unsigned char X[4 * DH_KP * DH_XREC];
     __shared__ __attribute__((aligned(16))) float O[4 * DH_KP * DH_OREC];
@@ -653,6 +707,15 @@
     int n = n_max;
     if (count) { const unsigned int c = *count; if ((unsigned int)n > c) n = (int)c; }
     const int k0 = blockIdx.x * DH_KP;
+    if (out_f16) {
+        for (int j = wave; j < DH_KP; j += NT / 64) {
+            const int kp = k0 + j;
+            if (kp < n || kp >= n_max) continue;
+            const float2 v = *reinterpret_cast<const float2 *>(out + (size_t)kp * 128 + 2 * lane);
+            half_t h[2] = {(half_t)v.x, (half_t)v.y};
+            *reinterpret_cast<unsigned int *>(out_f16 + (size_t)kp * 128 + 2 * lane) = *reinterpret_cast<const unsigned int *>(h);
+        }
+    }
     if (k0 >= n) return;
 
     h8_t a[16];
@@ -733,16 +796,22 @@
         SFD2_TAP(g.vy1 && g.vx1, g.w_se, 3)
 #undef SFD2_TAP
         const float nrm = sqrtf(wave_sum(a0 * a0 + a1 * a1));
-        *reinterpret_cast<float2 *>(out + (size_t)kp * 128 + 2 * lane) = make_float2(__fdiv_rn(a0, nrm), __fdiv_rn(a1, nrm));
+        const float2 d = make_float2(__fdiv_rn(a0, nrm), __fdiv_rn(a1, nrm));
+        *reinterpret_cast<float2 *>(out + (size_t)kp * 128 + 2 * lane) = d;
+        if (out_f16) {
+            half_t h[2] = {(half_t)d.x, (half_t)d.y};
+            *reinterpret_cast<unsigned int *>(out_f16 + (size_t)kp * 128 + 2 * lane) = *reinterpret_cast<const unsigned int *>(h);
+        }
     }
 }
 
 void launch_desc_head(hipStream_t st, const half_t *fmap, int hc, int wc, int nh, int nw, const half_t *wpk, int CoutP,
-                      const float *scale, const float *shift, const float *kpts, const unsigned int *count, int n_max, float *out, int compact)
+                      const float *scale, const float *shift, const float *kpts, const unsigned int *count, int n_max, float *out, int compact,
+                      half_t *out_f16)
 {
     if (n_max <= 0) return;
     hipLaunchKernelGGL(desc_head_kernel, dim3((n_max + DH_KP - 1) / DH_KP), dim3(NT), 0, st, fmap, hc, wc, (float)nw / 2.0f,
-                       (float)nh / 2.0f, wpk, CoutP, scale, shift, kpts, count, n_max, out, compact);
+                       (float)nh / 2.0f, wpk, CoutP, scale, shift, kpts, count, n_max, out, compact, out_f16);
 }
 
 __global__ __launch_bounds__(NT)
diff --git a/sfd2_amd/csrc/sfd2_ctx.h b/sfd2_amd/csrc/sfd2_ctx.h
--- a/sfd2_amd/csrc/sfd2_ctx.h
+++ b/sfd2_amd/csrc/sfd2_ctx.h
@@ -182,6 +182,15 @@
     hipStream_t side_stream = nullptr;
     hipStream_t cur_stream = nullptr;
     hipEvent_t ev_fork = nullptr, ev_join = nullptr;
+    int opt_finalize_fused = 1;
+    int opt_desc_f16_direct = 1;
+    int opt_jobs_static = 1;
+    int opt_topk_block_cursor = 1;
+    bool q16_want = false;
+    const void *q16_src = nullptr;
+    int q16_rows = 0;
+    bool jobs_defer = false;
+    size_t jobs_deferred = 0;
     struct GraphEntry *graphs = nullptr;
     int n_graphs = 0;
     unsigned long long graph_clock = 0;
diff --git a/sfd2_amd/csrc/sfd2_internal.h b/sfd2_amd/csrc/sfd2_internal.h
--- a/sfd2_amd/csrc/sfd2_internal.h
+++ b/sfd2_amd/csrc/sfd2_internal.h
@@ -362,7 +362,8 @@
                        int H, int W, float *heat);
 void launch_topk_sort(hipStream_t st, bool threshold_done, const unsigned long long *cand, int cand_cap, int top_k,
                       unsigned long long *sel, unsigned long long *sorted, int sel_cap, unsigned int *counters,
-                      unsigned long long *bnd, int W, float *kpts, float *scores);
+                      unsigned long long *bnd, int W, float *kpts, float *scores,
+                      int block_cursor = 0);
 #define SFD2_HIST_BINS 4096
 #define SFD2_COUNTER_BYTES (64 + SFD2_HIST_BINS * 4)
 __device__ __forceinline__ unsigned int key_bin(unsigned long long key)
@@ -437,7 +438,8 @@
 bool pb_heads_heat_clears(int hc8, int wc8, int n_zero);
 void launch_desc_store64(hipStream_t st, const float *in , const unsigned int *count, int n_max, double *out , int pitch);
 void launch_desc_head(hipStream_t st, const half_t *fmap, int hc, int wc, int nh, int nw, const half_t *wpk, int CoutP,
-                      const float *scale, const float *shift, const float *kpts, const unsigned int *count, int n_max, float *out, int compact = 0);
+                      const float *scale, const float *shift, const float *kpts, const unsigned int *count, int n_max, float *out, int compact = 0,
+                      half_t *out_f16 = nullptr );
 void launch_desc_normalise_nchw(hipStream_t st, const float *desc_nhwc, int npix, float *out_nchw);
 void launch_nhwc_h_to_nchw_f(hipStream_t st, const half_t *in, int npix, int c_pitch, int c, float *out);
 void launch_nhwc_f_to_nchw_f(hipStream_t st, const float *in, int npix, int c_pitch, int c, float *out);
@@ -475,7 +477,10 @@
 };
 struct MatchFinal;
 void launch_match_mutual(hipStream_t st, const MatchJob2 *jobs_dev, const MatchFinal *fins_dev, int npairs, int max_n0,
-                         int max_n1, int splits, int fwd_ids);
+                         int max_n1, int splits, int fwd_ids, int merge = 1);
+void launch_match_mutual_finalize(hipStream_t st, const MatchJob2 *jobs_dev, const MatchFinal *fins_dev, int npairs, int max_n0, int max_n1, int splits,
+                                  int flavour, int mutual, float ratio, float dist);
+int match_finalize_fused_cap(void);
 int match_mutual_max_chunk(void);
 int match_mutual_strip(void);
 void launch_match_decide(hipStream_t st, const MatchFinal *fin_dev, int npairs, int max_n, int flavour, int mutual,
```

New measurement: 714.6. No clear change (-0.6%).
